# alguoo314/JASPER

Hardware: AMD Instinct MI355X
Metric: assembly Mbp/s polished + Gk-mers/s counted, k=37 (higher is better)
Workload: dtype u64

## Files before the change

jasper_amd/csrc/polish.hip:

```cpp
#include "polish.hpp"
#include <algorithm>

namespace jk {

constexpr int SMAX = 384;

__device__ __forceinline__ void pyslice(int64_t len, int64_t a, int64_t b, int64_t &lo, int64_t &hi) {
    if (a < 0) { a += len; if (a < 0) a = 0; } else if (a > len) a = len;
    if (b < 0) { b += len; if (b < 0) b = 0; } else if (b > len) b = len;
    if (b < a) b = a;
    lo = a; hi = b;
}

__device__ __forceinline__ int64_t pyround(double x) { return (int64_t)rint(x); }

struct FrontEntry {
    uint32_t node;
    uint16_t tlen;
    uint8_t alive;
    uint8_t pad;
    uint8_t tail[72];
};
static_assert(sizeof(FrontEntry) == 80, "FrontEntry layout");

// ... 701 lines not shown
            nlook += 64;
            if (m) {
                const int f = (int)__builtin_ctzll(m);
                if (__shfl((int)oob, f)) spec_fail = 1;
                j = j - (int64_t)f;
                break;
            }
            j -= 64;
        }
        if (j < -1) j = -1;
        int64_t gb = j + k - 1;
        uint32_t prev = cnt_seq(j, k + j);
        if (j == -1) gb = -1;
        for (;;) {
            const int64_t il = i + lane;
            bool cont = false;
            if (il < len - k + 1) cont = cnt_seq(il, il + k) < thre;
            const bool giveup = cont && rolling_thre != 0 && (il - j > k);
            const uint64_t m = __ballot(!cont || giveup);
            nlook += 64;
            if (m) {
                const int f = (int)__builtin_ctzll(m);
                const bool g = __shfl((int)giveup, f) != 0;
                i += f;
                if (!is_last && i >= len - k + 1) spec_fail = 1;
                if (g) return i + 1;
                break;
            }
            i += 64;
        }
        int64_t ga = i;
        nlook += 4;
        if (2ull * cnt_seq(gb - k + 2, gb + 2) < (uint64_t)solid && 2ull * cnt_seq(gb - k + 3, gb + 3) < (uint64_t)solid) {
        } else if (rolling_thre == 0) {
            while (2ull * cnt_seq(gb - k + 2, gb + 2) >= (uint64_t)prev && gb - k + 1 < ga) {
                if (gb == -1) break;
                if (2ull * prev >= (uint64_t)thre && 2ull * cnt_seq(gb - k + 2, gb + 2) < (uint64_t)thre &&
                    2ull * cnt_seq(gb - k + 3, gb + 3) < (uint64_t)thre) break;
                prev = cnt_seq(gb - k + 2, gb + 2);
                gb++;
                nlook += 4;
            }
            if (gb >= len - 1) { if (!is_last) spec_fail = 1; brk = true; return i; }
        }
        int64_t s0 = gb - k + 2; if (s0 < 0) s0 = 0;
        if (s0 + k + k >= len) { if (!is_last) spec_fail = 1; brk = true; return s0 + k + k; }
        {
            uint32_t c = 0;
            if (lane == 0) c = cnt_seq(s0 + 1, s0 + k + 1);
            else if (lane == 1) c = cnt_seq(s0 + k - 2, s0 + k + k - 2);
            else if (lane == 2) c = cnt_seq(s0 + k - 1, s0 + k + k - 1);
            else if (lane == 3) c = cnt_seq(s0 + k, s0 + k + k);
            const uint64_t lowm = __ballot(lane < 4 && c < thre) & 0xFull;
            nlook += 4;
            if (lowm == 0x7ull) ga = s0 + k;
        }
        int64_t tlo, thi;
        pyslice(len, s0, ga + k - 1, tlo, thi);
        int64_t n = ga - s0; if (n < 0) n = 0;
        wrong += n;
        const uint64_t tf0 = phase_clock();
        tk[1] += tf0 - th0;
        struct FixTimer { uint64_t &acc; uint64_t t0; __device__ ~FixTimer() { acc += phase_clock() - t0; } } fix_timer{tk[2], tf0};
        if (fix) {
            if (gb < 0) return i;
            const int64_t L = thi - tlo;
            if (n <= k) {
                if (L > SMAX) { status = PS_STRING_TOO_LONG; return i; }
                cp_seq(s_tbf, tlo, thi);
                sync();
            }
            fixing_sid(L, thre, n, gb, ga);
            sync();
        }
        return i;
    }

    __device__ int64_t skip_good(int64_t i) {
        const int64_t end = len - k + 1;
        for (;;) {
            const int64_t p = i + (int64_t)lane * (k - 1);
            bool ev = true;
            bool known = false;
            if (p < end && cls != nullptr && p >= dirty_end + k) {
                const int64_t o = p - delta + seg_lo;
                if (!is_last && o >= stop_orig) known = true;
                else if (o >= 0 && o < cls_n) { known = true; ev = cls[o] != PC_CLEAN; }
            }
            if (p < end && !known) {
                uint32_t w[16];
                load_window(p, k, w);
                int nv;
                const u128 m = encode_words(w, k, nv);
                const bool valid = nv == k;
                if (valid) {
                    const uint32_t occ = clamp32(table_get(T, mix(canonical(m, k), T.B)));
                    ev = occ < solid;
                    if (!ev && p > 0) {
                        const int64_t a = p - k > 0 ? p - k : 0;
                        const int64_t b = p > k ? p : k;
                        ev = 50ull * occ < (uint64_t)cnt_seq(a, b);
                    }
                }
            }
            const uint64_t mask = __ballot(ev);
            nlook += 128;
            if (mask) return i + (int64_t)__builtin_ctzll(mask) * (k - 1);
            i += 64ll * (k - 1);
        }
    }

    __device__ void walk(bool fix, int64_t start_i, int64_t &wrong_out, long long &arrive_out) {
        int64_t i = start_i, wrong = 0;
        bool handed_over = false;
        arrive_out = ARRIVE_FAIL;
        while (i < len - k + 1 && status == PS_OK) {
            if (__ballot(spec_fail != 0)) { spec_fail = 1; break; }
            const uint64_t ts0 = phase_clock();
            i = skip_good(i);
            tk[0] += phase_clock() - ts0;
            if (i >= len - k + 1) { if (!is_last) spec_fail = 1; break; }
            if (!is_last && (i - delta + seg_lo) >= stop_orig) {
                if (i < dirty_end + k) spec_fail = 1;
                else { handed_over = true; arrive_out = i - delta + seg_lo; }
                break;
            }
            uint8_t ch = 'A';
            if (lane < k) ch = at(i + lane);
            const uint64_t inwin = (k >= 64) ? ~0ull : ((1ull << k) - 1ull);
            const uint64_t mN = __ballot(ch == 'N') & inwin;
            if (mN) {
                const int f = (int)__builtin_ctzll(mN);
                i += f + 1;
                if (f == 0) {
                    for (;;) {
                        const int64_t q = i + lane;
                        const bool stop = !(q < len - k + 1 && at(q) == 'N');
                        const uint64_t m = __ballot(stop);
                        if (m) { i += (int64_t)__builtin_ctzll(m); break; }
                        i += 64;
                    }
                }
                continue;
            }
            const uint64_t mn = __ballot(ch == 'n') & inwin;
            if (mn) { i += (int64_t)__builtin_ctzll(mn) + 1; continue; }
            const uint64_t mo = __ballot(code(ch) < 0) & inwin;
            if (mo) { i += 1; continue; }
            const uint32_t occ = cnt_seq(i, i + k);
            nlook += 1;
            bool brk = false;
            if (occ < solid) {
                i = handle_bad_kmers(i, wrong, fix, 0, brk);
                if (brk) break;
                continue;
            }
            bool cond2 = false;
            if (i > 0) {
                const int64_t a = i - k > 0 ? i - k : 0;
                const int64_t b = i > k ? i : k;
                cond2 = 50ull * occ < (uint64_t)cnt_seq(a, b);
                nlook += 1;
            }
            if (!cond2) { i += k - 1; continue; }
            int64_t ind0 = i - k > 0 ? i - k : 0;
            int64_t num = (i - ind0 + step - 1) / step;
            double sum = 0.0;
            for (int64_t base = 0; base < num; base += 64) {
                const int64_t t = base + lane;
                unsigned long long c = 0;
                if (t < num) { const int64_t ind = ind0 + (t + 1) * step; c = cnt_seq(ind, ind + k); }
                for (int o = 32; o > 0; o >>= 1) c += __shfl_xor(c, o);
                sum += (double)c;
            }
            nlook += (uint64_t)num;
            const int64_t rolling = pyround(sum / (double)num / 50.0);
            if ((int64_t)occ < rolling) {
                i = handle_bad_kmers(i, wrong, fix, pyround(sum / (double)num / 2.0), brk);
                if (brk) break;
            } else {
                i += k - 1;
            }
        }
        if (!is_last && !handed_over && status == PS_OK) spec_fail = 1;
        if (__ballot(spec_fail != 0)) spec_fail = 1;
        if (is_last && status == PS_OK && !spec_fail) arrive_out = ARRIVE_END;
        if (spec_fail || status != PS_OK) arrive_out = ARRIVE_FAIL;
        wrong_out = wrong;
    }
};

__device__ __forceinline__ void publish_arrival(long long *slot, long long v) {
    if (threadIdx.x == 0) __hip_atomic_store(slot, v, __ATOMIC_RELAXED, __HIP_MEMORY_SCOPE_AGENT);
}

__global__ __launch_bounds__(64, 2) void seg_walk_kernel(TableDev T, SegDev *segs, int n_segs, PolishParams P, int pass, ScratchPool pool,
                                                      unsigned int *ticket) {
    __shared__ uint8_t s_tbf[SMAX], s_t1[SMAX], s_t2[SMAX], s_gkb[64], s_gka[64];
    unsigned int tk = 0;
    if (threadIdx.x == 0) tk = atomicAdd(ticket, 1u);
    const int c = (int)__shfl(tk, 0);
    if (c >= n_segs) return;
    SegDev *C = &segs[c];
    if (C->status != PS_OK) { publish_arrival(C->arrive, ARRIVE_FAIL); return; }
    if (!C->chain_in) publish_arrival(C->arrive, ARRIVE_WALKING);
    const int k = P.k;
    const int lane = threadIdx.x;
    const uint64_t t0 = wall_clock64();
    int64_t start_i = C->start_i;
    if (C->chain_in) {
        const int64_t lo = C->seg_lo + 4ll * k;
        int64_t hi = C->last ? C->cls_n : C->stop_orig + k;
        if (hi > C->cls_n) hi = C->cls_n;
        bool dirty = C->cls == nullptr;
        static_assert(PC_CLEAN == 0, "the clean test below ORs class bytes");
        for (int64_t p0 = lo; p0 < hi && !dirty; p0 += 64 * 16) {
            bool nc = false;
            const int64_t p = p0 + (int64_t)lane * 16;
            if (p + 16 <= hi) {
                struct __attribute__((packed, aligned(1))) V16 { uint32_t w[4]; };
                const V16 v = *reinterpret_cast<const V16 *>(C->cls + p);
                nc = (v.w[0] | v.w[1] | v.w[2] | v.w[3]) != 0u;
            } else {
                for (int q = 0; q < 16; ++q) nc = nc || (p + q < hi && C->cls[p + q] != PC_CLEAN);
            }
            dirty = __ballot(nc) != 0ull;
        }
        if (lane == 0) __hip_atomic_store(C->arrive, dirty ? ARRIVE_WALKING : ARRIVE_CLEAN, __ATOMIC_RELAXED, __HIP_MEMORY_SCOPE_AGENT);
        long long a = ARRIVE_FAIL;
        {
            int back = 1;
            for (uint32_t spins = 0;; ++spins) {
                const int idx = c - back - lane;
                long long v = ARRIVE_FAIL;
                if (idx >= 0) v = __hip_atomic_load(C->arrive - (c - idx), __ATOMIC_RELAXED, __HIP_MEMORY_SCOPE_AGENT);
                const bool published = v >= 0 || v == ARRIVE_FAIL || v == ARRIVE_END;
                const bool skip = v == ARRIVE_CLEAN && !dirty;
                const unsigned long long stopper = __ballot(!skip);
                if (stopper) {
                    const int l = (int)__builtin_ctzll(stopper);
                    const bool ok = (__ballot(published) >> l) & 1ull;
                    if (ok) {
                        a = __shfl(v, l);
                        if (back + l > 1 && a >= 0) {
                            const long long stop = segs[c - 1].stop_orig;
                            if (a < stop) a += ((stop - a + (k - 2)) / (k - 1)) * (long long)(k - 1);
                        }
                        break;
                    }
                    if (spins > (1u << 24)) { a = ARRIVE_FAIL; break; }
                    __builtin_amdgcn_s_sleep(4);
                } else {
                    back += 64;
                    if (spins > (1u << 24)) { a = ARRIVE_FAIL; break; }
                }
            }
        }
        if (a < 0 || a < lo || a - C->seg_lo >= C->len0) {
            if (lane == 0) { C->spec_fail = 1; C->ticks = wall_clock64() - t0; }
            publish_arrival(C->arrive, ARRIVE_FAIL);
            return;
        }
        if (!dirty) {
            const int64_t stop = C->last ? C->cls_n : C->stop_orig;
            const int64_t steps = a >= stop ? 0 : (stop - a + (k - 2)) / (k - 1);
            if (lane == 0) {
                C->took_shortcut = 1;
                C->lookups = 2ull * (uint64_t)steps;
                C->ticks = wall_clock64() - t0;
            }
            publish_arrival(C->arrive, C->last ? ARRIVE_END : a + steps * (k - 1));
            return;
        }
        start_i = a - C->seg_lo;
    }
    Walker w;
    w.T = T; w.k = P.k; w.step = P.step; w.lane = threadIdx.x; w.solid = P.solid;
    w.buf = C->buf; w.len = C->len; w.gs = C->gs; w.glen = C->glen; w.cap = C->cap;
    w.C = C; w.chunk_id = C->chunk; w.nrec = 0; w.naux = 0; w.seqno = 0; w.nedit = 0; w.pass = pass;
    w.status = PS_OK; w.nlook = 0; for (int q = 0; q < 12; ++q) w.tk[q] = 0;
    w.s_tbf = s_tbf; w.s_t1 = s_t1; w.s_t2 = s_t2; w.s_gkb = s_gkb; w.s_gka = s_gka;
    w.delta = 0; w.dirty_end = INT64_MIN / 2; w.glo = P.k;
    w.is_first = C->first != 0; w.is_last = C->last != 0; w.spec_fail = 0;
    w.cls = C->cls; w.cls_n = C->cls_n; w.seg_lo = C->seg_lo; w.stop_orig = C->stop_orig;
    w.pool = pool; w.bfs_slot = -1; w.bfs_nodes = nullptr; w.bfs_front = nullptr; w.bfs_patch = nullptr;
    const bool fix = P.fix && pass < P.passes;
    int64_t wrong = 0;
    long long arrive = ARRIVE_FAIL;
    w.walk(fix, start_i, wrong, arrive);
    w.release_scratch();
    if (threadIdx.x == 0) {
        C->ticks = wall_clock64() - t0;
        for (int q = 0; q < 12; ++q) C->tk[q] = w.tk[q];
        C->len = w.len; C->gs = w.gs; C->glen = w.glen;
        C->nrec = w.nrec; C->naux = w.naux; C->nedit = w.nedit; C->status = w.status; C->spec_fail = w.spec_fail;
        C->wrong = wrong;
        C->lookups = w.nlook;
    }
    publish_arrival(C->arrive, arrive);
}

constexpr int SC_THREADS = 256, SC_GROUP = 16, SC_TILE = SC_THREADS * SC_GROUP, SC_HALO = 4;

__global__ __launch_bounds__(256) void seg_init_kernel(SegDev *segs, int n_segs, const uint8_t *const *chunk_text) {
    struct __attribute__((packed, aligned(1))) V16 { uint32_t w[4]; };
    for (int s = blockIdx.y; s < n_segs; s += gridDim.y) {
        const SegDev S = segs[s];
        const uint8_t *src = chunk_text[S.chunk] + S.seg_lo;
        uint8_t *dst = S.buf + S.glen;
        const int64_t nblk = (S.len0 + 15) >> 4;
        for (int64_t blk = blockIdx.x * (int64_t)blockDim.x + threadIdx.x; blk < nblk; blk += (int64_t)gridDim.x * blockDim.x) {
            const int64_t q0 = blk << 4;
            if (q0 + 16 <= S.len0) *reinterpret_cast<V16 *>(dst + q0) = *reinterpret_cast<const V16 *>(src + q0);
            else for (int64_t q = q0; q < S.len0; ++q) dst[q] = src[q];
        }
    }
}

constexpr uint32_t STITCH_MAX_EDITS = 32;
__global__ __launch_bounds__(256) void seg_stitch_kernel(const SegDev *segs, int n_segs, uint8_t *const *chunk_out, uint8_t *const *cls_out,
                                                         uint8_t *const *flags) {
    struct __attribute__((packed, aligned(1))) V16 { uint32_t w[4]; };
    for (int s = blockIdx.y; s < n_segs; s += gridDim.y) {
        const SegDev S = segs[s];
        uint8_t *dst = chunk_out[S.chunk] + S.out_off;
        uint8_t *cdst = cls_out ? cls_out[S.chunk] + S.out_off : nullptr;
        uint8_t *fl = cls_out ? flags[S.chunk] : nullptr;
        const int64_t n = S.own_hi - S.own_lo;
        const bool all_dirty = S.nedit > STITCH_MAX_EDITS;
        const int64_t nblk = (n + 15) >> 4;
        for (int64_t blk = blockIdx.x * (int64_t)blockDim.x + threadIdx.x; blk < nblk; blk += (int64_t)gridDim.x * blockDim.x) {
            const int64_t q0 = blk << 4;
            const int64_t p0 = S.own_lo + q0;
            const bool full = q0 + 16 <= n;
            bool text_done = false, cls_done = !cdst;
            if (full && (p0 + 16 <= S.gs || p0 >= S.gs)) {
                *reinterpret_cast<V16 *>(dst + q0) = *reinterpret_cast<const V16 *>(S.buf + (p0 < S.gs ? p0 : p0 + S.glen));
                text_done = true;
            }
            if (full && cdst && !all_dirty) {
                int64_t lA = p0, lB = p0 + 15;
                bool uniform = true;
                for (int e = (int)S.nedit - 1; e >= 0; --e) {
                    const EditRec E = S.edits[e];
                    if (lA > E.a + E.plen) { const int64_t d = (int64_t)E.plen - E.oldlen; lA -= d; lB -= d; }
                    else if (lB < E.a - 1) { }
                    else { uniform = false; break; }
                }
                if (uniform && S.seg_lo + lB < S.cls_n) {
                    *reinterpret_cast<V16 *>(cdst + q0) = *reinterpret_cast<const V16 *>(S.cls + S.seg_lo + lA);
                    cls_done = true;
                }
            }
            if (text_done && cls_done) continue;
            const int64_t qe = q0 + 16 < n ? q0 + 16 : n;
            for (int64_t q = q0; q < qe; ++q) {
                const int64_t p = S.own_lo + q;
                if (!text_done) dst[q] = S.buf[p < S.gs ? p : p + S.glen];
                if (cls_done) continue;
                int64_t l = p;
                bool dirty = all_dirty;
                if (!dirty)
                    for (int e = (int)S.nedit - 1; e >= 0; --e) {
                        const EditRec E = S.edits[e];
                        if (l > E.a + E.plen) l -= (int64_t)E.plen - E.oldlen;
                        else if (l >= E.a - 1) { dirty = true; break; }
                    }
                if (dirty) {
                    fl[(S.out_off + q) >> 6] = 1;
                    cdst[q] = PC_OTHER;
                } else {
                    const int64_t old = S.seg_lo + l;
                    cdst[q] = old < S.cls_n ? S.cls[old] : (uint8_t)PC_OTHER;
                }
            }
        }
    }
}

__global__ __launch_bounds__(64) void seg_gather_kernel(const SegDev *segs, int n_segs, const int64_t *idx_base, const uint32_t *seq_base,
                                                        const uint32_t *rec_off, const uint32_t *aux_off, FixRec *out_recs, uint8_t *out_aux) {
    const int s = blockIdx.x;
    if (s >= n_segs) return;
    const SegDev S = segs[s];
    for (uint32_t r = threadIdx.x; r < S.nrec; r += blockDim.x) {
        FixRec f = S.recs[r];
        f.index += idx_base[s];
        f.seqno += seq_base[s];
        if (f.kind == 'x') f.aux_off += aux_off[s];
        out_recs[rec_off[s] + r] = f;
    }
    for (uint32_t q = threadIdx.x; q < S.naux; q += blockDim.x) out_aux[aux_off[s] + q] = S.aux[q];
}

__device__ __forceinline__ long long wave_scan_incl64(long long v) {
    const int lane = threadIdx.x & 63;
#pragma unroll
    for (int o = 1; o < 64; o <<= 1) { const long long u = __shfl_up(v, o); if (lane >= o) v += u; }
    return v;
}
__global__ __launch_bounds__(64) void seg_summary_kernel(SegDev *segs, const int32_t *first_seg, int n_chunks, int64_t *idx_base, uint32_t *seq_base,
                                                         uint32_t *rec_off, uint32_t *aux_off, ChunkSummary *out) {
    const int c = blockIdx.x;
    if (c >= n_chunks) return;
    const int lane = threadIdx.x;
    const int s0 = first_seg[c], s1 = first_seg[c + 1];
    long long newlen = 0, shift = 0, seqc = 0, recc = 0, auxc = 0, wrong = 0, lookups = 0;
    int bad = -1, spec = 0;
    for (int base = s0; base < s1; base += 64) {
        const int s = base + lane;
        const bool in = s < s1;
        long long d = 0, own = 0, nrec = 0, naux = 0, seg_lo = 0, own_hi = 0;
        if (in) {
            SegDev &S = segs[s];
            d = S.len - S.len0;
            own_hi = S.last ? S.len : S.own_hi0 + d;
            own = own_hi - S.own_lo;
            nrec = S.nrec; naux = S.naux; seg_lo = S.seg_lo;
            wrong += S.wrong; lookups += (long long)S.lookups;
            if (S.status != PS_OK && (bad < 0 || s < bad)) bad = s;
            if (S.spec_fail && S.status == PS_OK) spec = 1;
        }
        const long long i_own = wave_scan_incl64(own), i_d = wave_scan_incl64(d), i_rec = wave_scan_incl64(nrec), i_aux = wave_scan_incl64(naux);
        if (in) {
            SegDev &S = segs[s];
            S.own_hi = own_hi;
            S.out_off = newlen + i_own - own;
            idx_base[s] = seg_lo + shift + i_d - d;
            seq_base[s] = (uint32_t)(seqc + i_rec - nrec);
            rec_off[s] = (uint32_t)(recc + i_rec - nrec);
            aux_off[s] = (uint32_t)(auxc + i_aux - naux);
        }
        newlen += __shfl(i_own, 63); shift += __shfl(i_d, 63);
        seqc += __shfl(i_rec, 63); recc += __shfl(i_rec, 63); auxc += __shfl(i_aux, 63);
    }
    for (int o = 32; o > 0; o >>= 1) {
        wrong += __shfl_xor(wrong, o); lookups += __shfl_xor(lookups, o);
        const int b2 = __shfl_xor(bad, o);
        bad = bad < 0 ? b2 : (b2 < 0 ? bad : (b2 < bad ? b2 : bad));
        spec |= __shfl_xor(spec, o);
    }
    if (lane == 0) {
        ChunkSummary R;
        R.newlen = newlen; R.wrong = wrong; R.lookups = (uint64_t)lookups; R.nrec = (uint32_t)recc; R.naux = (uint32_t)auxc; R.bad_seg = bad; R.spec_fail = spec;
        out[c] = R;
    }
}
__global__ __launch_bounds__(64) void seg_offsets_kernel(const int32_t *first_seg, int n_chunks, uint32_t *rec_off, uint32_t *aux_off, const ChunkSummary *sum) {
    const int c = blockIdx.x;
    if (c >= n_chunks || c == 0) return;
    const int lane = threadIdx.x;
    unsigned long long rb = 0, ab = 0;
    for (int q = lane; q < c; q += 64) { rb += sum[q].nrec; ab += sum[q].naux; }
    for (int o = 32; o > 0; o >>= 1) { rb += __shfl_xor(rb, o); ab += __shfl_xor(ab, o); }
    for (int s = first_seg[c] + lane; s < first_seg[c + 1]; s += 64) { rec_off[s] += (uint32_t)rb; aux_off[s] += (uint32_t)ab; }
}

constexpr int SC_BACK = 64;
constexpr int SC_STRIDE = SC_TILE - SC_BACK;
__global__ __launch_bounds__(SC_THREADS) void scan_classify_batch_kernel(const ScanChunk *__restrict__ chunks, int n_chunks, TableDev T, uint32_t solid) {
    __shared__ uint32_t s_code[SC_THREADS + SC_HALO];
    __shared__ uint32_t s_inv[SC_THREADS + SC_HALO];
    __shared__ uint32_t s_cnt[SC_TILE];
    __shared__ uint8_t s_ok[SC_TILE];
    const int t = threadIdx.x;
    const int k = T.k;
    const u128 kmask = maskbits(2 * k);
    for (int ci = blockIdx.y; ci < n_chunks; ci += gridDim.y) {
        const ScanChunk C = chunks[ci];
        const uint8_t *__restrict__ text = C.text;
        const int64_t n = C.len;
        const int64_t nwin = n - k + 1;
        if (nwin <= 0) continue;
        const int64_t ntiles = (n + SC_STRIDE - 1) / SC_STRIDE;
        for (int64_t tile = blockIdx.x; tile < ntiles; tile += gridDim.x) {
            const int64_t origin = tile * SC_STRIDE - SC_BACK;
            uint32_t c, iv;
            stage16(text, origin + (int64_t)t * SC_GROUP, n, c, iv);
            s_code[t + SC_HALO] = c;
            s_inv[t + SC_HALO] = iv;
            if (t < SC_HALO) {
                uint32_t hc, hiv;
                stage16(text, origin - (int64_t)(SC_HALO - t) * SC_GROUP, n, hc, hiv);
                s_code[t] = hc;
                s_inv[t] = hiv;
            }
            __syncthreads();
            const uint32_t w4 = s_code[t], w3 = s_code[t + 1], w2 = s_code[t + 2], w1 = s_code[t + 3];
            const uint64_t ivprev = ((uint64_t)s_inv[t] << 48) | ((uint64_t)s_inv[t + 1] << 32) | ((uint64_t)s_inv[t + 2] << 16) |
                                    (uint64_t)s_inv[t + 3];
            u128 fwd = band(mk(((uint64_t)w4 << 32) | w3, ((uint64_t)w2 << 32) | w1), kmask);
            u128 rc = revcomp(fwd, k);
            int run = ivprev ? (int)__builtin_ctzll(ivprev) : 64;
            const int64_t e0 = origin + (int64_t)t * SC_GROUP;
#pragma unroll
            for (int j0 = 0; j0 < SC_GROUP; j0 += 4) {
                u128 hs[4];
                bool ok[4];
                ulonglong2 ent[4];
#pragma unroll
                for (int u = 0; u < 4; ++u) {
                    const int j = j0 + u;
                    const uint32_t cj = (c >> (30 - 2 * j)) & 3u;
                    const bool bad = (iv >> (15 - j)) & 1u;
                    fwd = band(bor(shl(fwd, 2), mk(0, cj)), kmask);
                    rc = bor(shr(rc, 2), shl(mk(0, 3u - cj), 2 * (k - 1)));
                    run = bad ? 0 : run + 1;
                    const int64_t e = e0 + j;
                    ok[u] = run >= k && e - k + 1 >= 0 && e < n;
                    hs[u] = mix(lt(rc, fwd) ? rc : fwd, T.B);
                    ent[u] = make_ulonglong2(0ull, 0ull);
                    if (ok[u]) ent[u] = *reinterpret_cast<const ulonglong2 *>(read_slots(T, hs[u]) + 2 * home_of(hs[u], T.B, T.s));
                }
#pragma unroll
                for (int u = 0; u < 4; ++u) {
                    s_cnt[t * SC_GROUP + j0 + u] = ok[u] ? clamp32(table_get_prefetched(T, hs[u], ent[u])) : 0u;
                    s_ok[t * SC_GROUP + j0 + u] = ok[u] ? 1 : 0;
                }
            }
            __syncthreads();
            if (t >= SC_BACK / SC_GROUP) {
                struct __attribute__((packed, aligned(1))) V16 { uint32_t w[4]; };
                V16 out;
                out.w[0] = out.w[1] = out.w[2] = out.w[3] = 0;
                const int64_t p0 = e0 - k + 1;
#pragma unroll
                for (int j = 0; j < SC_GROUP; ++j) {
                    const int64_t p = p0 + j;
                    const uint32_t me = s_cnt[t * SC_GROUP + j];
                    uint8_t cl;
                    if (!s_ok[t * SC_GROUP + j]) cl = PC_OTHER;
                    else if (me < solid) cl = PC_BAD;
                    else if (p > 0) {
                        const int64_t qe = (p - k > 0 ? p - k : 0) + k - 1;
                        const int qi = (int)(qe - origin);
                        cl = (!s_ok[qi] || 50ull * me < (unsigned long long)s_cnt[qi]) ? PC_OTHER : PC_CLEAN;
                    } else cl = PC_CLEAN;
                    out.w[j >> 2] |= (uint32_t)cl << (8 * (j & 3));
                }
                if (p0 >= 0 && p0 + SC_GROUP <= nwin) *reinterpret_cast<V16 *>(C.cls + p0) = out;
                else {
#pragma unroll
                    for (int j = 0; j < SC_GROUP; ++j) {
                        const int64_t p = p0 + j;
                        if (p >= 0 && p < nwin) C.cls[p] = (uint8_t)((out.w[j >> 2] >> (8 * (j & 3))) & 0xFFu);
                    }
                }
            }
            __syncthreads();
        }
    }
}

__global__ __launch_bounds__(256) void find_sync_batch_kernel(const ScanChunk *__restrict__ chunks, int n_chunks, int k) {
    struct __attribute__((packed, aligned(1))) V16 { uint32_t w[4]; };
    const int64_t W = 4ll * k;
    for (int ci = blockIdx.y; ci < n_chunks; ci += gridDim.y) {
        const ScanChunk C = chunks[ci];
        if (!C.want_sync) continue;
        const int64_t nwin = C.len - k + 1;
        const uint8_t *__restrict__ cls = C.cls;
        static_assert(PC_CLEAN == 0 && PC_BAD == 1 && PC_OTHER == 2, "the block test below looks at bit 0 of the class bytes");
        const int64_t nblk = (nwin + 15) >> 4;
        for (int64_t blk = blockIdx.x * (int64_t)blockDim.x + threadIdx.x; blk < nblk; blk += (int64_t)gridDim.x * blockDim.x) {
            const int64_t p0 = blk << 4;
            uint32_t w[4];
            if (p0 + 16 <= nwin) {
                const V16 v = *reinterpret_cast<const V16 *>(cls + p0);
                w[0] = v.w[0]; w[1] = v.w[1]; w[2] = v.w[2]; w[3] = v.w[3];
                if (!((w[0] | w[1] | w[2] | w[3]) & 0x01010101u)) continue;
            }
            const int64_t pe = p0 + 16 < nwin ? p0 + 16 : nwin;
            for (int64_t p = p0; p < pe; ++p) {
                if (p < W || p + k - 1 > nwin) continue;
                if (cls[p] != PC_BAD || cls[p - 1] != PC_CLEAN) continue;
                uint32_t diff = 0;
                {
                    int64_t q = p + 1;
                    const int64_t qe = p + k - 1;
                    for (; q + 16 <= qe; q += 16) {
                        const V16 v = *reinterpret_cast<const V16 *>(cls + q);
                        diff |= (v.w[0] ^ 0x01010101u) | (v.w[1] ^ 0x01010101u) | (v.w[2] ^ 0x01010101u) | (v.w[3] ^ 0x01010101u);
                    }
                    for (; q < qe; ++q) diff |= (uint32_t)(cls[q] ^ (uint8_t)PC_BAD);
                    q = p - W;
                    const int64_t qf = p - 1;
                    for (; q + 16 <= qf; q += 16) {
                        const V16 v = *reinterpret_cast<const V16 *>(cls + q);
                        diff |= v.w[0] | v.w[1] | v.w[2] | v.w[3];
                    }
                    for (; q < qf; ++q) diff |= (uint32_t)cls[q];
                }
                if (diff) continue;
                const unsigned int idx = atomicAdd(C.cand_count, 1u);
                if (idx < C.cand_cap) C.cand[idx] = ((int64_t)ci << 40) | p;
            }
        }
    }
}

__global__ __launch_bounds__(256) void rescan_batch_kernel(const ScanChunk *__restrict__ chunks, int n_chunks, TableDev T, uint32_t solid) {
    __shared__ uint32_t s_cnt[4][128];
    __shared__ uint8_t s_valid[4][128];
    __shared__ uint8_t s_text[4][256];
    const int wave = threadIdx.x >> 6, lane = threadIdx.x & 63;
    const int k = T.k;
    for (int ci = blockIdx.y; ci < n_chunks; ci += gridDim.y) {
        const ScanChunk C = chunks[ci];
        const int64_t nwin = C.len - k + 1;
        if (nwin <= 0) continue;
        const int64_t ntile = (nwin + 63) >> 6, nflag = (C.len >> 6) + 1;
        const int64_t W = (int64_t)gridDim.x * 4;
        for (int64_t tile0 = (int64_t)blockIdx.x * 4 + wave; tile0 < ntile; tile0 += 64 * W) {
            uint8_t f = 0;
            {
                const int64_t tl = tile0 + (int64_t)lane * W;
                if (tl < ntile) {
                    f = C.flags[tl];
                    if (tl > 0) f |= C.flags[tl - 1];
                    if (tl + 1 < nflag) f |= C.flags[tl + 1];
                }
            }
            unsigned long long todo = __ballot(f != 0);
          while (todo) {
            const int64_t tile = tile0 + (int64_t)__builtin_ctzll(todo) * W;
            todo &= todo - 1ull;
            const int64_t base = tile * 64 - 64;
#pragma unroll
            for (int q = 0; q < 4; ++q) {
                const int64_t pos = base + (int64_t)lane * 4 + q;
                s_text[wave][lane * 4 + q] = (pos >= 0 && pos < C.len) ? C.text[pos] : (uint8_t)'N';
            }
            __builtin_amdgcn_fence(__ATOMIC_SEQ_CST, "workgroup");
            __builtin_amdgcn_wave_barrier();
#pragma unroll
            for (int r = 0; r < 2; ++r) {
                const int64_t p = base + r * 64 + lane;
                uint32_t cnt = 0;
                uint8_t valid = 0;
                if (p >= 0 && p < nwin) {
                    u128 fwd = mk(0, 0);
                    bool ok = true;
                    for (int j = 0; j < k; ++j) {
                        const int c = code(s_text[wave][r * 64 + lane + j]);
                        ok = ok && c >= 0;
                        fwd = bor(shl(fwd, 2), mk(0, (uint64_t)(c & 3)));
                    }
                    if (ok) {
                        cnt = clamp32(table_get(T, mix(canonical(fwd, k), T.B)));
                        valid = 1;
                    }
                }
                s_cnt[wave][r * 64 + lane] = cnt;
                s_valid[wave][r * 64 + lane] = valid;
            }
            __builtin_amdgcn_fence(__ATOMIC_SEQ_CST, "workgroup");
            __builtin_amdgcn_wave_barrier();
            const int64_t p = tile * 64 + lane;
            if (p < nwin) {
                const int me = 64 + lane;
                uint8_t c;
                if (!s_valid[wave][me]) c = PC_OTHER;
                else if (s_cnt[wave][me] < solid) c = PC_BAD;
                else if (p > 0) {
                    const int qi = p - k > 0 ? me - k : 64;
                    c = (!s_valid[wave][qi] || 50ull * s_cnt[wave][me] < (unsigned long long)s_cnt[wave][qi]) ? PC_OTHER : PC_CLEAN;
                } else c = PC_CLEAN;
                C.cls[p] = c;
            }
            __builtin_amdgcn_wave_barrier();
          }
        }
    }
}

__global__ __launch_bounds__(64) void find_clean_batch_kernel(const ScanChunk *__restrict__ chunks, int n_chunks, int k) {
    const int lane = threadIdx.x;
    for (int ci = blockIdx.y; ci < n_chunks; ci += gridDim.y) {
        const ScanChunk C = chunks[ci];
        const int64_t nwin = C.len - k + 1;
        for (uint32_t g = blockIdx.x; g < C.n_cells; g += gridDim.x) {
            int64_t p0 = (int64_t)g * CLEAN_CELL + CLEAN_CELL / 2;
            const int64_t cell_end = (int64_t)(g + 1) * CLEAN_CELL;
            int64_t cand = -1;
            for (int attempt = 0; attempt < 8; ++attempt) {
                if (p0 - 4ll * k < 0 || p0 + k > nwin || p0 + k > cell_end) break;
                int64_t last_bad = -1;
                for (int64_t q0 = p0 - 4ll * k; q0 < p0 + k; q0 += 64) {
                    const int64_t q = q0 + lane;
                    const bool nc = q < p0 + k && C.cls[q] != PC_CLEAN;
                    const uint64_t m = __ballot(nc);
                    if (m) last_bad = q0 + 63 - (int64_t)__builtin_clzll(m);
                }
                if (last_bad < 0) { cand = p0; break; }
                p0 = last_bad + 4ll * k + 1;
            }
            if (lane == 0) C.clean_cand[g] = cand;
        }
    }
}

static void launch_find_clean(const ScanChunk *d_chunks, int n_chunks, int k, hipStream_t stream) {
    const int gy = n_chunks < 1024 ? n_chunks : 1024;
    const int gx = std::max(1, 8192 / gy);
    hipLaunchKernelGGL(find_clean_batch_kernel, dim3(gx, gy), dim3(64), 0, stream, d_chunks, n_chunks, k);
}

void launch_rescan_batch(const TableDev &T, const ScanChunk *d_chunks, int n_chunks, int k, uint32_t solid, hipStream_t stream) {
    if (n_chunks <= 0) return;
    const int gy = n_chunks < 1024 ? n_chunks : 1024;
    const int gx = std::max(1, 4096 / gy);
    hipLaunchKernelGGL(rescan_batch_kernel, dim3(gx, gy), dim3(256), 0, stream, d_chunks, n_chunks, T, solid);
    hipLaunchKernelGGL(find_sync_batch_kernel, dim3(gx, gy), dim3(256), 0, stream, d_chunks, n_chunks, k);
    launch_find_clean(d_chunks, n_chunks, k, stream);
}

void launch_scan_batch(const TableDev &T, const ScanChunk *d_chunks, int n_chunks, int k, uint32_t solid, hipStream_t stream) {
    if (n_chunks <= 0) return;
    const int gy = n_chunks < 1024 ? n_chunks : 1024;
    const int gx = std::max(1, 4096 / gy);
    hipLaunchKernelGGL(scan_classify_batch_kernel, dim3(gx, gy), dim3(SC_THREADS), 0, stream, d_chunks, n_chunks, T, solid);
    hipLaunchKernelGGL(find_sync_batch_kernel, dim3(gx, gy), dim3(256), 0, stream, d_chunks, n_chunks, k);
    launch_find_clean(d_chunks, n_chunks, k, stream);
}

__global__ __launch_bounds__(256) void copy_chunks_kernel(uint8_t *const *__restrict__ chunk_ptr, uint8_t *__restrict__ pack, const int64_t *__restrict__ offs, int n,
                                                          int to_chunks) {
    for (int c = blockIdx.x; c < n; c += gridDim.x) {
        const int64_t len = offs[c + 1] - offs[c];
        uint8_t *a = chunk_ptr[c], *b = pack + offs[c];
        const uint8_t *src = to_chunks ? b : a;
        uint8_t *dst = to_chunks ? a : b;
        for (int64_t i = threadIdx.x; i < len; i += 256) dst[i] = src[i];
    }
}
void launch_copy_chunks(uint8_t *const *d_chunk_ptr, uint8_t *d_pack, const int64_t *d_offs, int n, bool to_chunks, hipStream_t stream) {
    if (n <= 0) return;
    hipLaunchKernelGGL(copy_chunks_kernel, dim3((unsigned)std::min(n, 256 * 16)), dim3(256), 0, stream, d_chunk_ptr, d_pack, d_offs, n, to_chunks ? 1 : 0);
}

void launch_seg_init(SegDev *d_segs, int n_segs, const uint8_t *const *d_chunk_text, hipStream_t stream) {
    if (n_segs <= 0) return;
    dim3 grid(n_segs >= 512 ? 4 : 64, n_segs < 4096 ? n_segs : 4096);
    hipLaunchKernelGGL(seg_init_kernel, grid, dim3(256), 0, stream, d_segs, n_segs, d_chunk_text);
}
void launch_seg_walk(const TableDev &T, SegDev *d_segs, int n_segs, PolishParams pp, int pass, ScratchPool pool, unsigned int *d_ticket,
                     hipStream_t stream) {
    if (n_segs <= 0) return;
    (void)hipMemsetAsync(d_ticket, 0, sizeof(unsigned int), stream);
    hipLaunchKernelGGL(seg_walk_kernel, dim3(n_segs), dim3(64), 0, stream, T, d_segs, n_segs, pp, pass, pool, d_ticket);
}
void launch_seg_summary(SegDev *d_segs, int n_segs, const int32_t *d_first_seg, int n_chunks, int64_t *idx_base, uint32_t *seq_base, uint32_t *rec_off,
                        uint32_t *aux_off, ChunkSummary *d_out, hipStream_t stream) {
    if (n_segs <= 0 || n_chunks <= 0) return;
    hipLaunchKernelGGL(seg_summary_kernel, dim3(n_chunks), dim3(64), 0, stream, d_segs, d_first_seg, n_chunks, idx_base, seq_base, rec_off, aux_off, d_out);
    hipLaunchKernelGGL(seg_offsets_kernel, dim3(n_chunks), dim3(64), 0, stream, d_first_seg, n_chunks, rec_off, aux_off, d_out);
}
void launch_seg_gather(const SegDev *d_segs, int n_segs, const int64_t *idx_base, const uint32_t *seq_base, const uint32_t *rec_off,
                       const uint32_t *aux_off, FixRec *out_recs, uint8_t *out_aux, hipStream_t stream) {
    if (n_segs <= 0) return;
    hipLaunchKernelGGL(seg_gather_kernel, dim3(n_segs), dim3(64), 0, stream, d_segs, n_segs, idx_base, seq_base, rec_off, aux_off, out_recs, out_aux);
}
void launch_seg_stitch(const SegDev *d_segs, int n_segs, uint8_t *const *d_chunk_out, uint8_t *const *d_cls_out, uint8_t *const *d_flags,
                       hipStream_t stream) {
    if (n_segs <= 0) return;
    dim3 grid(n_segs >= 2048 ? 2 : n_segs >= 512 ? 4 : 64, n_segs < 4096 ? n_segs : 4096);
    hipLaunchKernelGGL(seg_stitch_kernel, grid, dim3(256), 0, stream, d_segs, n_segs, d_chunk_out, d_cls_out, d_flags);
}

}
```

jasper_amd/csrc/polish.hpp:

```cpp
#pragma once
#include "table.hpp"

namespace jk {

struct FixRec {
    int64_t index;
    uint32_t chunk;
    uint32_t seqno;
    uint8_t pass;
    uint8_t kind;
    uint8_t newc;
    uint8_t oldc;
    uint32_t rep;
    uint32_t aux_off;
    uint32_t aux_len;
};
static_assert(sizeof(FixRec) == 32, "FixRec layout");

enum PolishStatus {
    PS_OK = 0,
    PS_GAP_EXHAUSTED = 1,
    PS_REC_OVERFLOW = 2,
    PS_AUX_OVERFLOW = 3,
    PS_BFS_ARENA = 4,
    PS_REF_INDEXERROR = 5,
    PS_STRING_TOO_LONG = 6
};

enum PosClass : uint8_t {
    PC_CLEAN = 0,
    PC_BAD = 1,
    PC_OTHER = 2
};

struct ScratchPool {
    unsigned int *locks;
    uint8_t *base;
    size_t stride;
    uint32_t nslots;
    uint32_t node_cap;
    uint32_t front_cap;
    uint32_t patch_cap;
    size_t off_front, off_patch;
};

struct EditRec {
    int64_t a;
    int32_t plen, oldlen;
};

struct SegDev {
    uint8_t *buf;
    int64_t cap;
    int64_t len;
    int64_t gs, glen;
    int64_t len0;
    int64_t seg_lo;
    int64_t start_i;
    int64_t stop_orig;
    int32_t first, last;
    int32_t chain_in;
    int32_t took_shortcut;
    long long *arrive;
    const uint8_t *cls;
    int64_t cls_n;
    FixRec *recs;
    uint32_t rec_cap, nrec;
    uint8_t *aux;
    uint32_t aux_cap, naux;
    EditRec *edits;
    uint32_t edit_cap, nedit;
    uint32_t chunk;
    int32_t status;
    int32_t spec_fail;
    int64_t wrong;
    uint64_t lookups;
    uint64_t ticks;
    uint64_t tk[12];
    int64_t own_lo, own_hi;
    int64_t own_hi0;
    int64_t out_off;
};

struct ChunkSummary {
    int64_t newlen;
    int64_t wrong;
    uint64_t lookups;
    uint32_t nrec, naux;
    int32_t bad_seg;
    int32_t spec_fail;
};

constexpr long long ARRIVE_PENDING = (long long)0x8080808080808080ull;
constexpr long long ARRIVE_FAIL = -2, ARRIVE_END = -1;
constexpr long long ARRIVE_CLEAN = -3, ARRIVE_WALKING = -4;

struct PolishParams {
    int k;
    int step;
    uint32_t solid;
    int passes;
    int fix;
};

struct ScanChunk {
    const uint8_t *text;
    int64_t len;
    uint8_t *cls;
    int64_t *cand;
    unsigned int *cand_count;
    unsigned int cand_cap;
    int32_t want_sync;
    const uint8_t *flags;
    int64_t *clean_cand;
    uint32_t n_cells;
};
constexpr int64_t CLEAN_CELL = 65536;
void launch_scan_batch(const TableDev &T, const ScanChunk *d_chunks, int n_chunks, int k, uint32_t solid, hipStream_t stream);
void launch_rescan_batch(const TableDev &T, const ScanChunk *d_chunks, int n_chunks, int k, uint32_t solid, hipStream_t stream);

void launch_copy_chunks(uint8_t *const *d_chunk_ptr, uint8_t *d_pack, const int64_t *d_offs, int n, bool to_chunks, hipStream_t stream);
void launch_seg_init(SegDev *d_segs, int n_segs, const uint8_t *const *d_chunk_text, hipStream_t stream);
void launch_seg_walk(const TableDev &T, SegDev *d_segs, int n_segs, PolishParams pp, int pass, ScratchPool pool, unsigned int *d_ticket,
                     hipStream_t stream);
void launch_seg_stitch(const SegDev *d_segs, int n_segs, uint8_t *const *d_chunk_out, uint8_t *const *d_cls_out, uint8_t *const *d_flags,
                       hipStream_t stream);
void launch_seg_summary(SegDev *d_segs, int n_segs, const int32_t *d_first_seg, int n_chunks, int64_t *idx_base, uint32_t *seq_base, uint32_t *rec_off,
                        uint32_t *aux_off, ChunkSummary *d_out, hipStream_t stream);
void launch_seg_gather(const SegDev *d_segs, int n_segs, const int64_t *idx_base, const uint32_t *seq_base, const uint32_t *rec_off,
                       const uint32_t *aux_off, FixRec *out_recs, uint8_t *out_aux, hipStream_t stream);

}
```

jasper_amd/csrc/polish_host.hip:

```cpp
#include "polish_host.hpp"
#include <algorithm>
#include <chrono>
#include <cstdio>
#include <cstdlib>
#include <cstring>
#include <thread>

namespace jk {

#define HIPCHK(x)                                                                     \
    do {                                                                              \
        hipError_t e_ = (x);                                                          \
        if (e_ != hipSuccess) {                                                       \
            err = std::string(#x) + ": " + hipGetErrorString(e_);                     \
            return -1;                                                                \
        }                                                                             \
    } while (0)

static inline size_t al256(size_t x) { return (x + 255) & ~(size_t)255; }

namespace {
struct DevBuf {
    void *p = nullptr;
    bool owned = false;
    ~DevBuf() { if (p && owned) (void)hipFree(p); }
    template <typename T> T *as() { return reinterpret_cast<T *>(p); }
};
}

static int run_polish_lane(Table &T, const int lane, hipStream_t st, int n_chunks, const char *const *seqs, const int64_t *lens, int solid_thre, int passes, int fix,
                           PolishOut &R, std::string &err, bool device_in, bool keep_on_device, int roomy) {
    const int64_t RM = roomy ? 8 : 1;
    const bool tight = !roomy && getenv("JASPER_POLISH_TIGHT") != nullptr;
    const int k = T.k;
    const int64_t W = 4ll * k;
    const int64_t M = 3ll * k;
    const int64_t TMIN = 1024;
    const int64_t CMIN = 32768;
    HIPCHK(hipSetDevice(T.device));
    const int ws_base = lane ? Table::WS_LANE0 + (lane - 1) * Table::WS_POLISH_MAX : 0, pin_base = lane * Table::PIN_PER_LANE;
    R.seqs.assign(n_chunks, std::string());
    R.d_seqs.clear();
    R.d_lens.clear();
    R.aux.assign(n_chunks, std::string());
    R.recs.clear();
    R.qv[0] = R.qv[1] = R.qv[2] = R.qv[3] = 0;
    R.qv_chunk.assign((size_t)4 * n_chunks, 0);
    R.lookups = 0;
    R.seconds = 0;
    R.n_segments = 0;
    R.n_respeculated = 0;
    if (n_chunks == 0) return 0;

    const bool dbg = getenv("JASPER_POLISH_DEBUG") != nullptr;
    auto now = []() { return std::chrono::duration<double, std::milli>(std::chrono::steady_clock::now().time_since_epoch()).count(); };
    const double t_begin = now();
    std::vector<int64_t> len(lens, lens + n_chunks), cap(n_chunks);
    std::vector<size_t> off_text(n_chunks), off_pos(n_chunks), off_cand(n_chunks), off_flag(n_chunks), off_cell(n_chunks);
    std::vector<uint32_t> n_cells(n_chunks);
    size_t cell_items = 0;
    std::vector<uint32_t> cand_cap(n_chunks);
    size_t text_bytes = 0, pos_items = 0, cand_items = 0, flag_items = 0, seg_text_bound = 0, seg_rec_bound = 0, seg_aux_bound = 0;
    int64_t max_segs = 0;
    for (int c = 0; c < n_chunks; ++c) {
        cap[c] = len[c] + RM * std::max<int64_t>(4096, len[c] / 8) + 64;
        off_text[c] = text_bytes;  text_bytes += al256((size_t)cap[c]);
        off_pos[c] = pos_items;    pos_items += al256((size_t)cap[c]);
        cand_cap[c] = (uint32_t)std::min<int64_t>(1 << 28, cap[c] / (4 * k) + 16);
        off_cand[c] = cand_items;  cand_items += cand_cap[c];
        off_flag[c] = flag_items;  flag_items += al256((size_t)(cap[c] >> 6) + 2);
        n_cells[c] = (uint32_t)(cap[c] / CLEAN_CELL + 1);
        off_cell[c] = cell_items;  cell_items += n_cells[c];
        const int64_t ms = cap[c] / TMIN + 2;
        max_segs += ms;
        const int64_t tb = cap[c] + ms * (W + M + 64);
        seg_text_bound += (size_t)(tb + RM * (tb / 8 + ms * 1280));
        seg_rec_bound += (size_t)(RM * (2 * tb / k + 16 * ms));
        seg_aux_bound += (size_t)(RM * (2 * tb + 1024 * ms));
    }
    DevBuf b_textA, b_textB, b_pack, b_cls, b_clsB, b_flags, b_segedit, b_cells, b_arrive, b_ptrA, b_segs, b_segtext, b_segrec, b_segaux, b_pool, b_locks, b_scan, b_ticket;
    int ws_next = 0;
    auto dmalloc = [&](DevBuf &b, size_t bytes) -> bool {
        if (ws_next >= Table::WS_POLISH_MAX) { err = "polish: workspace slots exhausted"; return false; }
        b.p = T.workspace(ws_base + ws_next++, bytes, err);
        b.owned = false;
        return b.p != nullptr;
    };
    if (!dmalloc(b_textA, text_bytes) || !dmalloc(b_textB, text_bytes) || 
        !dmalloc(b_cls, pos_items) || !dmalloc(b_clsB, pos_items) || !dmalloc(b_flags, flag_items) ||
        !dmalloc(b_segedit, seg_rec_bound * sizeof(EditRec)) || !dmalloc(b_cells, (2 + cell_items + cand_items) * 8) ||
        !dmalloc(b_arrive, ((size_t)max_segs + 4) * 8) ||
        !dmalloc(b_ptrA, (size_t)6 * n_chunks * sizeof(void *)) ||
        !dmalloc(b_segs, (size_t)max_segs * sizeof(SegDev)) || !dmalloc(b_segtext, seg_text_bound) ||
        !dmalloc(b_segrec, seg_rec_bound * sizeof(FixRec)) || !dmalloc(b_segaux, seg_aux_bound))
        return -2;
    ScratchPool pool;
    pool.nslots = 256;
    pool.node_cap = (uint32_t)(RM << 18);
    pool.front_cap = 20480;
    pool.patch_cap = (uint32_t)(RM << 16);
    if (roomy) pool.nslots = 64;
    if (const char *e = getenv("JASPER_POLISH_TEST_NSLOTS")) pool.nslots = (uint32_t)std::max(1, std::min(atoi(e), 256));
    pool.off_front = al256((size_t)pool.node_cap * 4);
    pool.off_patch = pool.off_front + al256((size_t)pool.front_cap * 80);
    pool.stride = pool.off_patch + al256(pool.patch_cap);
    if (!dmalloc(b_pool, pool.stride * pool.nslots) || !dmalloc(b_locks, pool.nslots * 4) || !dmalloc(b_scan, sizeof(ScanChunk) * n_chunks) ||
        !dmalloc(b_ticket, 256)) return -2;
    DevBuf b_first, b_sum, b_idx, b_seq, b_ro, b_ao;
    if (!dmalloc(b_first, ((size_t)n_chunks + 1) * 4) || !dmalloc(b_sum, (size_t)n_chunks * sizeof(ChunkSummary)) || !dmalloc(b_idx, (size_t)max_segs * 8) ||
        !dmalloc(b_seq, (size_t)max_segs * 4) || !dmalloc(b_ro, (size_t)max_segs * 4) || !dmalloc(b_ao, (size_t)max_segs * 4)) return -2;
    const size_t PIN_RECS = 1u << 18, PIN_AUX = 8u << 20;
    SegDev *segs_p = reinterpret_cast<SegDev *>(T.pinned(pin_base + 0, (size_t)max_segs * sizeof(SegDev), err));
    int32_t *first_p = reinterpret_cast<int32_t *>(T.pinned(pin_base + 1, ((size_t)n_chunks + 1) * 4, err));
    ChunkSummary *sum_p = reinterpret_cast<ChunkSummary *>(T.pinned(pin_base + 2, (size_t)n_chunks * sizeof(ChunkSummary), err));
    int64_t *cand_p = reinterpret_cast<int64_t *>(T.pinned(pin_base + 3, (std::min<size_t>(cand_items, 32768) + cell_items + 8) * 8, err));
    FixRec *recs_p = reinterpret_cast<FixRec *>(T.pinned(pin_base + 4, PIN_RECS * sizeof(FixRec), err));
    uint8_t *aux_p = reinterpret_cast<uint8_t *>(T.pinned(pin_base + 5, PIN_AUX, err));
    ScanChunk *sc_p = reinterpret_cast<ScanChunk *>(T.pinned(pin_base + 6, sizeof(ScanChunk) * (size_t)n_chunks, err));
    if (!segs_p || !first_p || !sum_p || !cand_p || !recs_p || !aux_p || !sc_p) return -2;
    int64_t total_len = 0;
    for (int c = 0; c < n_chunks; ++c) total_len += len[c];
    const bool packed_io = !device_in && n_chunks > 256 && total_len / n_chunks < 65536 && !getenv("JASPER_POLISH_NO_PACKED_IO");
    DevBuf b_iooffs;
    std::vector<int64_t> io_offs;
    uint8_t *io_stage = nullptr;
    if (!packed_io) ws_next += 2;
    if (packed_io) {
        if (!dmalloc(b_iooffs, ((size_t)n_chunks + 1) * 8) || !dmalloc(b_pack, text_bytes)) return -2;
        io_offs.resize((size_t)n_chunks + 1);
        io_stage = reinterpret_cast<uint8_t *>(T.pinned(pin_base + 7, std::max<size_t>((size_t)total_len, 1) + (size_t)(RM * std::max<int64_t>(4096, total_len / 8)) + 64, err));
        if (!io_stage) return -2;
    }
    size_t pin_recs_used = 0, pin_aux_used = 0;
    struct PinnedPass { size_t rec_at, nrec, aux_at, naux, r0, pass_i; };
    std::vector<PinnedPass> pinned_passes;
    pool.base = b_pool.as<uint8_t>();
    pool.locks = b_locks.as<unsigned int>();
    HIPCHK(hipMemsetAsync(pool.locks, 0, pool.nslots * 4, st));

    uint8_t *clsIn = b_cls.as<uint8_t>(), *clsOut = b_clsB.as<uint8_t>();
    std::vector<uint8_t *> tables((size_t)6 * n_chunks);
    uint8_t **hIn = tables.data(), **hOut = hIn + n_chunks, **hSpare = hOut + n_chunks, **hCA = hSpare + n_chunks, **hCB = hCA + n_chunks,
            **hF = hCB + n_chunks;
    for (int c = 0; c < n_chunks; ++c) {
        uint8_t *a = b_textA.as<uint8_t>() + off_text[c];
        hIn[c] = device_in ? reinterpret_cast<uint8_t *>(const_cast<char *>(seqs[c])) : a;
        hOut[c] = b_textB.as<uint8_t>() + off_text[c];
        hSpare[c] = a;
        hCA[c] = b_cls.as<uint8_t>() + off_pos[c];
        hCB[c] = b_clsB.as<uint8_t>() + off_pos[c];
        hF[c] = b_flags.as<uint8_t>() + off_flag[c];
        if (len[c] && !device_in && !packed_io) HIPCHK(hipMemcpyAsync(a, seqs[c], (size_t)len[c], hipMemcpyHostToDevice, st));
    }
    HIPCHK(hipMemcpyAsync(b_ptrA.p, tables.data(), tables.size() * sizeof(void *), hipMemcpyHostToDevice, st));
    uint8_t **dIn = b_ptrA.as<uint8_t *>(), **dOut = dIn + n_chunks, **dSpare = dOut + n_chunks;
    uint8_t **ptrClsIn = dSpare + n_chunks, **ptrClsOut = ptrClsIn + n_chunks, **ptrFlags = ptrClsOut + n_chunks;
    if (packed_io) {
        int64_t at = 0;
        for (int c = 0; c < n_chunks; ++c) { io_offs[c] = at; if (len[c]) memcpy(io_stage + at, seqs[c], (size_t)len[c]); at += len[c]; }
        io_offs[n_chunks] = at;
        HIPCHK(hipMemcpyAsync(b_iooffs.p, io_offs.data(), io_offs.size() * 8, hipMemcpyHostToDevice, st));
        if (at) HIPCHK(hipMemcpyAsync(b_pack.p, io_stage, (size_t)at, hipMemcpyHostToDevice, st));
        launch_copy_chunks(dIn, b_pack.as<uint8_t>(), b_iooffs.as<int64_t>(), n_chunks, true, st);
        HIPCHK(hipGetLastError());
        HIPCHK(jk_stream_wait(st));
    }

    if (dbg) { (void)jk_stream_wait(st); fprintf(stderr, "[polish] setup + H2D: %.2f ms\n", now() - t_begin); }
    const double t_loop = now();
    PolishParams pp;
    pp.k = k;
    pp.step = std::max(2, (int)std::nearbyint((double)k / 8.0));
    pp.solid = (uint32_t)solid_thre;
    pp.passes = passes;
    pp.fix = fix ? 1 : 0;

    hipEvent_t ev0, ev1;
    HIPCHK(hipEventCreate(&ev0));
    HIPCHK(hipEventCreate(&ev1));
    HIPCHK(hipEventRecord(ev0, st));

    std::vector<SegDev> segs;
    std::vector<ScanChunk> sc(n_chunks);
    int64_t *const d_count = b_cells.as<int64_t>(), *const d_cells = d_count + 2, *const d_cands = d_cells + cell_items;
    std::vector<int64_t> all_cands(cand_items);
    std::vector<int64_t> all_cells(cell_items);
    std::vector<std::vector<int64_t>> chunk_cands(n_chunks);
    std::vector<int64_t> cands;
    std::vector<uint32_t> aux_total(n_chunks, 0);
    std::vector<std::vector<uint8_t>> aux_pass;
    std::vector<size_t> rec_pass_begin;
    int rc = 0;

    for (int pass = 0; pass <= passes && rc == 0; ++pass) {
        HIPCHK(hipMemsetAsync(d_count, 0, 4, st));
        {
            for (int c = 0; c < n_chunks; ++c) {
                ScanChunk &S = sc[c];
                S.text = hIn[c];
                S.len = len[c];
                S.cls = clsIn + off_pos[c];
                S.flags = b_flags.as<uint8_t>() + off_flag[c];
                S.cand = d_cands;
                S.cand_count = reinterpret_cast<unsigned int *>(d_count);
                S.cand_cap = (unsigned int)std::min<size_t>(cand_items, 0x7fffffffu);
                S.want_sync = (len[c] - k + 1) > 2 * TMIN;
                S.clean_cand = d_cells + off_cell[c];
                S.n_cells = (uint32_t)std::min<int64_t>(n_cells[c], std::max<int64_t>(0, len[c] - k + 1) / CLEAN_CELL + 1);
            }
            memcpy(sc_p, sc.data(), sizeof(ScanChunk) * n_chunks);
            HIPCHK(hipMemcpyAsync(b_scan.p, sc_p, sizeof(ScanChunk) * n_chunks, hipMemcpyHostToDevice, st));
            if (pass == 0) launch_scan_batch(T.d, b_scan.as<ScanChunk>(), n_chunks, k, pp.solid, st);
            else launch_rescan_batch(T.d, b_scan.as<ScanChunk>(), n_chunks, k, pp.solid, st);
        }
        HIPCHK(hipGetLastError());
        const size_t CAND_PRE = std::min<size_t>(cand_items, 32768);
        unsigned int n_cand = 0;
        {
            HIPCHK(hipMemcpyAsync(cand_p, d_count, (2 + cell_items + CAND_PRE) * 8, hipMemcpyDeviceToHost, st));
            HIPCHK(jk_stream_wait(st));
            n_cand = *reinterpret_cast<const unsigned int *>(cand_p);
            if (cell_items) memcpy(all_cells.data(), cand_p + 2, cell_items * 8);
            if (CAND_PRE) memcpy(all_cands.data(), cand_p + 2 + cell_items, std::min<size_t>(n_cand, CAND_PRE) * 8);
        }
        n_cand = (unsigned int)std::min<size_t>(n_cand, cand_items);
        if (n_cand > CAND_PRE) {
            HIPCHK(hipMemcpyAsync(all_cands.data() + CAND_PRE, d_cands + CAND_PRE, (n_cand - CAND_PRE) * 8, hipMemcpyDeviceToHost, st));
            HIPCHK(jk_stream_wait(st));
        }
        for (int c = 0; c < n_chunks; ++c) chunk_cands[c].clear();
        for (unsigned int i = 0; i < n_cand; ++i) {
            const int64_t v = all_cands[i];
            const int64_t c = v >> 40;
            if (c >= 0 && c < n_chunks) chunk_cands[c].push_back(v & ((1ll << 40) - 1));
        }

        auto build_segments = [&](const std::vector<int> &chunks, bool speculate, SegDev *out, size_t &n_out, int32_t *first_of, std::string &e2) -> int {
            n_out = 0;
            size_t tpos = 0, rpos = 0, apos = 0, ci = 0;
            for (int c : chunks) {
                if (first_of) first_of[ci++] = (int32_t)n_out;
                std::vector<int64_t> sync;
                if (speculate && !chunk_cands[c].empty()) {
                    cands = chunk_cands[c];
                    std::sort(cands.begin(), cands.end());
                    int64_t last = 0;
                    for (int64_t p : cands)
                        if (p - last >= TMIN && len[c] - p >= TMIN) { sync.push_back(p); last = p; }
                }
                std::vector<char> chained(sync.size(), 0);
                if (speculate && len[c] - k + 1 > 2 * CMIN) {
                    const uint32_t nc = sc[c].n_cells;
                    std::vector<int64_t> merged;
                    std::vector<char> mtype;
                    size_t si = 0;
                    int64_t last = 0;
                    for (uint32_t g = 0; g <= nc; ++g) {
                        const int64_t p = g < nc ? all_cells[off_cell[c] + g] : INT64_MAX;
                        while (si < sync.size() && sync[si] <= p) { merged.push_back(sync[si]); mtype.push_back(0); last = sync[si]; ++si; }
                        if (g == nc || p < 0) continue;
                        const int64_t next = si < sync.size() ? sync[si] : len[c];
                        if (p - last >= CMIN && next - p >= CMIN) { merged.push_back(p); mtype.push_back(1); last = p; }
                    }
                    sync.swap(merged);
                    chained.swap(mtype);
                }
                const int m = (int)sync.size();
                if ((int64_t)n_out + m + 1 > max_segs) { e2 = "polish: internal segment arena bound exceeded"; return -2; }
                for (int j = 0; j <= m; ++j) {
                    SegDev &S = out[n_out++];
                    memset(&S, 0, sizeof S);
                    S.chunk = (uint32_t)c;
                    S.first = (j == 0);
                    S.last = (j == m);
                    S.seg_lo = j == 0 ? 0 : sync[j - 1] - W;
                    S.start_i = j == 0 ? 0 : W;
                    S.chain_in = j > 0 && chained[j - 1];
                    S.arrive = b_arrive.as<long long>() + n_out;
                    S.stop_orig = j == m ? INT64_MAX : sync[j];
                    const int64_t seg_hi = j == m ? len[c] : std::min<int64_t>(len[c], sync[j] + M);
                    S.len0 = seg_hi - S.seg_lo;
                    S.len = S.len0;
                    S.cap = S.len0 + (tight ? 2 : RM * std::max<int64_t>(1024, S.len0 / 8));
                    S.gs = 0;
                    S.glen = S.cap - S.len0;
                    S.cls = (len[c] - k + 1 > 0) ? clsIn + off_pos[c] : nullptr;
                    S.cls_n = std::max<int64_t>(0, len[c] - k + 1);
                    S.rec_cap = (uint32_t)std::min<int64_t>(0x7fffffff, RM * (2 * S.len0 / k + 16));
                    S.aux_cap = (uint32_t)std::min<int64_t>(0x7fffffff, RM * (2 * S.len0 + 1024));
                    S.buf = b_segtext.as<uint8_t>() + tpos;            tpos += al256((size_t)S.cap);
                    S.recs = b_segrec.as<FixRec>() + rpos;
                    S.edits = b_segedit.as<EditRec>() + rpos;
                    S.edit_cap = S.rec_cap;                            rpos += S.rec_cap;
                    S.aux = b_segaux.as<uint8_t>() + apos;             apos += al256(S.aux_cap);
                    S.own_lo = j == 0 ? 0 : 2ll * k;
                    S.own_hi = j == m ? -1 : (sync[j] - 2ll * k) - S.seg_lo;
                    S.own_hi0 = S.own_hi;
                }
            }
            if (first_of) first_of[ci] = (int32_t)n_out;
            if (tpos > seg_text_bound || rpos > seg_rec_bound || apos > seg_aux_bound || (int64_t)n_out > max_segs) {
                e2 = "polish: internal segment arena bound exceeded"; return -2;
            }
            return 0;
        };
        auto run_segments = [&](SegDev *sv, size_t nsv, bool summary, std::string &e2) -> int {
            if (!nsv) return 0;
            const bool fine = dbg && getenv("JASPER_POLISH_DEBUG") && atoi(getenv("JASPER_POLISH_DEBUG")) >= 2;
            double tf[5] = {fine ? now() : 0, 0, 0, 0, 0};
            if (hipMemcpyAsync(b_segs.p, sv, nsv * sizeof(SegDev), hipMemcpyHostToDevice, st) != hipSuccess) { e2 = "polish: H2D segs"; return -1; }
            if (summary && hipMemcpyAsync(b_first.p, first_p, ((size_t)n_chunks + 1) * 4, hipMemcpyHostToDevice, st) != hipSuccess) { e2 = "polish: H2D first"; return -1; }
            if (fine) { (void)jk_stream_wait(st); tf[1] = now(); }
            launch_seg_init(b_segs.as<SegDev>(), (int)nsv, (const uint8_t *const *)dIn, st);
            if (hipMemsetAsync(b_arrive.p, 0x80, (nsv + 2) * 8, st) != hipSuccess) { e2 = "polish: memset"; return -1; }
            if (fine) { (void)jk_stream_wait(st); tf[2] = now(); }
            launch_seg_walk(T.d, b_segs.as<SegDev>(), (int)nsv, pp, pass, pool, b_ticket.as<unsigned int>(), st);
            if (hipGetLastError() != hipSuccess) { e2 = "polish: kernel launch failed"; return -1; }
            if (fine) { (void)jk_stream_wait(st); tf[3] = now(); }
            if (summary) {
                launch_seg_summary(b_segs.as<SegDev>(), (int)nsv, b_first.as<int32_t>(), n_chunks, b_idx.as<int64_t>(), b_seq.as<uint32_t>(), b_ro.as<uint32_t>(),
                                   b_ao.as<uint32_t>(), b_sum.as<ChunkSummary>(), st);
                if (hipMemcpyAsync(sum_p, b_sum.p, (size_t)n_chunks * sizeof(ChunkSummary), hipMemcpyDeviceToHost, st) != hipSuccess) { e2 = "polish: D2H summary"; return -1; }
            } else if (hipMemcpyAsync(sv, b_segs.p, nsv * sizeof(SegDev), hipMemcpyDeviceToHost, st) != hipSuccess) { e2 = "polish: D2H segs"; return -1; }
            if (jk_stream_wait(st) != hipSuccess) { e2 = "polish: kernel execution failed"; return -1; }
            if (fine) {
                tf[4] = now();
                fprintf(stderr, "[polish]     %zu segments x %zu B: H2D %.3f ms, init + memset %.3f ms, walk %.3f ms, %s %.3f ms\n", nsv, sizeof(SegDev), tf[1] - tf[0], tf[2] - tf[1],
                        tf[3] - tf[2], summary ? "summary + D2H" : "D2H", tf[4] - tf[3]);
            }
            return 0;
        };
        std::vector<int> all(n_chunks);
        for (int c = 0; c < n_chunks; ++c) all[c] = c;
        const double tb0 = dbg ? now() : 0;
        size_t ns = 0;
        if ((rc = build_segments(all, true, segs_p, ns, first_p, err))) break;
        const double tb1 = dbg ? now() : 0;
        if ((rc = run_segments(segs_p, ns, true, err))) break;
        if (dbg) fprintf(stderr, "[polish]   host: build %zu segments %.3f ms, upload + walk + summary %.3f ms\n", ns, tb1 - tb0, now() - tb1);

        bool ordinary = !getenv("JASPER_POLISH_DEBUG") && !getenv("JASPER_POLISH_HOST_BOOKKEEPING");
        for (int c = 0; c < n_chunks && ordinary; ++c) ordinary = sum_p[c].bad_seg < 0 && !sum_p[c].spec_fail;
        std::vector<int64_t> idx_base;
        std::vector<uint32_t> seq_base, rec_off, aux_off;
        std::vector<int64_t> newlen(n_chunks, 0), shift(n_chunks, 0);
        std::vector<uint32_t> seqc(n_chunks, 0);
        size_t nrec_pass = 0, naux_pass = 0;
        if (ordinary) {
            R.n_segments += ns;
            for (int c = 0; c < n_chunks; ++c) {
                const ChunkSummary &S = sum_p[c];
                newlen[c] = S.newlen;
                nrec_pass += S.nrec;
                naux_pass += S.naux;
                R.lookups += S.lookups;
                if (pass == 0) { R.qv[0] += S.wrong; R.qv_chunk[4 * (size_t)c + 0] += S.wrong; }
                if (pass == passes) { R.qv[2] += S.wrong; R.qv_chunk[4 * (size_t)c + 2] += S.wrong; }
            }
        } else {
        segs.resize(ns);
        HIPCHK(hipMemcpyAsync(segs.data(), b_segs.p, ns * sizeof(SegDev), hipMemcpyDeviceToHost, st));
        HIPCHK(jk_stream_wait(st));
        R.n_segments += segs.size();

        std::vector<char> failed(n_chunks, 0);
        bool any_failed = false;
        for (const SegDev &S : segs)
            if (S.spec_fail && S.status == PS_OK) { failed[S.chunk] = 1; any_failed = true; }
        if (any_failed) {
            std::vector<int> redo;
            for (int c = 0; c < n_chunks; ++c) if (failed[c]) redo.push_back(c);
            R.n_respeculated += redo.size();
            std::vector<SegDev> good, bad;
            for (const SegDev &S : segs) if (!failed[S.chunk]) good.push_back(S);
            size_t tpos = 0, rpos = 0, apos = 0;
            for (const SegDev &S : segs) { tpos += al256((size_t)S.cap); rpos += S.rec_cap; apos += al256(S.aux_cap); }
            std::vector<SegDev> redo_segs((size_t)max_segs);
            size_t nredo = 0;
            if ((rc = build_segments(redo, false, redo_segs.data(), nredo, nullptr, err))) break;
            redo_segs.resize(nredo);
            size_t t2 = tpos, r2 = rpos, a2 = apos;
            for (SegDev &S : redo_segs) {
                S.buf = b_segtext.as<uint8_t>() + t2;  t2 += al256((size_t)S.cap);
                S.recs = b_segrec.as<FixRec>() + r2;
                S.edits = b_segedit.as<EditRec>() + r2; r2 += S.rec_cap;
                S.aux = b_segaux.as<uint8_t>() + a2;   a2 += al256(S.aux_cap);
            }
            if (t2 > seg_text_bound || r2 > seg_rec_bound || a2 > seg_aux_bound) {
                segs.assign((size_t)max_segs, SegDev{});
                size_t nall = 0;
                if ((rc = build_segments(all, false, segs.data(), nall, nullptr, err))) break;
                segs.resize(nall);
                if ((rc = run_segments(segs.data(), segs.size(), false, err))) break;
            } else {
                if ((rc = run_segments(redo_segs.data(), redo_segs.size(), false, err))) break;
                segs = good;
                segs.insert(segs.end(), redo_segs.begin(), redo_segs.end());
                std::stable_sort(segs.begin(), segs.end(), [](const SegDev &a, const SegDev &b) {
                    return a.chunk != b.chunk ? a.chunk < b.chunk : a.seg_lo < b.seg_lo;
                });
            }
        }
        if (getenv("JASPER_POLISH_DEBUG")) {
            uint64_t mx = 0, sum = 0, mxl = 0; int64_t mxlen = 0; size_t nrecs = 0, mxrec = 0;
            uint64_t tks[12] = {0, 0, 0, 0, 0, 0, 0, 0, 0, 0, 0, 0}, mxtk[12] = {0, 0, 0, 0, 0, 0, 0, 0, 0, 0, 0, 0};
            for (const SegDev &S : segs) {
                sum += S.ticks; nrecs += S.nrec;
                for (int q = 0; q < 12; ++q) tks[q] += S.tk[q];
                if (S.ticks > mx) { mx = S.ticks; mxl = S.lookups; mxlen = S.len0; mxrec = S.nrec; for (int q = 0; q < 12; ++q) mxtk[q] = S.tk[q]; }
            }
            fprintf(stderr, "[polish] pass %d: %zu segments, %zu records, walk ticks(10ns): mean %.0f max %llu (that segment: len %lld, %llu lookups, %zu records)\n",
                    pass, segs.size(), nrecs, segs.empty() ? 0.0 : (double)sum / segs.size(), (unsigned long long)mx, (long long)mxlen,
                    (unsigned long long)mxl, mxrec);
            fprintf(stderr, "[polish]   of all walk ticks: skip_good %.1f%%, find run %.1f%%, choose fix %.1f%% (of which splice %.1f%%)\n",
                    100.0 * tks[0] / (sum + 1), 100.0 * tks[1] / (sum + 1), 100.0 * tks[2] / (sum + 1), 100.0 * tks[3] / (sum + 1));
            fprintf(stderr, "[polish]   inside choose fix: k_case_sub %.1f%%, insert %.1f%%, del %.1f%%, diploid %.1f%%, same_base_del %.1f%%, same_base_ins %.1f%%, path search %.1f%%\n",
                    100.0 * tks[4] / (sum + 1), 100.0 * tks[5] / (sum + 1), 100.0 * tks[6] / (sum + 1), 100.0 * tks[7] / (sum + 1),
                    100.0 * tks[8] / (sum + 1), 100.0 * tks[9] / (sum + 1), 100.0 * tks[10] / (sum + 1));
            fprintf(stderr, "[polish]   slowest segment (10ns ticks): skip %llu, find run %llu, choose fix %llu [sub %llu ins %llu del %llu diploid %llu sb_del %llu sb_ins %llu path %llu], splice %llu\n",
                    (unsigned long long)mxtk[0], (unsigned long long)mxtk[1], (unsigned long long)mxtk[2], (unsigned long long)mxtk[4], (unsigned long long)mxtk[5],
                    (unsigned long long)mxtk[6], (unsigned long long)mxtk[7], (unsigned long long)mxtk[8], (unsigned long long)mxtk[9], (unsigned long long)mxtk[10],
                    (unsigned long long)mxtk[3]);
            int hb[8] = {0, 0, 0, 0, 0, 0, 0, 0};
            for (const SegDev &S : segs) { double ms = S.ticks * 1e-5; int b = ms < 0.1 ? 0 : ms < 0.3 ? 1 : ms < 1 ? 2 : ms < 2 ? 3 : ms < 4 ? 4 : ms < 8 ? 5 : ms < 16 ? 6 : 7; hb[b]++; }
            fprintf(stderr, "[polish]   segments by walk time: <0.1ms %d, <0.3 %d, <1 %d, <2 %d, <4 %d, <8 %d, <16 %d, more %d\n", hb[0], hb[1], hb[2], hb[3], hb[4], hb[5], hb[6], hb[7]);
        }

        ns = segs.size();
        idx_base.assign(ns, 0);
        seq_base.assign(ns, 0); rec_off.assign(ns, 0); aux_off.assign(ns, 0);
        for (size_t s = 0; s < ns && rc == 0; ++s) {
            SegDev &S = segs[s];
            const int c = (int)S.chunk;
            if (S.status != PS_OK) {
                static const char *names[] = {"ok", "text grew beyond its slack", "fix-record buffer overflow", "aux buffer overflow",
                                              "path-extension scratch exhausted", "reference IndexError (src/jasper.py:221)",
                                              "trial string too long"};
                err = std::string("polish: chunk ") + std::to_string(c) + ": " + names[S.status];
                rc = S.status == PS_REF_INDEXERROR ? -4 : -2;
                break;
            }
            const int64_t d = S.len - S.len0;
            S.own_hi = S.last ? S.len : S.own_hi0 + d;
            S.out_off = newlen[c];
            newlen[c] += S.own_hi - S.own_lo;
            idx_base[s] = S.seg_lo + shift[c];
            shift[c] += d;
            seq_base[s] = seqc[c];
            seqc[c] += S.nrec;
            rec_off[s] = (uint32_t)nrec_pass;
            aux_off[s] = (uint32_t)naux_pass;
            nrec_pass += S.nrec;
            naux_pass += S.naux;
            R.lookups += S.lookups;
            if (pass == 0) { R.qv[0] += S.wrong; R.qv_chunk[4 * (size_t)c + 0] += S.wrong; }
            if (pass == passes) { R.qv[2] += S.wrong; R.qv_chunk[4 * (size_t)c + 2] += S.wrong; }
        }
        if (rc) break;
        }
        if (rc) break;
        for (int c = 0; c < n_chunks; ++c) {
            if (pass == 0) { R.qv[1] += len[c] - k + 1; R.qv_chunk[4 * (size_t)c + 1] += len[c] - k + 1; }
            if (pass == passes) { R.qv[3] += len[c] - k + 1; R.qv_chunk[4 * (size_t)c + 3] += len[c] - k + 1; }
            if (newlen[c] > cap[c]) { err = "polish: chunk grew beyond its slack"; rc = -2; }
        }
        if (rc) break;

        rec_pass_begin.push_back(R.recs.size());
        aux_pass.emplace_back();
        const int64_t *g_idx = b_idx.as<int64_t>();
        const uint32_t *g_seq = b_seq.as<uint32_t>(), *g_ro = b_ro.as<uint32_t>(), *g_ao = b_ao.as<uint32_t>();
        if (!ordinary) {
            HIPCHK(hipMemcpyAsync(b_segs.p, segs.data(), ns * sizeof(SegDev), hipMemcpyHostToDevice, st));
            HIPCHK(hipMemcpyAsync(b_idx.p, idx_base.data(), ns * 8, hipMemcpyHostToDevice, st));
            HIPCHK(hipMemcpyAsync(b_seq.p, seq_base.data(), ns * 4, hipMemcpyHostToDevice, st));
            HIPCHK(hipMemcpyAsync(b_ro.p, rec_off.data(), ns * 4, hipMemcpyHostToDevice, st));
            HIPCHK(hipMemcpyAsync(b_ao.p, aux_off.data(), ns * 4, hipMemcpyHostToDevice, st));
        }
        if (nrec_pass) {
            DevBuf d_recs, d_aux;
            int ws_save = ws_next;
            if (!dmalloc(d_recs, nrec_pass * sizeof(FixRec)) || !dmalloc(d_aux, naux_pass)) { rc = -2; break; }
            ws_next = ws_save;
            launch_seg_gather(b_segs.as<SegDev>(), (int)ns, g_idx, g_seq, g_ro, g_ao, d_recs.as<FixRec>(), d_aux.as<uint8_t>(), st);
            HIPCHK(hipGetLastError());
            const size_t r0 = R.recs.size();
            R.recs.resize(r0 + nrec_pass);
            aux_pass.back().resize(naux_pass);
            if (pin_recs_used + nrec_pass <= PIN_RECS && pin_aux_used + naux_pass <= PIN_AUX) {
                HIPCHK(hipMemcpyAsync(recs_p + pin_recs_used, d_recs.p, nrec_pass * sizeof(FixRec), hipMemcpyDeviceToHost, st));
                if (naux_pass) HIPCHK(hipMemcpyAsync(aux_p + pin_aux_used, d_aux.p, naux_pass, hipMemcpyDeviceToHost, st));
                pinned_passes.push_back(PinnedPass{pin_recs_used, nrec_pass, pin_aux_used, naux_pass, r0, aux_pass.size() - 1});
                pin_recs_used += nrec_pass;
                pin_aux_used += naux_pass;
            } else {
                HIPCHK(hipMemcpyAsync(&R.recs[r0], d_recs.p, nrec_pass * sizeof(FixRec), hipMemcpyDeviceToHost, st));
                if (naux_pass) HIPCHK(hipMemcpyAsync(aux_pass.back().data(), d_aux.p, naux_pass, hipMemcpyDeviceToHost, st));
                HIPCHK(jk_stream_wait(st));
            }
        }
        const bool carry = pass < passes;
        if (carry) HIPCHK(hipMemsetAsync(b_flags.p, 0, flag_items, st));
        launch_seg_stitch(b_segs.as<SegDev>(), (int)ns, (uint8_t *const *)dOut, carry ? (uint8_t *const *)ptrClsOut : nullptr,
                          carry ? (uint8_t *const *)ptrFlags : nullptr, st);
        HIPCHK(hipGetLastError());
        for (int c = 0; c < n_chunks; ++c) len[c] = newlen[c];
        if (!ordinary) HIPCHK(jk_stream_wait(st));
        std::swap(hIn, hOut);
        std::swap(dIn, dOut);
        if (pass == 0) { hOut = hSpare; dOut = dSpare; }
        std::swap(clsIn, clsOut);
        std::swap(ptrClsIn, ptrClsOut);
    }
    if (dbg) { (void)jk_stream_wait(st); fprintf(stderr, "[polish] passes: %.2f ms\n", now() - t_loop); }
    const double t_out = now();
    if (rc == 0) {
        HIPCHK(hipEventRecord(ev1, st));
        if (keep_on_device) {
            R.d_seqs.resize(n_chunks);
            R.d_lens.assign(len.begin(), len.end());
            for (int c = 0; c < n_chunks; ++c) R.d_seqs[c] = hIn[c];
        }
        bool packed_back = false;
        if (packed_io && !keep_on_device) {
            int64_t at = 0;
            for (int c = 0; c < n_chunks; ++c) { io_offs[c] = at; at += len[c]; }
            io_offs[n_chunks] = at;
            if ((size_t)at <= text_bytes && (size_t)at <= (size_t)total_len + (size_t)(RM * std::max<int64_t>(4096, total_len / 8)) + 64) {
                packed_back = true;
                HIPCHK(hipMemcpyAsync(b_iooffs.p, io_offs.data(), io_offs.size() * 8, hipMemcpyHostToDevice, st));
                launch_copy_chunks(dIn, b_pack.as<uint8_t>(), b_iooffs.as<int64_t>(), n_chunks, false, st);
                HIPCHK(hipGetLastError());
                if (at) HIPCHK(hipMemcpyAsync(io_stage, b_pack.p, (size_t)at, hipMemcpyDeviceToHost, st));
            }
        }
        for (int c = 0; c < n_chunks && !keep_on_device && !packed_back; ++c) {
            R.seqs[c].resize((size_t)len[c]);
            if (len[c]) HIPCHK(hipMemcpyAsync(&R.seqs[c][0], hIn[c], (size_t)len[c], hipMemcpyDeviceToHost, st));
        }
        HIPCHK(jk_stream_wait(st));
        if (packed_back)
            for (int c = 0; c < n_chunks; ++c) R.seqs[c].assign(reinterpret_cast<const char *>(io_stage) + io_offs[c], (size_t)len[c]);
        float ms = 0;
        HIPCHK(hipEventElapsedTime(&ms, ev0, ev1));
        R.seconds = ms * 1e-3;
        for (const PinnedPass &P : pinned_passes) {
            memcpy(&R.recs[P.r0], recs_p + P.rec_at, P.nrec * sizeof(FixRec));
            if (P.naux) memcpy(aux_pass[P.pass_i].data(), aux_p + P.aux_at, P.naux);
        }
        for (size_t p = 0; p < rec_pass_begin.size(); ++p) {
            const size_t b = rec_pass_begin[p], e = p + 1 < rec_pass_begin.size() ? rec_pass_begin[p + 1] : R.recs.size();
            for (size_t i = b; i < e; ++i) {
                FixRec &f = R.recs[i];
                if (f.kind == 'x') {
                    std::string &a = R.aux[f.chunk];
                    const size_t n = (size_t)f.aux_len + f.rep;
                    const uint32_t no = (uint32_t)a.size();
                    a.append(reinterpret_cast<const char *>(aux_pass[p].data()) + f.aux_off, n);
                    f.aux_off = no;
                }
            }
        }
        std::stable_sort(R.recs.begin(), R.recs.end(), [](const FixRec &a, const FixRec &b) {
            if (a.chunk != b.chunk) return a.chunk < b.chunk;
            if (a.pass != b.pass) return a.pass < b.pass;
            return a.seqno < b.seqno;
        });
    }
    (void)jk_stream_wait(st);
    if (dbg) fprintf(stderr, "[polish] D2H + record sort: %.2f ms; total %.2f ms\n", now() - t_out, now() - t_begin);
    (void)hipEventDestroy(ev0);
    (void)hipEventDestroy(ev1);
    return rc;
}

int run_polish(Table &T, int n_chunks, const char *const *seqs, const int64_t *lens, int solid_thre, int passes, int fix,
               PolishOut &R, std::string &err, bool device_in, bool keep_on_device, int roomy) {
    HIPCHK(hipSetDevice(T.device));
    if (T.materialize(err)) return -1;
    int lanes = T.polish_calls++ >= 1 && n_chunks >= 12 ? 3 : 1;
    if (const char *e = getenv("JASPER_POLISH_LANES")) lanes = atoi(e);
    if (getenv("JASPER_POLISH_DEBUG")) lanes = 1;
    lanes = std::max(1, std::min(std::min(lanes, (int)Table::POLISH_LANES_MAX), n_chunks / 2));
    if (lanes == 1) return run_polish_lane(T, 0, T.stream, n_chunks, seqs, lens, solid_thre, passes, fix, R, err, device_in, keep_on_device, roomy);

    std::vector<int> order(n_chunks);
    for (int c = 0; c < n_chunks; ++c) order[c] = c;
    std::stable_sort(order.begin(), order.end(), [&](int a, int b) { return lens[a] > lens[b]; });
    std::vector<std::vector<int>> mine(lanes);
    std::vector<int64_t> load(lanes, 0);
    for (int c : order) {
        int l = 0;
        for (int j = 1; j < lanes; ++j) if (load[j] < load[l]) l = j;
        mine[l].push_back(c);
        load[l] += lens[c];
    }
    for (auto &m : mine) std::sort(m.begin(), m.end());
    if (!T.polish_ev) HIPCHK(hipEventCreateWithFlags(&T.polish_ev, hipEventDisableTiming));
    HIPCHK(hipEventRecord(T.polish_ev, T.stream));
    for (int l = 1; l < lanes; ++l) {
        if (!T.polish_stream[l]) HIPCHK(hipStreamCreateWithFlags(&T.polish_stream[l], hipStreamNonBlocking));
        HIPCHK(hipStreamWaitEvent(T.polish_stream[l], T.polish_ev, 0));
    }
    std::vector<PolishOut> out(lanes);
    std::vector<std::string> errs(lanes);
    std::vector<int> rcs(lanes, 0);
    std::vector<std::vector<const char *>> lseqs(lanes);
    std::vector<std::vector<int64_t>> llens(lanes);
    for (int l = 0; l < lanes; ++l)
        for (int c : mine[l]) { lseqs[l].push_back(seqs[c]); llens[l].push_back(lens[c]); }
    auto run = [&](int l) {
        rcs[l] = run_polish_lane(T, l, l ? T.polish_stream[l] : T.stream, (int)mine[l].size(), lseqs[l].data(), llens[l].data(), solid_thre, passes, fix, out[l],
                                 errs[l], device_in, keep_on_device, roomy);
    };
    {
        std::vector<std::thread> th;
        for (int l = 1; l < lanes; ++l) th.emplace_back(run, l);
        run(0);
        for (auto &t : th) t.join();
    }
    for (int want : {-1, -4, -2})
        for (int l = 0; l < lanes; ++l)
            if (rcs[l] == want) { err = errs[l]; return want; }
    for (int l = 0; l < lanes; ++l)
        if (rcs[l]) { err = errs[l]; return rcs[l]; }
    R.seqs.assign(n_chunks, std::string());
    R.aux.assign(n_chunks, std::string());
    R.d_seqs.clear();
    R.d_lens.clear();
    if (keep_on_device) { R.d_seqs.assign(n_chunks, nullptr); R.d_lens.assign(n_chunks, 0); }
    R.recs.clear();
    R.qv[0] = R.qv[1] = R.qv[2] = R.qv[3] = 0;
    R.qv_chunk.assign((size_t)4 * n_chunks, 0);
    R.lookups = 0; R.seconds = 0; R.n_segments = 0; R.n_respeculated = 0;
    for (int l = 0; l < lanes; ++l) {
        PolishOut &O = out[l];
        for (size_t j = 0; j < mine[l].size(); ++j) {
            const int c = mine[l][j];
            R.seqs[c].swap(O.seqs[j]);
            R.aux[c].swap(O.aux[j]);
            if (keep_on_device) { R.d_seqs[c] = O.d_seqs[j]; R.d_lens[c] = O.d_lens[j]; }
            for (int q = 0; q < 4; ++q) R.qv_chunk[4 * (size_t)c + q] = O.qv_chunk[4 * j + q];
        }
        for (FixRec f : O.recs) { f.chunk = (uint32_t)mine[l][f.chunk]; R.recs.push_back(f); }
        for (int q = 0; q < 4; ++q) R.qv[q] += O.qv[q];
        R.lookups += O.lookups;
        R.n_segments += O.n_segments;
        R.n_respeculated += O.n_respeculated;
        R.seconds = std::max(R.seconds, O.seconds);
    }
    std::stable_sort(R.recs.begin(), R.recs.end(), [](const FixRec &a, const FixRec &b) {
        if (a.chunk != b.chunk) return a.chunk < b.chunk;
        if (a.pass != b.pass) return a.pass < b.pass;
        return a.seqno < b.seqno;
    });
    return 0;
}

}
```

jasper_amd/csrc/table.hip:

```cpp
#include "table.hpp"
#include <algorithm>
#include <cmath>
#include <cstdio>
#include <cstdlib>
#include <cstring>
#include <ctime>
#include <thread>
#include <chrono>
#include <vector>

namespace jk {

#define HIPCHK(x)                                                                     \
    do {                                                                              \
        hipError_t e_ = (x);                                                          \
        if (e_ != hipSuccess) {                                                       \
            err = std::string(#x) + ": " + hipGetErrorString(e_);                     \
            return -1;                                                                \
        }                                                                             \
    } while (0)

constexpr int CT_THREADS = 256;
constexpr int CT_GROUP = 16;
constexpr int CT_TILE = CT_THREADS * CT_GROUP;
// ... 311 lines not shown
        if (have && idx < cap) out[(size_t)owner * cap + idx] = o;
        __syncthreads();
    }
}

__device__ __forceinline__ int table_set(const TableDev &T, u128 h, unsigned long long val) {
    if (T.ext) return table_put_wide(T, h, val, true);
    const uint64_t home = home_of(h, T.B, T.s);
    const uint64_t rem = rem_of(h, T.B, T.s);
    for (uint32_t off = 0; off < MAXPROBE; ++off) {
        const uint64_t slot = (home + off) & T.mask;
        const unsigned long long want = tag_of(rem, off);
        unsigned long long *p = T.slots + 2 * slot;
        unsigned long long cur = __hip_atomic_load(p, __ATOMIC_RELAXED, __HIP_MEMORY_SCOPE_AGENT);
        int fresh = 1;
        if (cur == 0ull) {
            cur = atomicCAS(p, 0ull, want);
            if (cur == 0ull) { fresh = 2; cur = want; }
        }
        if (cur == want) {
            __hip_atomic_store(p + 1, val, __ATOMIC_RELAXED, __HIP_MEMORY_SCOPE_AGENT);
            return fresh;
        }
    }
    return 0;
}

__global__ __launch_bounds__(256) void import_packed_kernel(const ulonglong2 *__restrict__ in, uint64_t n, TableDev T, int mode) {
    unsigned long long fresh = 0;
    const int sh = packed_count_shift(T.B);
    const unsigned long long himask = sh ? ((1ull << sh) - 1ull) : 0ull;
    for (uint64_t i = blockIdx.x * (uint64_t)blockDim.x + threadIdx.x; i < n; i += (uint64_t)gridDim.x * blockDim.x) {
        const ulonglong2 e = in[i];
        const u128 h = mk(e.y & himask, e.x);
        const unsigned long long c = sh ? (e.y >> sh) : e.y;
        if (!c) continue;
        if (mode == 0) fresh += table_add_or_spill(T, h, c);
        else {
            const int r = table_set(T, h, c);
            if (r == 2) ++fresh;
            else if (r == 0) table_spill(T, h, c);
        }
    }
    for (int o = 32; o > 0; o >>= 1) fresh += __shfl_xor(fresh, o);
    if ((threadIdx.x & 63) == 0 && fresh) atomicAdd(&T.stats[ST_DISTINCT], fresh);
}

struct MultiSrc { const ulonglong2 *p[MAX_SHARDS]; unsigned long long n[MAX_SHARDS]; uint32_t n_src; };
constexpr uint32_t IMP_BPC = 64;
__global__ __launch_bounds__(256) void import_packed_multi_kernel(MultiSrc S, uint32_t nchunks, TableDev T) {
    unsigned long long fresh = 0;
    const int sh = packed_count_shift(T.B);
    const unsigned long long himask = sh ? ((1ull << sh) - 1ull) : 0ull;
    const uint32_t c = blockIdx.x / IMP_BPC, j = blockIdx.x % IMP_BPC;
#pragma unroll 1
    for (uint32_t s = 0; s < S.n_src; ++s) {
        const ulonglong2 *__restrict__ in = S.p[s];
        const unsigned long long lo = S.n[s] / nchunks * c + (S.n[s] % nchunks) * c / nchunks;
        const unsigned long long hi = c + 1 == nchunks ? S.n[s] : S.n[s] / nchunks * (c + 1) + (S.n[s] % nchunks) * (c + 1) / nchunks;
        for (unsigned long long i = lo + (unsigned long long)j * 256 + threadIdx.x; i < hi; i += (unsigned long long)IMP_BPC * 256) {
            const ulonglong2 e = in[i];
            const u128 h = mk(e.y & himask, e.x);
            const unsigned long long cnt = sh ? (e.y >> sh) : e.y;
            if (cnt) fresh += table_add_or_spill(T, h, cnt);
        }
    }
    for (int o = 32; o > 0; o >>= 1) fresh += __shfl_xor(fresh, o);
    if ((threadIdx.x & 63) == 0 && fresh) atomicAdd(&T.stats[ST_DISTINCT], fresh);
}

constexpr uint32_t IMPR_LOG = 12, IMPR = 1u << IMPR_LOG;
__global__ __launch_bounds__(256) void imp_region_hist_kernel(MultiSrc S, TableDev T, uint32_t nreg, unsigned int *__restrict__ hist) {
    const int sh = packed_count_shift(T.B);
    const unsigned long long himask = sh ? ((1ull << sh) - 1ull) : 0ull;
    for (uint32_t s = 0; s < S.n_src; ++s) {
        const ulonglong2 *__restrict__ in = S.p[s];
        unsigned int *__restrict__ hs = hist + (size_t)s * (nreg + 1);
        const unsigned long long n = S.n[s], step = (unsigned long long)gridDim.x * blockDim.x;
        for (unsigned long long i0 = (unsigned long long)blockIdx.x * blockDim.x; i0 < n; i0 += step) {
            const unsigned long long i = i0 + threadIdx.x;
            uint32_t reg = 0xFFFFFFFFu;
            if (i < n) {
                const ulonglong2 e = in[i];
                reg = (uint32_t)(home_of(mk(e.y & himask, e.x), T.B, T.s) >> IMPR_LOG);
            }
            uint64_t todo = __ballot(reg != 0xFFFFFFFFu);
            while (todo) {
                const int leader = (int)__builtin_ctzll(todo);
                const uint32_t r = __shfl(reg, leader);
                const uint64_t same = __ballot(reg == r);
                if ((threadIdx.x & 63) == leader) atomicAdd(&hs[r], (unsigned int)__popcll(same));
                todo &= ~same;
            }
        }
    }
}
__global__ __launch_bounds__(1024) void imp_region_scan_kernel(unsigned int *__restrict__ hist, uint32_t nreg) {
    __shared__ unsigned int s_w[16];
    __shared__ unsigned int s_carry;
    unsigned int *h = hist + (size_t)blockIdx.x * (nreg + 1);
    const int t = threadIdx.x;
    if (t == 0) s_carry = 0;
    __syncthreads();
    for (uint32_t base = 0; base < nreg; base += 1024) {
        const unsigned int v = base + t < nreg ? h[base + t] : 0u;
        unsigned int inc = v;
        for (int o = 1; o < 64; o <<= 1) { const unsigned int u = __shfl_up(inc, o); if ((t & 63) >= o) inc += u; }
        if ((t & 63) == 63) s_w[t >> 6] = inc;
        __syncthreads();
        unsigned int wbase = s_carry;
        for (int w = 0; w < (t >> 6); ++w) wbase += s_w[w];
        if (base + t < nreg) h[base + t] = wbase + inc - v;
        __syncthreads();
        if (t == 1023) s_carry = wbase + inc;
        __syncthreads();
    }
    if (t == 0) h[nreg] = s_carry;
}
__global__ __launch_bounds__(256) void lds_import_kernel(MultiSrc S, TableDev T, uint32_t nreg, const unsigned int *__restrict__ bounds,
                                                         ulonglong2 *__restrict__ deferred, unsigned long long *__restrict__ deferred_n, unsigned long long deferred_cap) {
    __shared__ unsigned long long s_tag[IMPR];
    __shared__ unsigned long long s_cnt[IMPR];
    __shared__ unsigned int s_fresh[4];
    const uint32_t r = blockIdx.x;
    const int sh = packed_count_shift(T.B);
    const unsigned long long himask = sh ? ((1ull << sh) - 1ull) : 0ull;
    for (uint32_t j = threadIdx.x; j < IMPR; j += 256) { s_tag[j] = 0ull; s_cnt[j] = 0ull; }
    __syncthreads();
    unsigned int fresh = 0;
    for (uint32_t s = 0; s < S.n_src; ++s) {
        const ulonglong2 *__restrict__ in = S.p[s];
        const unsigned int *__restrict__ b = bounds + (size_t)s * (nreg + 1);
        const unsigned int lo = b[r], hi = b[r + 1];
        for (unsigned int i = lo + threadIdx.x; i < hi; i += 256) {
            const ulonglong2 e = in[i];
            const u128 h = mk(e.y & himask, e.x);
            const unsigned long long c = sh ? (e.y >> sh) : e.y;
            if (!c) continue;
            const uint64_t home = home_of(h, T.B, T.s);
            bool placed = false;
            if ((uint32_t)(home >> IMPR_LOG) == r) {
                const uint64_t rem = rem_of(h, T.B, T.s);
                const uint32_t local = (uint32_t)(home & (IMPR - 1));
                for (uint32_t off = 0; off < MAXPROBE && local + off < IMPR; ++off) {
                    const unsigned long long want = tag_of(rem, off);
                    unsigned long long cur = s_tag[local + off];
                    if (cur == 0ull) {
                        cur = atomicCAS(&s_tag[local + off], 0ull, want);
                        if (cur == 0ull) { ++fresh; cur = want; }
                    }
                    if (cur == want) { atomicAdd(&s_cnt[local + off], c); placed = true; break; }
                }
            }
            if (!placed) {
                const unsigned long long di = atomicAdd(deferred_n, 1ull);
                if (di < deferred_cap) deferred[di] = e;
            }
        }
    }
    __syncthreads();
    ulonglong2 *out = reinterpret_cast<ulonglong2 *>(T.slots) + (size_t)r * IMPR;
    for (uint32_t j = threadIdx.x; j < IMPR; j += 256) out[j] = make_ulonglong2(s_tag[j], s_cnt[j]);
    for (int o = 32; o > 0; o >>= 1) fresh += __shfl_xor(fresh, o);
    if ((threadIdx.x & 63) == 0) s_fresh[threadIdx.x >> 6] = fresh;
    __syncthreads();
    if (threadIdx.x == 0) {
        const unsigned int f = s_fresh[0] + s_fresh[1] + s_fresh[2] + s_fresh[3];
        if (f) atomicAdd(&T.stats[ST_DISTINCT], (unsigned long long)f);
    }
}

__global__ __launch_bounds__(256) void zero_kernel(ulonglong2 *__restrict__ p, uint64_t n16) {
    for (uint64_t i = blockIdx.x * (uint64_t)blockDim.x + threadIdx.x; i < n16; i += (uint64_t)gridDim.x * blockDim.x)
        p[i] = make_ulonglong2(0ull, 0ull);
}

__global__ __launch_bounds__(256) void rehash_kernel(TableDev oldT, TableDev newT) {
    unsigned long long fresh = 0;
    const uint64_t nslots = oldT.mask + 1;
    for (uint64_t i = blockIdx.x * (uint64_t)blockDim.x + threadIdx.x; i < nslots; i += (uint64_t)gridDim.x * blockDim.x) {
        const ulonglong2 e = *reinterpret_cast<const ulonglong2 *>(oldT.slots + 2 * i);
        if (e.x == 0ull) continue;
        fresh += table_add_or_spill(newT, slot_hash(oldT, i, e.x), e.y);
    }
    for (int o = 32; o > 0; o >>= 1) fresh += __shfl_xor(fresh, o);
    if ((threadIdx.x & 63) == 0 && fresh) atomicAdd(&newT.stats[ST_DISTINCT], fresh);
}

static size_t slot_alloc_bytes(uint64_t nslots) {
    size_t b = (size_t)nslots * 16;
    if ((b & (1ull << 31)) && !getenv("JASPER_NO_IPC_PAD")) b += 1ull << 31;
    return b;
}

static int grid_for(uint64_t work_items, int per_block) {
    uint64_t b = (work_items + per_block - 1) / per_block;
    const uint64_t cap = 256ull * 8;
    if (b > cap) b = cap;
    if (b < 1) b = 1;
    return (int)b;
}

int Table::min_log2_slots(int k) {
    int need = 2 * k - (63 - OFFBITS) - 64;
    return std::max(need, 10);
}

int Table::init(int k_, uint64_t min_slots, int device_, std::string &err) {
    if (k_ < 1 || k_ > 64) { err = "k must be in [1,64]"; return -1; }
    k = k_;
    device = device_;
    HIPCHK(hipSetDevice(device));
    if (const char *e = getenv("JASPER_EXPERIMENT_CU_MASK")) {
        uint32_t m[8];
        for (int w = 0; w < 8; ++w)
            m[w] = !strcmp(e, "alt2") ? 0x55555555u : !strcmp(e, "alt4x3") ? 0x77777777u : !strcmp(e, "lo128") ? (w < 4 ? ~0u : 0u) : !strcmp(e, "lo192") ? (w < 6 ? ~0u : 0u) : ~0u;
        HIPCHK(hipExtStreamCreateWithCUMask(&stream, 8, m));
    } else
    HIPCHK(hipStreamCreateWithFlags(&stream, hipStreamNonBlocking));
    int s = min_log2_slots(k);
    size_hint = min_slots;
    while ((1ull << s) < min_slots) ++s;
    if (s > 2 * k) s = 2 * k;
    if (s < min_log2_slots(k)) {
        err = "internal: slot count below tag-format minimum"; return -1;
    }
    nslots = 1ull << s;
    d = TableDev{};
    d.s = s; d.B = 2 * k; d.k = k; d.mask = nslots - 1;
    d.spill_cap = 1u << 16;
    HIPCHK(hipMalloc((void **)&d.slots, slot_alloc_bytes(nslots)));
    if (wide_rem(d.B, d.s)) HIPCHK(hipMalloc((void **)&d.ext, (size_t)nslots * 8));
    HIPCHK(hipMalloc((void **)&d.stats, ST_WORDS * sizeof(unsigned long long)));
    HIPCHK(hipMalloc((void **)&d.spill, d.spill_cap * 3 * sizeof(unsigned long long)));
    HIPCHK(hipMalloc((void **)&d_histo, 2 * HISTO_WORDS * sizeof(unsigned long long)));
    histo_cached = histo_request = false;
    slots_dirty = true;
    HIPCHK(hipMemsetAsync(d.stats, 0, ST_WORDS * sizeof(unsigned long long), stream));
    HIPCHK(hipHostMalloc((void **)&h_stats, ST_WORDS * sizeof(unsigned long long), hipHostMallocDefault));
    HIPCHK(hipEventCreate(&ev_k0));
    HIPCHK(hipEventCreate(&ev_k1));
    memset(h_stats, 0, ST_WORDS * sizeof(unsigned long long));
    HIPCHK(jk_stream_wait(stream));
    return 0;
}

std::atomic<int> g_cancel{0};

void Table::wait_streams() {
    if (stream) (void)jk_stream_wait(stream);
    for (hipStream_t ps : polish_stream) if (ps) (void)jk_stream_wait(ps);
    if (jf_stream) (void)jk_stream_wait(jf_stream);
    if (ingest_stream) (void)jk_stream_wait(ingest_stream);
    if (ingest_copy_stream) (void)jk_stream_wait(ingest_copy_stream);
    if (gz_stream) (void)jk_stream_wait(gz_stream);
}

void *Table::workspace(int id, size_t bytes, std::string &err) {
    if (bytes == 0) bytes = 256;
    WsBuf &b = ws[id];
    if (b.bytes >= bytes) return b.p;
    if (b.p) { wait_streams(); (void)hipFree(b.p); b.p = nullptr; b.bytes = 0; }
    const size_t want = bytes + std::min<size_t>(bytes / 8, (size_t)256 << 20);
    const char *dbg_e = getenv("JASPER_COUNT_DEBUG");
    const bool dbg = dbg_e != nullptr && (want >= (256u << 20) || atoi(dbg_e) >= 2);
    const auto t0 = std::chrono::steady_clock::now();
    hipError_t e = hipMalloc(&b.p, want);
    if (dbg) fprintf(stderr, "[workspace] slot %d: hipMalloc of %.3f GB took %.1f ms\n", id, (double)want / 1e9,
                     std::chrono::duration<double, std::milli>(std::chrono::steady_clock::now() - t0).count());
    if (e != hipSuccess) {
        e = hipMalloc(&b.p, bytes);
        if (e != hipSuccess) { err = std::string("device workspace allocation failed: ") + hipGetErrorString(e); b.p = nullptr; return nullptr; }
        b.bytes = bytes;
        return b.p;
    }
    b.bytes = want;
    if (const char *pz = getenv("JASPER_DEBUG_POISON")) {
        const char *only = getenv("JASPER_DEBUG_POISON_SLOT");
        if (!only || atoi(only) == id) { (void)hipMemset(b.p, atoi(pz) & 0xFF, want); (void)hipDeviceSynchronize(); }
    }
    return b.p;
}

void *Table::pinned(int id, size_t bytes, std::string &err) {
    if (bytes == 0) bytes = 256;
    WsBuf &b = pin[id];
    if (b.bytes >= bytes) return b.p;
    if (b.p) { wait_streams(); (void)hipHostFree(b.p); b.p = nullptr; b.bytes = 0; }
    const size_t want = bytes + bytes / 4;
    const char *dbg_e = getenv("JASPER_COUNT_DEBUG");
    const auto t0 = std::chrono::steady_clock::now();
    if (hipHostMalloc(&b.p, want, hipHostMallocDefault) != hipSuccess) { err = "pinned host buffer allocation failed"; b.p = nullptr; return nullptr; }
    if (dbg_e && atoi(dbg_e) >= 2) fprintf(stderr, "[pinned] slot %d: hipHostMalloc of %.1f MB took %.1f ms\n", id, (double)want / 1e6,
                                           std::chrono::duration<double, std::milli>(std::chrono::steady_clock::now() - t0).count());
    b.bytes = want;
    return b.p;
}

void Table::destroy() {
    feed_stop();
    (void)hipSetDevice(device);
    if (stream) (void)jk_stream_wait(stream);
    detach_shards();
    for (hipStream_t &ps : polish_stream) { if (ps) { (void)jk_stream_wait(ps); (void)hipStreamDestroy(ps); ps = nullptr; } }
    if (polish_ev) { (void)hipEventDestroy(polish_ev); polish_ev = nullptr; }
    if (jf_stream) { (void)jk_stream_wait(jf_stream); (void)hipStreamDestroy(jf_stream); jf_stream = nullptr; }
    if (ingest_stream) { (void)jk_stream_wait(ingest_stream); (void)hipStreamDestroy(ingest_stream); ingest_stream = nullptr; }
    if (ingest_copy_stream) { (void)jk_stream_wait(ingest_copy_stream); (void)hipStreamDestroy(ingest_copy_stream); ingest_copy_stream = nullptr; }
    for (hipEvent_t &e : ingest_copy_ev) { if (e) (void)hipEventDestroy(e); e = nullptr; }
    if (gz_stream) { (void)jk_stream_wait(gz_stream); (void)hipStreamDestroy(gz_stream); gz_stream = nullptr; }
    for (WsBuf &b : ws) { if (b.p) (void)hipFree(b.p); b.p = nullptr; b.bytes = 0; }
    for (WsBuf &b : pin) { if (b.p) (void)hipHostFree(b.p); b.p = nullptr; b.bytes = 0; }
    for (int i = 0; i < 2; ++i) {
        if (d_stage[i]) (void)hipFree(d_stage[i]);
        if (h_stage[i]) (void)hipHostFree(h_stage[i]);
        if (ev_stage[i]) (void)hipEventDestroy(ev_stage[i]);
    }
    release_retired();
    if (d.slots) (void)hipFree(d.slots);
    if (d.ext) (void)hipFree(d.ext);
    if (d.stats) (void)hipFree(d.stats);
    if (d.spill) (void)hipFree(d.spill);
    if (d_histo) (void)hipFree(d_histo);
    d_histo = nullptr;
    if (h_ingest) (void)hipHostFree(h_ingest);
    h_ingest = nullptr;
    if (h_stats) (void)hipHostFree(h_stats);
    if (ev_k0) (void)hipEventDestroy(ev_k0);
    if (ev_k1) (void)hipEventDestroy(ev_k1);
    if (stream) (void)hipStreamDestroy(stream);
    d = TableDev{};
    stream = nullptr;
}

int Table::zero_slots(unsigned long long *slots, uint64_t n, std::string &err) {
    hipLaunchKernelGGL(zero_kernel, dim3(256 * 16), dim3(256), 0, stream, reinterpret_cast<ulonglong2 *>(slots), n);
    HIPCHK(hipGetLastError());
    return 0;
}

__global__ void zero_stats_kernel(unsigned long long *stats) { if (threadIdx.x < ST_WORDS) stats[threadIdx.x] = 0ull; }

int Table::clear(std::string &err) {
    HIPCHK(hipSetDevice(device));
    slots_dirty = true;
    histo_cached = false;
    timespec a, b, c;
    const bool dbg = getenv("JASPER_COUNT_DEBUG") != nullptr;
    if (dbg) clock_gettime(CLOCK_MONOTONIC, &a);
    hipLaunchKernelGGL(zero_stats_kernel, dim3(1), dim3(64), 0, stream, d.stats);
    HIPCHK(hipGetLastError());
    if (dbg) {
        clock_gettime(CLOCK_MONOTONIC, &b);
        (void)jk_stream_wait(stream);
        clock_gettime(CLOCK_MONOTONIC, &c);
        fprintf(stderr, "[count] clear: launch %.3f ms, wait %.3f ms\n", (b.tv_sec - a.tv_sec) * 1e3 + (b.tv_nsec - a.tv_nsec) * 1e-6,
                (c.tv_sec - b.tv_sec) * 1e3 + (c.tv_nsec - b.tv_nsec) * 1e-6);
    }
    return 0;
}

int Table::read_stats(std::string &err) {
    HIPCHK(hipSetDevice(device));
    HIPCHK(hipMemcpyAsync(h_stats, d.stats, ST_WORDS * sizeof(unsigned long long), hipMemcpyDeviceToHost, stream));
    HIPCHK(jk_stream_wait(stream));
    return 0;
}

int Table::grow(int new_s, std::string &err) {
    if (new_s > d.B) new_s = d.B;
    if (new_s <= d.s) return 0;
    return resize(new_s, err);
}

int Table::fit(double max_load, std::string &err) {
    HIPCHK(hipSetDevice(device));
    if (materialize(err)) return -1;
    if (read_stats(err)) return -1;
    if (!(max_load > 0.05 && max_load <= 0.9)) { err = "fit: load must be in (0.05, 0.9]"; return -1; }
    int ns = min_log2_slots(k);
    if (!d.ext) ns = std::max(ns, std::min(d.s, d.B - (63 - OFFBITS)));
    while ((double)h_stats[ST_DISTINCT] > max_load * (double)(1ull << ns) && ns < d.B) ++ns;
    if (ns == d.s) return 0;
    histo_cached = false;
    if (resize(ns, err)) return -1;
    return after_batch(err);
}

int Table::resize(int new_s, std::string &err) {
    if (new_s == d.s) return 0;
    detach_shards();
    unsigned long long *new_ext = nullptr, *ns = nullptr;
    auto fail = [&](hipError_t e, const char *what) {
        err = std::string(what) + ": " + hipGetErrorString(e);
        if (new_ext) (void)hipFree(new_ext);
        if (ns) (void)hipFree(ns);
        return -1;
    };
    hipError_t e;
    if (wide_rem(d.B, new_s) && (e = hipMalloc((void **)&new_ext, (size_t)(1ull << new_s) * 8)) != hipSuccess) return fail(e, "resize: hipMalloc(ext)");
    if ((e = hipMalloc((void **)&ns, slot_alloc_bytes(1ull << new_s))) != hipSuccess) return fail(e, "resize: hipMalloc(slots)");
    auto drop_old = [&]() {
        if (exported) { retired.push_back(d.slots); exported = false; }
        else (void)hipFree(d.slots);
        if (d.ext) (void)hipFree(d.ext);
    };
    if (slots_dirty) {
        if ((e = jk_stream_wait(stream)) != hipSuccess) return fail(e, "resize: stream");
        drop_old();
        d.slots = ns; d.ext = new_ext; d.s = new_s; d.mask = (1ull << new_s) - 1; nslots = 1ull << new_s;
        return 0;
    }
    TableDev nt = d;
    nt.s = new_s;
    nt.mask = (1ull << new_s) - 1;
    nt.ext = new_ext;
    nt.slots = ns;
    if (zero_slots(nt.slots, 1ull << new_s, err)) { (void)fail(hipSuccess, "resize"); return -1; }
    if ((e = hipMemsetAsync(d.stats + ST_DISTINCT, 0, sizeof(unsigned long long), stream)) != hipSuccess) return fail(e, "resize: memset");
    hipLaunchKernelGGL(rehash_kernel, dim3(grid_for(nslots, 256)), dim3(256), 0, stream, d, nt);
    if ((e = hipGetLastError()) != hipSuccess) return fail(e, "resize: rehash launch");
    if ((e = jk_stream_wait(stream)) != hipSuccess) return fail(e, "resize: rehash");
    drop_old();
    d = nt;
    nslots = 1ull << new_s;
    return 0;
}

int Table::after_batch(std::string &err) {
    for (int round = 0; round < 8; ++round) {
        if (read_stats(err)) return -1;
        if (h_stats[ST_FATAL]) { err = "k-mer table overflow (spill buffer exhausted): pass a larger size hint"; return -2; }
        const uint64_t spilled = h_stats[ST_SPILL];
        if (getenv("JASPER_COUNT_DEBUG") && spilled) fprintf(stderr, "[count] after_batch: %llu spilled insertions\n", (unsigned long long)spilled);
        const bool too_full = (double)h_stats[ST_DISTINCT] > grow_at * (double)nslots && d.s < d.B;
        if (!spilled && !too_full) return 0;
        std::vector<unsigned long long> sp;
        if (spilled) {
            sp.resize(3 * spilled);
            HIPCHK(hipMemcpy(sp.data(), d.spill, sp.size() * sizeof(unsigned long long), hipMemcpyDeviceToHost));
            HIPCHK(hipMemsetAsync(d.stats + ST_SPILL, 0, sizeof(unsigned long long), stream));
        }
        int ns = d.s + 1;
        while ((double)h_stats[ST_DISTINCT] > 0.5 * grow_at * (double)(1ull << ns) && ns < d.B) ++ns;
        if (d.s >= d.B && spilled) { err = "k-mer table cannot grow further"; return -2; }
        if (grow(ns, err)) return -1;
        if (spilled) {
            unsigned long long *tmp = nullptr;
            HIPCHK(hipMalloc((void **)&tmp, sp.size() * sizeof(unsigned long long)));
            HIPCHK(hipMemcpy(tmp, sp.data(), sp.size() * sizeof(unsigned long long), hipMemcpyHostToDevice));
            hipLaunchKernelGGL(import_kernel, dim3(grid_for(spilled, 256)), dim3(256), 0, stream, tmp, spilled, d);
            HIPCHK(hipGetLastError());
            HIPCHK(jk_stream_wait(stream));
            HIPCHK(hipFree(tmp));
        }
    }
    err = "k-mer table did not settle after growth";
    return -2;
}

int Table::ensure_capacity(uint64_t upcoming_kmers, std::string &err) {
    if (read_stats(err)) return -1;
    int ns = d.s;
    while ((double)(h_stats[ST_DISTINCT] + upcoming_kmers) > 0.75 * (double)(1ull << ns) && ns < d.B) ++ns;
    if (ns != d.s) return grow(ns, err);
    return 0;
}

int Table::launch_count(const uint8_t *d_piece, uint64_t len, uint64_t emit_from, std::string &err) {
    alignas(16) char geom[64];
    if (!part_off && len >= (slots_dirty ? nslots / 6 : nslots / 4)) {
        if (partition_geometry(len, geom)) {
            ++count_partitioned_launches;
            return launch_count_partitioned(d_piece, len, emit_from, geom, err);
        }
    }
    histo_request = false;
    count_path = 0;
    if (materialize(err)) return -1;
    const uint64_t ntiles = (len + CT_TILE - 1) / CT_TILE;
    HIPCHK(hipEventRecord(ev_k0, stream));
    static const int mode = getenv("JASPER_EXPERIMENT_MODE") ? atoi(getenv("JASPER_EXPERIMENT_MODE")) : 0;
    if (mode == 1) hipLaunchKernelGGL(count_kernel<1>, dim3(grid_for(ntiles, 1)), dim3(CT_THREADS), 0, stream, d_piece, len, ntiles, emit_from, d);
    else if (mode == 2) hipLaunchKernelGGL(count_kernel<2>, dim3(grid_for(ntiles, 1)), dim3(CT_THREADS), 0, stream, d_piece, len, ntiles, emit_from, d);
    else hipLaunchKernelGGL(count_kernel<0>, dim3(grid_for(ntiles, 1)), dim3(CT_THREADS), 0, stream, d_piece, len, ntiles, emit_from, d);
    HIPCHK(hipGetLastError());
    HIPCHK(hipEventRecord(ev_k1, stream));
    return 0;
}

int Table::count_device(const uint8_t *d_bases, uint64_t n, std::string &err, uint64_t first_new) {
    HIPCHK(hipSetDevice(device));
    if (read_stats(err)) return -1;
    histo_cached = false;
    const uint64_t halo = (uint64_t)(k - 1);
    const uint64_t misalign = reinterpret_cast<uintptr_t>(d_bases) & 15;
    uint64_t pos = std::min(first_new, n);
    bool have_ratio = false;
    if (size_hint > 0 && n > (1u << 24) && h_stats[ST_DISTINCT] == 0 && h_stats[ST_OCCURRENCES] == 0) {
        dup_ratio = std::min(1.0, (double)size_hint / (double)n);
        have_ratio = dup_ratio < 0.6;
    }
    const bool started_empty = h_stats[ST_DISTINCT] == 0 && h_stats[ST_OCCURRENCES] == 0;
    size_t mem_have = 0;
    {
        size_t free_b = 0, total_b = 0;
        if (hipMemGetInfo(&free_b, &total_b) == hipSuccess) {
            mem_have = free_b;
            for (int w = WS_COUNT; w < WS_COUNT + 4; ++w) mem_have += ws[w].bytes;
        }
    }
    const bool dbg = getenv("JASPER_COUNT_DEBUG") != nullptr;
    auto now_ms = []() { timespec ts; clock_gettime(CLOCK_MONOTONIC, &ts); return ts.tv_sec * 1e3 + ts.tv_nsec * 1e-6; };
    const double t_call = now_ms();
    if (dbg) fprintf(stderr, "[count] call start: %llu bases\n", (unsigned long long)n);
    while (pos < n) {
        const uint64_t room = (uint64_t)(0.75 * (double)nslots) > h_stats[ST_DISTINCT] ? (uint64_t)(0.75 * (double)nslots) - h_stats[ST_DISTINCT] : 0;
        uint64_t piece = std::max<uint64_t>(room, 1u << 20);
        if ((pos > 0 || have_ratio) && dup_ratio < 0.6) piece = std::max<uint64_t>(piece, (uint64_t)((double)room / std::max(0.05, 1.5 * dup_ratio)));
        if (mem_have) piece = std::min<uint64_t>(piece, std::max<uint64_t>(mem_have / 28, 1u << 20));
        piece = std::min<uint64_t>(piece, 1ull << 33);
        if ((pos > 0 || have_ratio) && dup_ratio < 0.6 && n - pos <= piece + piece / 4 && n - pos <= (1ull << 33)) piece = n - pos;
        if (have_ratio && pos == 0 && (double)n * dup_ratio <= (double)room && n <= (1ull << 33) && (!mem_have || n <= mem_have / 28)) piece = n;
        if (const char *e = getenv("JASPER_EXPERIMENT_PIECE")) piece = strtoull(e, nullptr, 10);
        {
            const uint64_t todo = std::min<uint64_t>(piece, n - pos);
            const uint64_t expect = (pos > 0 || have_ratio) && dup_ratio < 0.6 ? (uint64_t)((double)todo * std::min(1.0, dup_ratio)) : todo;
            if (expect > room && !getenv("JASPER_EXPERIMENT_PIECE")) {
                if (ensure_capacity(expect, err)) return -1;
            }
        }
        uint64_t start = pos >= halo ? pos - halo : 0;
        const uint64_t a = (start + misalign) & 15;
        start = start >= a ? start - a : 0;
        const uint64_t end = std::min<uint64_t>(n, pos + piece);
        const uint64_t distinct_before = h_stats[ST_DISTINCT], occ_before = h_stats[ST_OCCURRENCES];
        const double t_l0 = dbg ? now_ms() : 0;
        if (dbg) fprintf(stderr, "[count] host: %.2f ms since call start (sizing, capacity)\n", t_l0 - t_call);
        histo_request = started_empty && pos == 0 && first_new == 0 && end == n && h_stats[ST_DISTINCT] == 0;
        histo_cached = false;
        const int lrc = launch_count(d_bases + start, end - start, pos - start, err);
        const bool fused_histo = histo_request;
        histo_request = false;
        if (lrc) return -1;
        const double t_l1 = dbg ? now_ms() : 0;
        const uint64_t pos_piece = pos;
        pos = end;
        int rc = after_batch(err);
        histo_cached = rc == 0 && fused_histo;
        if (rc == -2 && count_path == 1 && part_defer_header) {
            unsigned long long abandoned = 0;
            HIPCHK(hipMemcpy(&abandoned, part_defer_header + 1, 8, hipMemcpyDeviceToHost));
            if (abandoned) {
                if (dbg) {
                    float m1 = 0, m2 = 0;
                    (void)hipEventElapsedTime(&m1, ev_stage_t[0], ev_stage_t[1]);
                    (void)hipEventElapsedTime(&m2, ev_stage_t[1], ev_stage_t[2]);
                    fprintf(stderr, "[count] partitioned piece abandoned (lists overflowed the deferred list; its partition passes took %.2f + %.2f ms): direct kernel from here on\n", m1, m2);
                }
                err.clear();
                part_off = true;
                part_stage_pending = false;
                slots_dirty = part_slots_dirty_before;
                const unsigned long long zero = 0, occ = occ_before;
                HIPCHK(hipMemcpy(d.stats + ST_FATAL, &zero, 8, hipMemcpyHostToDevice));
                HIPCHK(hipMemcpy(d.stats + ST_OCCURRENCES, &occ, 8, hipMemcpyHostToDevice));
                if (read_stats(err)) return -1;
                pos = pos_piece;
                continue;
            }
        }
        if (dbg) fprintf(stderr, "[count] host: launch calls %.2f ms, wait + after_batch %.2f ms\n", t_l1 - t_l0, now_ms() - t_l1);
        if (rc == -2 && have_ratio && started_empty) {
            if (dbg) fprintf(stderr, "[count] size hint too small for this input: restarting with worst-case sizing\n");
            err.clear();
            if (clear(err)) return -1;
            if (read_stats(err)) return -1;
            if (grow(std::min(d.B, d.s + 2), err)) return -1;
            have_ratio = false;
            dup_ratio = 1.0;
            pos = std::min(first_new, n);
            continue;
        }
        if (rc) return rc;
        if (h_stats[ST_OCCURRENCES] > occ_before)
            dup_ratio = (double)(h_stats[ST_DISTINCT] - distinct_before) / (double)(h_stats[ST_OCCURRENCES] - occ_before);
        if (part_stage_pending) {
            for (int i = 0; i < part_stage_n; ++i) { float m = 0; if (hipEventElapsedTime(&m, ev_stage_t[i], ev_stage_t[i + 1]) == hipSuccess) part_stage_ms[i] += m; }
            part_stage_pending = false;
        }
        if (getenv("JASPER_COUNT_DEBUG"))
            fprintf(stderr, "[count] piece done: pos %llu / %llu, distinct %llu, slots 2^%d, dup_ratio %.3f, stage ms so far %.2f %.2f %.2f %.2f %.2f\n",
                    (unsigned long long)pos, (unsigned long long)n, (unsigned long long)h_stats[ST_DISTINCT], d.s, dup_ratio,
                    part_stage_ms[0], part_stage_ms[1], part_stage_ms[2], part_stage_ms[3], part_stage_ms[4]);
        float ms = 0;
        HIPCHK(hipEventElapsedTime(&ms, ev_k0, ev_k1));
        count_kernel_ms += ms;
        count_launches += 1;
    }
    return 0;
}

int Table::count_host(const char *bases, uint64_t n, std::string &err) {
    HIPCHK(hipSetDevice(device));
    if (read_stats(err)) return -1;
    histo_cached = histo_request = false;
// ... 427 lines not shown
```

jasper_amd/csrc/table.hpp:

```cpp
#pragma once
#include "kmer.hpp"
#include <atomic>
#include <functional>
#include <string>
#include <vector>

namespace jk {

extern std::atomic<int> g_cancel;


constexpr uint32_t MAX_SHARDS = 8;
struct TableDev {
    unsigned long long *slots;
    uint64_t mask;
    int s;
    int B;
    int k;
    unsigned long long *stats;
    unsigned long long *spill;
    uint64_t spill_cap;
    const unsigned long long *shard[MAX_SHARDS];
    uint32_t nshard;
    unsigned long long *ext;
};

__device__ __forceinline__ u128 slot_hash(const TableDev &T, uint64_t i, unsigned long long tag) {
    const uint32_t off = (uint32_t)(tag & (MAXPROBE - 1));
    const uint64_t rem = (tag & ~OCC) >> OFFBITS;
    const uint64_t home = (i - off) & T.mask;
    if (T.ext) return hash_from_wide(home, rem, T.ext[i], T.B, T.s);
    return hash_from(home, rem, T.B, T.s);
}
__device__ __forceinline__ int table_put_wide(const TableDev &T, u128 h, unsigned long long val, bool assign) {
    const uint64_t home = home_of(h, T.B, T.s);
    const uint64_t rem = tag_rem_of(h, T.B, T.s);
    const unsigned long long ext = ext_of(h, T.B, T.s);
    int result = -1;
    uint32_t off = 0, waited = 0;
    for (;;) {
        if (result < 0) {
            const uint64_t slot = (home + off) & T.mask;
            const unsigned long long want = tag_of(rem, off);
            unsigned long long *p = T.slots + 2 * slot;
            unsigned long long cur = __hip_atomic_load(p, __ATOMIC_RELAXED, __HIP_MEMORY_SCOPE_AGENT);
            if (cur == 0ull) {
                cur = atomicCAS(p, 0ull, want);
                if (cur == 0ull) {
                    __hip_atomic_store(T.ext + slot, ext, __ATOMIC_RELAXED, __HIP_MEMORY_SCOPE_AGENT);
                    __hip_atomic_store(p + 1, val, __ATOMIC_RELEASE, __HIP_MEMORY_SCOPE_AGENT);
                    result = 2;
                }
            }
            if (result < 0) {
                bool next = true;
                if (cur == want) {
                    const unsigned long long c = __hip_atomic_load(p + 1, __ATOMIC_ACQUIRE, __HIP_MEMORY_SCOPE_AGENT);
                    if (c == 0ull) {
                        next = false;
                        if (++waited > (1u << 16)) result = 0;
                    } else if (__hip_atomic_load(T.ext + slot, __ATOMIC_RELAXED, __HIP_MEMORY_SCOPE_AGENT) == ext) {
                        if (assign) __hip_atomic_store(p + 1, val, __ATOMIC_RELAXED, __HIP_MEMORY_SCOPE_AGENT);
                        else __hip_atomic_fetch_add(p + 1, val, __ATOMIC_RELAXED, __HIP_MEMORY_SCOPE_AGENT);
                        result = 1;
                    }
                }
                if (result < 0 && next && ++off >= MAXPROBE) result = 0;
            }
        }
        if (__ballot(result < 0) == 0ull) break;
    }
    return result;
}

JK_HD uint32_t owner_of(u128 h, uint32_t n) {
    uint32_t x = (uint32_t)h.lo ^ (uint32_t)(h.lo >> 32) ^ (uint32_t)h.hi;
    x *= 0x9E3779B1u; x ^= x >> 15; x *= 0x85EBCA77u; x ^= x >> 13;
    return (uint32_t)(((uint64_t)x * n) >> 32);
}
__device__ __forceinline__ const unsigned long long *read_slots(const TableDev &T, u128 h) {
    if (T.nshard <= 1) return T.slots;
    const uint32_t o = owner_of(h, T.nshard);
    const unsigned long long *b = T.shard[0];
#pragma unroll
    for (uint32_t i = 1; i < MAX_SHARDS; ++i) b = (o == i) ? T.shard[i] : b;
    return b;
}

enum { ST_DISTINCT = 0, ST_SPILL = 1, ST_OCCURRENCES = 2, ST_FATAL = 3, ST_WORDS = 8 };

__device__ __forceinline__ int table_add(const TableDev &T, u128 h, unsigned long long inc) {
    if (T.ext) return table_put_wide(T, h, inc, false);
    const uint64_t home = home_of(h, T.B, T.s);
    const uint64_t rem = rem_of(h, T.B, T.s);
    for (uint32_t off = 0; off < MAXPROBE; ++off) {
        const uint64_t slot = (home + off) & T.mask;
        const unsigned long long want = tag_of(rem, off);
        unsigned long long *p = T.slots + 2 * slot;
        unsigned long long cur = __hip_atomic_load(p, __ATOMIC_RELAXED, __HIP_MEMORY_SCOPE_AGENT);
        int fresh = 1;
        if (cur == 0ull) {
            cur = atomicCAS(p, 0ull, want);
            if (cur == 0ull) {
                fresh = 2;
                cur = want;
            }
        }
        if (cur == want) {
            __hip_atomic_fetch_add(p + 1, inc, __ATOMIC_RELAXED, __HIP_MEMORY_SCOPE_AGENT);
            return fresh;
        }
    }
    return 0;
}

__device__ __forceinline__ int table_add_prefetched(const TableDev &T, u128 h, unsigned long long inc, unsigned long long cur0) {
    if (T.ext) return table_add(T, h, inc);
    const uint64_t home = home_of(h, T.B, T.s);
    const uint64_t rem = rem_of(h, T.B, T.s);
    for (uint32_t off = 0; off < MAXPROBE; ++off) {
        const uint64_t slot = (home + off) & T.mask;
        const unsigned long long want = tag_of(rem, off);
        unsigned long long *p = T.slots + 2 * slot;
        unsigned long long cur = off == 0 ? cur0 : __hip_atomic_load(p, __ATOMIC_RELAXED, __HIP_MEMORY_SCOPE_AGENT);
        int fresh = 1;
        if (cur == 0ull) {
            cur = atomicCAS(p, 0ull, want);
            if (cur == 0ull) { fresh = 2; cur = want; }
        }
        if (cur == want) {
            __hip_atomic_fetch_add(p + 1, inc, __ATOMIC_RELAXED, __HIP_MEMORY_SCOPE_AGENT);
            return fresh;
        }
    }
    return 0;
}
__device__ __forceinline__ void table_spill(const TableDev &T, u128 h, unsigned long long inc) {
    unsigned long long idx = atomicAdd(&T.stats[ST_SPILL], 1ull);
    if (idx < T.spill_cap) {
        T.spill[3 * idx + 0] = h.hi;
        T.spill[3 * idx + 1] = h.lo;
        T.spill[3 * idx + 2] = inc;
    } else {
        atomicExch(&T.stats[ST_FATAL], 1ull);
    }
}

__device__ __forceinline__ unsigned table_add_or_spill(const TableDev &T, u128 h, unsigned long long inc) {
    const int r = table_add(T, h, inc);
    if (r == 2) return 1u;
    if (r == 0) {
        unsigned long long idx = atomicAdd(&T.stats[ST_SPILL], 1ull);
        if (idx < T.spill_cap) {
            T.spill[3 * idx + 0] = h.hi;
            T.spill[3 * idx + 1] = h.lo;
            T.spill[3 * idx + 2] = inc;
        } else {
            atomicExch(&T.stats[ST_FATAL], 1ull);
        }
    }
    return 0u;
}

__device__ __forceinline__ unsigned long long table_get(const TableDev &T, u128 h) {
    const uint64_t home = home_of(h, T.B, T.s);
    const uint64_t rem = tag_rem_of(h, T.B, T.s);
    const unsigned long long *S = read_slots(T, h);
    const bool wide = T.ext != nullptr;
    const unsigned long long ext = wide ? ext_of(h, T.B, T.s) : 0ull;
    for (uint32_t off = 0; off < MAXPROBE; ++off) {
        const uint64_t slot = (home + off) & T.mask;
        const ulonglong2 e = *reinterpret_cast<const ulonglong2 *>(S + 2 * slot);
        if (e.x == tag_of(rem, off) && (!wide || T.ext[slot] == ext)) return e.y;
        if (e.x == 0ull) return 0ull;
    }
    return 0ull;
}

__device__ __forceinline__ unsigned long long table_get_prefetched(const TableDev &T, u128 h, ulonglong2 e0) {
    if (T.ext) return table_get(T, h);
    const uint64_t home = home_of(h, T.B, T.s);
    const uint64_t rem = rem_of(h, T.B, T.s);
    if (e0.x == tag_of(rem, 0)) return e0.y;
    if (e0.x == 0ull) return 0ull;
    const unsigned long long *S = read_slots(T, h);
    for (uint32_t off = 1; off < MAXPROBE; ++off) {
        const uint64_t slot = (home + off) & T.mask;
        const ulonglong2 e = *reinterpret_cast<const ulonglong2 *>(S + 2 * slot);
        if (e.x == tag_of(rem, off)) return e.y;
        if (e.x == 0ull) return 0ull;
    }
    return 0ull;
}

__device__ __forceinline__ uint32_t clamp32(unsigned long long c) { return c > 0xFFFFFFFFull ? 0xFFFFFFFFu : (uint32_t)c; }

__device__ __forceinline__ void encode16(const uint32_t w[4], uint32_t &codes, uint32_t &inv) {
    codes = 0;
    inv = 0;
#pragma unroll
    for (int i = 0; i < 4; ++i) {
        const uint32_t x0 = (w[i] >> 1) & 0x03030303u;
        const uint32_t x = x0 ^ ((x0 >> 1) & 0x01010101u);
        const uint32_t expect = __builtin_amdgcn_perm(0u, 0x54474341u, x);
        const uint32_t d = expect ^ (w[i] & 0xDFDFDFDFu);
        const uint32_t nz = (((d & 0x7F7F7F7Fu) + 0x7F7F7F7Fu) | d) & 0x80808080u;
        codes = (codes << 8) | ((x * 0x40100401u) >> 24);
        inv = (inv << 4) | ((((nz >> 7) * 0x08040201u) >> 24) & 0xFu);
    }
}
struct Raw16 { uint32_t w[4]; };
__device__ __forceinline__ Raw16 load16(const uint8_t *__restrict__ text, int64_t pos, int64_t n) {
    struct __attribute__((packed, aligned(1))) V16 { uint32_t w[4]; };
    Raw16 r;
    if (pos >= 0 && pos + 16 <= n) {
        const V16 v = *reinterpret_cast<const V16 *>(text + pos);
        r.w[0] = v.w[0]; r.w[1] = v.w[1]; r.w[2] = v.w[2]; r.w[3] = v.w[3];
    } else {
        r.w[0] = r.w[1] = r.w[2] = r.w[3] = 0x4E4E4E4Eu;
#pragma unroll
        for (int j = 0; j < 16; ++j) {
            const int64_t p = pos + j;
            if (p >= 0 && p < n) r.w[j >> 2] = (r.w[j >> 2] & ~(0xFFu << (8 * (j & 3)))) | ((uint32_t)text[p] << (8 * (j & 3)));
        }
    }
    return r;
}
__device__ __forceinline__ void stage16(const uint8_t *__restrict__ text, int64_t pos, int64_t n, uint32_t &codes, uint32_t &inv) {
    const Raw16 r = load16(text, pos, n);
    encode16(r.w, codes, inv);
}

template <typename Get>
__device__ __forceinline__ u128 encode_padded(int k, long n, Get get) {
    u128 m = mk(0, 0);
    int t = 0;
    const int lim = n < k ? (int)n : k;
    for (; t < lim; ++t) {
        int c = code(get(t));
        if (c < 0) break;
        m = bor(shl(m, 2), mk(0, (uint64_t)c));
    }
    if (t < k) m = shl(m, 2 * (k - t));
    return m;
}

struct Table {
    int device = 0;
    int k = 0;
    hipStream_t stream = nullptr;
    TableDev d{};
    uint64_t nslots = 0;
    uint8_t *d_stage[2] = {nullptr, nullptr};
    uint8_t *h_stage[2] = {nullptr, nullptr};
    hipEvent_t ev_stage[2] = {nullptr, nullptr};
    size_t stage_bytes = 0;
    unsigned long long *h_stats = nullptr;
    double grow_at = 0.5;
    hipEvent_t ev_k0 = nullptr, ev_k1 = nullptr;
    double count_kernel_ms = 0;
    uint64_t count_launches = 0;
    void reset_timing() { count_kernel_ms = 0; count_launches = 0; count_partitioned_launches = 0; for (double &m : part_stage_ms) m = 0; }
    int launch_count(const uint8_t *d_piece, uint64_t len, uint64_t emit_from, std::string &err);
    bool partition_geometry(uint64_t piece_bases, void *geom_out) const;
    int launch_count_partitioned(const uint8_t *d_piece, uint64_t len, uint64_t emit_from, const void *geom, std::string &err);
    uint64_t count_partitioned_launches = 0;
    static constexpr int N_STAGES = 8;
    hipEvent_t ev_stage_t[N_STAGES + 1] = {};
    double part_stage_ms[N_STAGES] = {};
    int part_stage_n = 5;
    int count_path = 0;
    bool part_stage_pending = false;
    unsigned long long *part_defer_header = nullptr;
    bool part_slots_dirty_before = false, part_off = false;
    bool xchg_partitioned = false;
    bool xchg_deduped = false;
    static constexpr int HISTO_WORDS = 10002 + 6;
    unsigned long long *d_histo = nullptr;
    bool histo_cached = false, histo_request = false;
    double dup_ratio = 1.0;
    uint64_t size_hint = 0;
    struct WsBuf { void *p = nullptr; size_t bytes = 0; };
    static constexpr int POLISH_LANES_MAX = 4;
    static constexpr int WS_POLISH_MAX = 40, WS_COUNT = 40, WS_INGEST = 44, WS_XCHG = 51, WS_HOSTBASES = 55, WS_LANE0 = 56,
                         WS_GZ = WS_LANE0 + (POLISH_LANES_MAX - 1) * WS_POLISH_MAX,
                         WS_SLOTS = WS_GZ + 5;
    WsBuf ws[WS_SLOTS];
    hipStream_t polish_stream[POLISH_LANES_MAX] = {nullptr, nullptr, nullptr, nullptr};
    hipEvent_t polish_ev = nullptr;
    uint64_t polish_calls = 0;
    hipStream_t jf_stream = nullptr;
    hipStream_t ingest_stream = nullptr;
    hipStream_t ingest_copy_stream = nullptr;
    hipEvent_t ingest_copy_ev[2] = {nullptr, nullptr};
    void *workspace(int id, size_t bytes, std::string &err);
    void wait_streams();
    static constexpr int PIN_PER_LANE = 8, PIN_SLOTS = PIN_PER_LANE * POLISH_LANES_MAX;
    WsBuf pin[PIN_SLOTS];
    void *pinned(int id, size_t bytes, std::string &err);

    static int min_log2_slots(int k);
    int init(int k, uint64_t min_slots, int device, std::string &err);
    void destroy();
    int read_stats(std::string &err);
    int zero_slots(unsigned long long *slots, uint64_t n, std::string &err);
    bool slots_dirty = false;
    int materialize(std::string &err) { if (!slots_dirty) return 0; slots_dirty = false; return zero_slots(d.slots, nslots, err); }
    int clear(std::string &err);
    int ensure_capacity(uint64_t upcoming_kmers, std::string &err);
    int grow(int new_s, std::string &err);
    int resize(int new_s, std::string &err);
    int ensure_narrow(std::string &err);
    int fit(double max_load, std::string &err);
    int after_batch(std::string &err);
    int count_device(const uint8_t *d_bases, uint64_t n, std::string &err, uint64_t first_new = 0);
    int count_host(const char *bases, uint64_t n, std::string &err);
    int count_files_gpu(const char *const *paths, int n_paths, uint64_t *gpu_bytes, uint64_t *host_bytes, std::string &err);
    uint64_t ingest_gpu_bytes = 0, ingest_host_bytes = 0;
    uint64_t inflate_stats[6] = {};
    hipStream_t gz_stream = nullptr;
    const int64_t *ingest_begin = nullptr, *ingest_end = nullptr;
    std::function<int(const uint8_t *d_bases, uint64_t n)> bases_sink;
    struct Feed;
    Feed *feed = nullptr;
    int feed_start(const char *const *paths, const int64_t *begins, const int64_t *ends, int n_paths, std::string &err);
    int feed_next(const void **d_bases, uint64_t *n, std::string &err);
    int feed_release(std::string &err);
    void feed_stop();
    char *h_ingest = nullptr;
    size_t ingest_chunk = 0;
    int histogram(uint64_t *out10002, std::string &err);
    int histogram_part(uint32_t part, uint32_t nparts, uint64_t *out10002, std::string &err);
    void part_span(uint32_t part, uint32_t nparts, uint64_t &first, uint64_t &span) const;
    int lookup_strings(const char *chars, const int64_t *offsets, uint64_t n, uint32_t *out, std::string &err);
    int export_entries(uint64_t *n_out, unsigned long long **d_entries_out, std::string &err);
    int import_entries(const unsigned long long *d_entries, uint64_t n, std::string &err);
    int export_packed(void *d_dst, uint64_t cap, uint64_t *n_out, uint32_t part, uint32_t nparts, std::string &err);
    int import_packed(const void *d_src, uint64_t n, int mode, std::string &err);
    int import_packed_multi(const void *const *d_srcs, const uint64_t *counts, uint32_t n_src, std::string &err);
    int reserve(uint64_t min_slots, std::string &err);
    int export_owner(void *d_dst, uint64_t cap, uint32_t nown, int sort_r, uint64_t *counts_out, std::string &err);
    int xchg_plan(uint64_t piece_max, uint64_t records_max, uint32_t nown, uint64_t out[8], std::string &err);
    int xchg_scan(const uint8_t *d_bases, uint64_t n, uint64_t pos, uint64_t end, uint64_t piece_max, uint32_t nown, void *d_defer, uint64_t defer_cap, uint64_t *records,
                  std::string &err);
    int xchg_partition(uint64_t piece_max, uint64_t records_max, uint32_t nown, void *d_send, void *d_send_cnt, void *d_defer, uint64_t defer_cap, std::string &err);
    int xchg_dedupe(uint64_t piece_max, uint64_t records_max, uint32_t nown, void *d_send, void *d_send_cnt, uint32_t *max_fill, int *cbits_out, std::string &err);
    int xchg_insert(const void *d_recv, const void *d_recv_cnt, uint64_t piece_max, uint64_t records_max, uint32_t nown, uint32_t self, const void *d_defer_all,
                    uint64_t n_defer_all, int whole_input, uint32_t slice_cap, int cbits, std::string &err);
    int ipc_handle(void *out64, std::string &err);
    int attach_ipc(const void *handles64, uint32_t n, uint32_t self, std::string &err);
    int attach_tables(Table *const *peers, uint32_t n, uint32_t self, std::string &err);
    void detach_shards();
    bool exported = false;
    std::vector<void *> retired;
    void release_retired();
    void *ipc_mapped[MAX_SHARDS] = {};
    int write_jf(const char *path, const char *const *cmdline, int n_cmd, std::string &err, int r_bits = -1, int what = 0);
    int load_jf_records(const char *path, uint64_t data_offset, uint64_t n_records, int key_len_bits, int counter_len, std::string &err);
};

}
```

Before: 3056.

## Cut polish launch and host overhead with fused kernels, device seg expansion, and a worker pool

Several changes aim to reduce per-call overhead in the polish pipeline. Segment descriptors are now expanded into SegDev on device inside seg_init, which also resets arrival flags and the ticket, removing a memset and host-side setup. An in-place mode skips the text copy. find_sync and find_clean are fused into one launch, and summary plus offsets become a single-block kernel when there are few chunks. On the host, lane threads are reused through a persistent worker pool, and a k-way merge of per-lane record runs replaces the full stable sort. The cost is more complex code, and correctness of ordering now depends on the ticket reset moving into earlier kernels.

```diff
diff --git a/jasper_amd/csrc/polish.hip b/jasper_amd/csrc/polish.hip
--- a/jasper_amd/csrc/polish.hip
+++ b/jasper_amd/csrc/polish.hip
@@ -1027,11 +1027,31 @@
 
 constexpr int SC_THREADS = 256, SC_GROUP = 16, SC_TILE = SC_THREADS * SC_GROUP, SC_HALO = 4;
 
-__global__ __launch_bounds__(256) void seg_init_kernel(SegDev *segs, int n_segs, const uint8_t *const *chunk_text) {
+__global__ __launch_bounds__(256) void seg_init_kernel(SegDev *segs, const SegDesc *descs, int n_segs, const ScanChunk *__restrict__ chunks, SegArena A,
+                                                       unsigned int *ticket) {
     struct __attribute__((packed, aligned(1))) V16 { uint32_t w[4]; };
+    const bool writer = blockIdx.x == 0 && threadIdx.x == 0;
+    if (writer && blockIdx.y == 0) *ticket = 0u;
     for (int s = blockIdx.y; s < n_segs; s += gridDim.y) {
-        const SegDev S = segs[s];
-        const uint8_t *src = chunk_text[S.chunk] + S.seg_lo;
+        SegDev S;
+        const uint8_t *text;
+        if (descs) {
+            const SegDesc D = descs[s];
+            const ScanChunk C = chunks[D.chunk];
+            seg_expand(S, D, (size_t)s, C.len, C.cls, C.text, A);
+            text = C.text;
+            if (writer) segs[s] = S;
+        } else {
+            S = segs[s];
+            text = chunks[S.chunk].text;
+        }
+        if (writer) {
+            A.arrive[s + 1] = ARRIVE_PENDING;
+            if (s == 0) A.arrive[0] = ARRIVE_PENDING;
+            if (s == n_segs - 1) A.arrive[n_segs + 1] = ARRIVE_PENDING;
+        }
+        if (A.in_place) continue;
+        const uint8_t *src = text + S.seg_lo;
         uint8_t *dst = S.buf + S.glen;
         const int64_t nblk = (S.len0 + 15) >> 4;
         for (int64_t blk = blockIdx.x * (int64_t)blockDim.x + threadIdx.x; blk < nblk; blk += (int64_t)gridDim.x * blockDim.x) {
@@ -1124,11 +1144,9 @@
     for (int o = 1; o < 64; o <<= 1) { const long long u = __shfl_up(v, o); if (lane >= o) v += u; }
     return v;
 }
-__global__ __launch_bounds__(64) void seg_summary_kernel(SegDev *segs, const int32_t *first_seg, int n_chunks, int64_t *idx_base, uint32_t *seq_base,
-                                                         uint32_t *rec_off, uint32_t *aux_off, ChunkSummary *out) {
-    const int c = blockIdx.x;
-    if (c >= n_chunks) return;
-    const int lane = threadIdx.x;
+__device__ __forceinline__ ChunkSummary summarize_chunk(SegDev *segs, const int32_t *first_seg, int c, int64_t *idx_base, uint32_t *seq_base,
+                                                        uint32_t *rec_off, uint32_t *aux_off) {
+    const int lane = threadIdx.x & 63;
     const int s0 = first_seg[c], s1 = first_seg[c + 1];
     long long newlen = 0, shift = 0, seqc = 0, recc = 0, auxc = 0, wrong = 0, lookups = 0;
     int bad = -1, spec = 0;
@@ -1165,11 +1183,17 @@
         bad = bad < 0 ? b2 : (b2 < 0 ? bad : (b2 < bad ? b2 : bad));
         spec |= __shfl_xor(spec, o);
     }
-    if (lane == 0) {
-        ChunkSummary R;
-        R.newlen = newlen; R.wrong = wrong; R.lookups = (uint64_t)lookups; R.nrec = (uint32_t)recc; R.naux = (uint32_t)auxc; R.bad_seg = bad; R.spec_fail = spec;
-        out[c] = R;
-    }
+    ChunkSummary R;
+    R.newlen = newlen; R.wrong = wrong; R.lookups = (uint64_t)lookups; R.nrec = (uint32_t)recc; R.naux = (uint32_t)auxc; R.bad_seg = bad; R.spec_fail = spec;
+    return R;
+}
+__global__ __launch_bounds__(64) void seg_summary_kernel(SegDev *segs, const int32_t *first_seg, int n_chunks, int64_t *idx_base, uint32_t *seq_base,
+                                                         uint32_t *rec_off, uint32_t *aux_off, ChunkSummary *out, unsigned int *zero_word) {
+    const int c = blockIdx.x;
+    if (c >= n_chunks) return;
+    if (zero_word && c == 0 && threadIdx.x == 0) *zero_word = 0u;
+    const ChunkSummary R = summarize_chunk(segs, first_seg, c, idx_base, seq_base, rec_off, aux_off);
+    if (threadIdx.x == 0) out[c] = R;
 }
 __global__ __launch_bounds__(64) void seg_offsets_kernel(const int32_t *first_seg, int n_chunks, uint32_t *rec_off, uint32_t *aux_off, const ChunkSummary *sum) {
     const int c = blockIdx.x;
@@ -1179,6 +1203,26 @@
     for (int q = lane; q < c; q += 64) { rb += sum[q].nrec; ab += sum[q].naux; }
     for (int o = 32; o > 0; o >>= 1) { rb += __shfl_xor(rb, o); ab += __shfl_xor(ab, o); }
     for (int s = first_seg[c] + lane; s < first_seg[c + 1]; s += 64) { rec_off[s] += (uint32_t)rb; aux_off[s] += (uint32_t)ab; }
+}
+
+constexpr int SUMMARY_FUSED_MAX = 64, SUMMARY_FUSED_WAVES = 16;
+__global__ __launch_bounds__(64 * SUMMARY_FUSED_WAVES) void seg_summary_offsets_kernel(SegDev *segs, const int32_t *first_seg, int n_chunks, int64_t *idx_base,
+                                                                                       uint32_t *seq_base, uint32_t *rec_off, uint32_t *aux_off,
+                                                                                       ChunkSummary *out, unsigned int *zero_word) {
+    __shared__ uint32_t s_nrec[SUMMARY_FUSED_MAX], s_naux[SUMMARY_FUSED_MAX];
+    const int wave = threadIdx.x >> 6, lane = threadIdx.x & 63;
+    if (zero_word && threadIdx.x == 0) *zero_word = 0u;
+    for (int c = wave; c < n_chunks; c += SUMMARY_FUSED_WAVES) {
+        const ChunkSummary R = summarize_chunk(segs, first_seg, c, idx_base, seq_base, rec_off, aux_off);
+        if (lane == 0) { out[c] = R; s_nrec[c] = R.nrec; s_naux[c] = R.naux; }
+    }
+    __syncthreads();
+    for (int c = wave; c < n_chunks; c += SUMMARY_FUSED_WAVES) {
+        if (c == 0) continue;
+        uint32_t rb = 0, ab = 0;
+        for (int q = 0; q < c; ++q) { rb += s_nrec[q]; ab += s_naux[q]; }
+        for (int s = first_seg[c] + lane; s < first_seg[c + 1]; s += 64) { rec_off[s] += rb; aux_off[s] += ab; }
+    }
 }
 
 constexpr int SC_BACK = 64;
@@ -1277,7 +1321,7 @@
     }
 }
 
-__global__ __launch_bounds__(256) void find_sync_batch_kernel(const ScanChunk *__restrict__ chunks, int n_chunks, int k) {
+__device__ __forceinline__ void find_sync_blocks(const ScanChunk *__restrict__ chunks, int n_chunks, int k, int bx, int nbx) {
     struct __attribute__((packed, aligned(1))) V16 { uint32_t w[4]; };
     const int64_t W = 4ll * k;
     for (int ci = blockIdx.y; ci < n_chunks; ci += gridDim.y) {
@@ -1287,7 +1331,7 @@
         const uint8_t *__restrict__ cls = C.cls;
         static_assert(PC_CLEAN == 0 && PC_BAD == 1 && PC_OTHER == 2, "the block test below looks at bit 0 of the class bytes");
         const int64_t nblk = (nwin + 15) >> 4;
-        for (int64_t blk = blockIdx.x * (int64_t)blockDim.x + threadIdx.x; blk < nblk; blk += (int64_t)gridDim.x * blockDim.x) {
+        for (int64_t blk = bx * (int64_t)blockDim.x + threadIdx.x; blk < nblk; blk += (int64_t)nbx * blockDim.x) {
             const int64_t p0 = blk << 4;
             uint32_t w[4];
             if (p0 + 16 <= nwin) {
@@ -1399,12 +1443,12 @@
     }
 }
 
-__global__ __launch_bounds__(64) void find_clean_batch_kernel(const ScanChunk *__restrict__ chunks, int n_chunks, int k) {
-    const int lane = threadIdx.x;
+__device__ __forceinline__ void find_clean_waves(const ScanChunk *__restrict__ chunks, int n_chunks, int k, uint32_t wx, uint32_t nwx) {
+    const int lane = threadIdx.x & 63;
     for (int ci = blockIdx.y; ci < n_chunks; ci += gridDim.y) {
         const ScanChunk C = chunks[ci];
         const int64_t nwin = C.len - k + 1;
-        for (uint32_t g = blockIdx.x; g < C.n_cells; g += gridDim.x) {
+        for (uint32_t g = wx; g < C.n_cells; g += nwx) {
             int64_t p0 = (int64_t)g * CLEAN_CELL + CLEAN_CELL / 2;
             const int64_t cell_end = (int64_t)(g + 1) * CLEAN_CELL;
             int64_t cand = -1;
@@ -1425,10 +1469,13 @@
     }
 }
 
-static void launch_find_clean(const ScanChunk *d_chunks, int n_chunks, int k, hipStream_t stream) {
-    const int gy = n_chunks < 1024 ? n_chunks : 1024;
-    const int gx = std::max(1, 8192 / gy);
-    hipLaunchKernelGGL(find_clean_batch_kernel, dim3(gx, gy), dim3(64), 0, stream, d_chunks, n_chunks, k);
+__global__ __launch_bounds__(256) void find_sync_clean_batch_kernel(const ScanChunk *__restrict__ chunks, int n_chunks, int k, int sync_bx) {
+    if ((int)blockIdx.x < sync_bx) find_sync_blocks(chunks, n_chunks, k, (int)blockIdx.x, sync_bx);
+    else find_clean_waves(chunks, n_chunks, k, (blockIdx.x - sync_bx) * 4u + (threadIdx.x >> 6), (gridDim.x - sync_bx) * 4u);
+}
+static void launch_find_sync_clean(const ScanChunk *d_chunks, int n_chunks, int k, int sync_bx, int gy, hipStream_t stream) {
+    const int clean_bx = std::max(1, 2048 / gy);
+    hipLaunchKernelGGL(find_sync_clean_batch_kernel, dim3(sync_bx + clean_bx, gy), dim3(256), 0, stream, d_chunks, n_chunks, k, sync_bx);
 }
 
 void launch_rescan_batch(const TableDev &T, const ScanChunk *d_chunks, int n_chunks, int k, uint32_t solid, hipStream_t stream) {
@@ -1436,8 +1483,7 @@
     const int gy = n_chunks < 1024 ? n_chunks : 1024;
     const int gx = std::max(1, 4096 / gy);
     hipLaunchKernelGGL(rescan_batch_kernel, dim3(gx, gy), dim3(256), 0, stream, d_chunks, n_chunks, T, solid);
-    hipLaunchKernelGGL(find_sync_batch_kernel, dim3(gx, gy), dim3(256), 0, stream, d_chunks, n_chunks, k);
-    launch_find_clean(d_chunks, n_chunks, k, stream);
+    launch_find_sync_clean(d_chunks, n_chunks, k, gx, gy, stream);
 }
 
 void launch_scan_batch(const TableDev &T, const ScanChunk *d_chunks, int n_chunks, int k, uint32_t solid, hipStream_t stream) {
@@ -1445,8 +1491,7 @@
     const int gy = n_chunks < 1024 ? n_chunks : 1024;
     const int gx = std::max(1, 4096 / gy);
     hipLaunchKernelGGL(scan_classify_batch_kernel, dim3(gx, gy), dim3(SC_THREADS), 0, stream, d_chunks, n_chunks, T, solid);
-    hipLaunchKernelGGL(find_sync_batch_kernel, dim3(gx, gy), dim3(256), 0, stream, d_chunks, n_chunks, k);
-    launch_find_clean(d_chunks, n_chunks, k, stream);
+    launch_find_sync_clean(d_chunks, n_chunks, k, gx, gy, stream);
 }
 
 __global__ __launch_bounds__(256) void copy_chunks_kernel(uint8_t *const *__restrict__ chunk_ptr, uint8_t *__restrict__ pack, const int64_t *__restrict__ offs, int n,
@@ -1464,21 +1509,26 @@
     hipLaunchKernelGGL(copy_chunks_kernel, dim3((unsigned)std::min(n, 256 * 16)), dim3(256), 0, stream, d_chunk_ptr, d_pack, d_offs, n, to_chunks ? 1 : 0);
 }
 
-void launch_seg_init(SegDev *d_segs, int n_segs, const uint8_t *const *d_chunk_text, hipStream_t stream) {
+void launch_seg_init(SegDev *d_segs, const SegDesc *d_descs, int n_segs, const ScanChunk *d_chunks, const SegArena &arena, unsigned int *d_ticket,
+                     hipStream_t stream) {
     if (n_segs <= 0) return;
-    dim3 grid(n_segs >= 512 ? 4 : 64, n_segs < 4096 ? n_segs : 4096);
-    hipLaunchKernelGGL(seg_init_kernel, grid, dim3(256), 0, stream, d_segs, n_segs, d_chunk_text);
+    dim3 grid(arena.in_place ? 1 : n_segs >= 512 ? 4 : 64, n_segs < 4096 ? n_segs : 4096);
+    hipLaunchKernelGGL(seg_init_kernel, grid, dim3(256), 0, stream, d_segs, d_descs, n_segs, d_chunks, arena, d_ticket);
 }
 void launch_seg_walk(const TableDev &T, SegDev *d_segs, int n_segs, PolishParams pp, int pass, ScratchPool pool, unsigned int *d_ticket,
                      hipStream_t stream) {
     if (n_segs <= 0) return;
-    (void)hipMemsetAsync(d_ticket, 0, sizeof(unsigned int), stream);
     hipLaunchKernelGGL(seg_walk_kernel, dim3(n_segs), dim3(64), 0, stream, T, d_segs, n_segs, pp, pass, pool, d_ticket);
 }
 void launch_seg_summary(SegDev *d_segs, int n_segs, const int32_t *d_first_seg, int n_chunks, int64_t *idx_base, uint32_t *seq_base, uint32_t *rec_off,
-                        uint32_t *aux_off, ChunkSummary *d_out, hipStream_t stream) {
+                        uint32_t *aux_off, ChunkSummary *d_out, unsigned int *d_zero_word, hipStream_t stream) {
     if (n_segs <= 0 || n_chunks <= 0) return;
-    hipLaunchKernelGGL(seg_summary_kernel, dim3(n_chunks), dim3(64), 0, stream, d_segs, d_first_seg, n_chunks, idx_base, seq_base, rec_off, aux_off, d_out);
+    if (n_chunks <= SUMMARY_FUSED_MAX) {
+        hipLaunchKernelGGL(seg_summary_offsets_kernel, dim3(1), dim3(64 * SUMMARY_FUSED_WAVES), 0, stream, d_segs, d_first_seg, n_chunks, idx_base, seq_base, rec_off,
+                           aux_off, d_out, d_zero_word);
+        return;
+    }
+    hipLaunchKernelGGL(seg_summary_kernel, dim3(n_chunks), dim3(64), 0, stream, d_segs, d_first_seg, n_chunks, idx_base, seq_base, rec_off, aux_off, d_out, d_zero_word);
     hipLaunchKernelGGL(seg_offsets_kernel, dim3(n_chunks), dim3(64), 0, stream, d_first_seg, n_chunks, rec_off, aux_off, d_out);
 }
 void launch_seg_gather(const SegDev *d_segs, int n_segs, const int64_t *idx_base, const uint32_t *seq_base, const uint32_t *rec_off,
diff --git a/jasper_amd/csrc/polish.hpp b/jasper_amd/csrc/polish.hpp
--- a/jasper_amd/csrc/polish.hpp
+++ b/jasper_amd/csrc/polish.hpp
@@ -1,21 +1,8 @@
 #pragma once
 #include "table.hpp"
+#include "polish_seg.hpp"
 
 namespace jk {
-
-struct FixRec {
-    int64_t index;
-    uint32_t chunk;
-    uint32_t seqno;
-    uint8_t pass;
-    uint8_t kind;
-    uint8_t newc;
-    uint8_t oldc;
-    uint32_t rep;
-    uint32_t aux_off;
-    uint32_t aux_len;
-};
-static_assert(sizeof(FixRec) == 32, "FixRec layout");
 
 enum PolishStatus {
     PS_OK = 0,
@@ -42,44 +29,6 @@
     uint32_t front_cap;
     uint32_t patch_cap;
     size_t off_front, off_patch;
-};
-
-struct EditRec {
-    int64_t a;
-    int32_t plen, oldlen;
-};
-
-struct SegDev {
-    uint8_t *buf;
-    int64_t cap;
-    int64_t len;
-    int64_t gs, glen;
-    int64_t len0;
-    int64_t seg_lo;
-    int64_t start_i;
-    int64_t stop_orig;
-    int32_t first, last;
-    int32_t chain_in;
-    int32_t took_shortcut;
-    long long *arrive;
-    const uint8_t *cls;
-    int64_t cls_n;
-    FixRec *recs;
-    uint32_t rec_cap, nrec;
-    uint8_t *aux;
-    uint32_t aux_cap, naux;
-    EditRec *edits;
-    uint32_t edit_cap, nedit;
-    uint32_t chunk;
-    int32_t status;
-    int32_t spec_fail;
-    int64_t wrong;
-    uint64_t lookups;
-    uint64_t ticks;
-    uint64_t tk[12];
-    int64_t own_lo, own_hi;
-    int64_t own_hi0;
-    int64_t out_off;
 };
 
 struct ChunkSummary {
@@ -120,13 +69,14 @@
 void launch_rescan_batch(const TableDev &T, const ScanChunk *d_chunks, int n_chunks, int k, uint32_t solid, hipStream_t stream);
 
 void launch_copy_chunks(uint8_t *const *d_chunk_ptr, uint8_t *d_pack, const int64_t *d_offs, int n, bool to_chunks, hipStream_t stream);
-void launch_seg_init(SegDev *d_segs, int n_segs, const uint8_t *const *d_chunk_text, hipStream_t stream);
+void launch_seg_init(SegDev *d_segs, const SegDesc *d_descs, int n_segs, const ScanChunk *d_chunks, const SegArena &arena, unsigned int *d_ticket,
+                     hipStream_t stream);
 void launch_seg_walk(const TableDev &T, SegDev *d_segs, int n_segs, PolishParams pp, int pass, ScratchPool pool, unsigned int *d_ticket,
                      hipStream_t stream);
 void launch_seg_stitch(const SegDev *d_segs, int n_segs, uint8_t *const *d_chunk_out, uint8_t *const *d_cls_out, uint8_t *const *d_flags,
                        hipStream_t stream);
 void launch_seg_summary(SegDev *d_segs, int n_segs, const int32_t *d_first_seg, int n_chunks, int64_t *idx_base, uint32_t *seq_base, uint32_t *rec_off,
-                        uint32_t *aux_off, ChunkSummary *d_out, hipStream_t stream);
+                        uint32_t *aux_off, ChunkSummary *d_out, unsigned int *d_zero_word, hipStream_t stream);
 void launch_seg_gather(const SegDev *d_segs, int n_segs, const int64_t *idx_base, const uint32_t *seq_base, const uint32_t *rec_off,
                        const uint32_t *aux_off, FixRec *out_recs, uint8_t *out_aux, hipStream_t stream);
 
diff --git a/jasper_amd/csrc/polish_host.hip b/jasper_amd/csrc/polish_host.hip
--- a/jasper_amd/csrc/polish_host.hip
+++ b/jasper_amd/csrc/polish_host.hip
@@ -4,6 +4,9 @@
 #include <cstdio>
 #include <cstdlib>
 #include <cstring>
+#include <condition_variable>
+#include <functional>
+#include <mutex>
 #include <thread>
 
 namespace jk {
@@ -26,6 +29,25 @@
     ~DevBuf() { if (p && owned) (void)hipFree(p); }
     template <typename T> T *as() { return reinterpret_cast<T *>(p); }
 };
+}
+
+static inline bool rec_before(const FixRec &a, const FixRec &b) {
+    if (a.chunk != b.chunk) return a.chunk < b.chunk;
+    if (a.pass != b.pass) return a.pass < b.pass;
+    return a.seqno < b.seqno;
+}
+static void merge_record_runs(std::vector<FixRec> &recs, const std::vector<size_t> &run_begin, int n_chunks) {
+    const size_t nr = run_begin.size();
+    if (nr <= 1 || recs.empty()) { if (!std::is_sorted(recs.begin(), recs.end(), rec_before)) std::stable_sort(recs.begin(), recs.end(), rec_before); return; }
+    std::vector<size_t> cur(run_begin), end(nr);
+    for (size_t r = 0; r < nr; ++r) end[r] = r + 1 < nr ? run_begin[r + 1] : recs.size();
+    std::vector<FixRec> out;
+    out.reserve(recs.size());
+    for (int c = 0; c < n_chunks && out.size() < recs.size(); ++c)
+        for (size_t r = 0; r < nr; ++r)
+            while (cur[r] < end[r] && recs[cur[r]].chunk == (uint32_t)c) out.push_back(recs[cur[r]++]);
+    if (out.size() == recs.size() && std::is_sorted(out.begin(), out.end(), rec_before)) recs.swap(out);
+    else std::stable_sort(recs.begin(), recs.end(), rec_before);
 }
 
 static int run_polish_lane(Table &T, const int lane, hipStream_t st, int n_chunks, const char *const *seqs, const int64_t *lens, int solid_thre, int passes, int fix,
@@ -78,7 +100,7 @@
         seg_rec_bound += (size_t)(RM * (2 * tb / k + 16 * ms));
         seg_aux_bound += (size_t)(RM * (2 * tb + 1024 * ms));
     }
-    DevBuf b_textA, b_textB, b_pack, b_cls, b_clsB, b_flags, b_segedit, b_cells, b_arrive, b_ptrA, b_segs, b_segtext, b_segrec, b_segaux, b_pool, b_locks, b_scan, b_ticket;
+    DevBuf b_textA, b_textB, b_pack, b_cls, b_clsB, b_flags, b_segedit, b_cells, b_arrive, b_ptrA, b_segs, b_desc, b_segtext, b_segrec, b_segaux, b_pool, b_locks, b_scan, b_ticket;
     int ws_next = 0;
     auto dmalloc = [&](DevBuf &b, size_t bytes) -> bool {
         if (ws_next >= Table::WS_POLISH_MAX) { err = "polish: workspace slots exhausted"; return false; }
@@ -91,7 +113,7 @@
         !dmalloc(b_segedit, seg_rec_bound * sizeof(EditRec)) || !dmalloc(b_cells, (2 + cell_items + cand_items) * 8) ||
         !dmalloc(b_arrive, ((size_t)max_segs + 4) * 8) ||
         !dmalloc(b_ptrA, (size_t)6 * n_chunks * sizeof(void *)) ||
-        !dmalloc(b_segs, (size_t)max_segs * sizeof(SegDev)) || !dmalloc(b_segtext, seg_text_bound) ||
+        !dmalloc(b_segs, (size_t)max_segs * sizeof(SegDev)) || !dmalloc(b_desc, (size_t)max_segs * sizeof(SegDesc)) || !dmalloc(b_segtext, seg_text_bound) ||
         !dmalloc(b_segrec, seg_rec_bound * sizeof(FixRec)) || !dmalloc(b_segaux, seg_aux_bound))
         return -2;
     ScratchPool pool;
@@ -110,14 +132,18 @@
     if (!dmalloc(b_first, ((size_t)n_chunks + 1) * 4) || !dmalloc(b_sum, (size_t)n_chunks * sizeof(ChunkSummary)) || !dmalloc(b_idx, (size_t)max_segs * 8) ||
         !dmalloc(b_seq, (size_t)max_segs * 4) || !dmalloc(b_ro, (size_t)max_segs * 4) || !dmalloc(b_ao, (size_t)max_segs * 4)) return -2;
     const size_t PIN_RECS = 1u << 18, PIN_AUX = 8u << 20;
-    SegDev *segs_p = reinterpret_cast<SegDev *>(T.pinned(pin_base + 0, (size_t)max_segs * sizeof(SegDev), err));
+    const char *su = getenv("JASPER_POLISH_SEG_UPLOAD");
+    const bool full_upload = su && !strcmp(su, "full");
+    SegDev *segs_p = full_upload ? reinterpret_cast<SegDev *>(T.pinned(pin_base + 0, (size_t)max_segs * sizeof(SegDev), err)) : nullptr;
+    SegDesc *desc_p = full_upload ? nullptr : reinterpret_cast<SegDesc *>(T.pinned(pin_base + 0, (size_t)max_segs * sizeof(SegDesc), err));
+    std::vector<SegDesc> descs_h;
     int32_t *first_p = reinterpret_cast<int32_t *>(T.pinned(pin_base + 1, ((size_t)n_chunks + 1) * 4, err));
     ChunkSummary *sum_p = reinterpret_cast<ChunkSummary *>(T.pinned(pin_base + 2, (size_t)n_chunks * sizeof(ChunkSummary), err));
     int64_t *cand_p = reinterpret_cast<int64_t *>(T.pinned(pin_base + 3, (std::min<size_t>(cand_items, 32768) + cell_items + 8) * 8, err));
     FixRec *recs_p = reinterpret_cast<FixRec *>(T.pinned(pin_base + 4, PIN_RECS * sizeof(FixRec), err));
     uint8_t *aux_p = reinterpret_cast<uint8_t *>(T.pinned(pin_base + 5, PIN_AUX, err));
     ScanChunk *sc_p = reinterpret_cast<ScanChunk *>(T.pinned(pin_base + 6, sizeof(ScanChunk) * (size_t)n_chunks, err));
-    if (!segs_p || !first_p || !sum_p || !cand_p || !recs_p || !aux_p || !sc_p) return -2;
+    if ((!segs_p && !desc_p) || !first_p || !sum_p || !cand_p || !recs_p || !aux_p || !sc_p) return -2;
     int64_t total_len = 0;
     for (int c = 0; c < n_chunks; ++c) total_len += len[c];
     const bool packed_io = !device_in && n_chunks > 256 && total_len / n_chunks < 65536 && !getenv("JASPER_POLISH_NO_PACKED_IO");
@@ -183,7 +209,7 @@
     std::vector<SegDev> segs;
     std::vector<ScanChunk> sc(n_chunks);
     int64_t *const d_count = b_cells.as<int64_t>(), *const d_cells = d_count + 2, *const d_cands = d_cells + cell_items;
-    std::vector<int64_t> all_cands(cand_items);
+    std::vector<int64_t> all_cands;
     std::vector<int64_t> all_cells(cell_items);
     std::vector<std::vector<int64_t>> chunk_cands(n_chunks);
     std::vector<int64_t> cands;
@@ -191,9 +217,25 @@
     std::vector<std::vector<uint8_t>> aux_pass;
     std::vector<size_t> rec_pass_begin;
     int rc = 0;
+    bool count_cleared = false;
+    SegArena arena;
+    arena.k = k;
+    arena.tight = tight ? 1 : 0;
+    arena.RM = RM;
+    arena.in_place = 0;
+    arena.text = b_segtext.as<uint8_t>();
+    arena.recs = b_segrec.as<FixRec>();
+    arena.edits = b_segedit.as<EditRec>();
+    arena.aux = b_segaux.as<uint8_t>();
+    arena.arrive = b_arrive.as<long long>();
 
     for (int pass = 0; pass <= passes && rc == 0; ++pass) {
-        HIPCHK(hipMemsetAsync(d_count, 0, 4, st));
+        const bool qv_in_place = pass == passes && !getenv("JASPER_POLISH_QV_COPY");
+        const bool reads_caller_text = device_in && pass == 0;
+        const bool carry = pass < passes;
+
+        if (!count_cleared) HIPCHK(hipMemsetAsync(d_count, 0, 4, st));
+        count_cleared = false;
         {
             for (int c = 0; c < n_chunks; ++c) {
                 ScanChunk &S = sc[c];
@@ -220,8 +262,9 @@
             HIPCHK(hipMemcpyAsync(cand_p, d_count, (2 + cell_items + CAND_PRE) * 8, hipMemcpyDeviceToHost, st));
             HIPCHK(jk_stream_wait(st));
             n_cand = *reinterpret_cast<const unsigned int *>(cand_p);
+            if (all_cands.size() < std::min<size_t>(n_cand, cand_items)) all_cands.resize(std::min<size_t>(n_cand, cand_items));
             if (cell_items) memcpy(all_cells.data(), cand_p + 2, cell_items * 8);
-            if (CAND_PRE) memcpy(all_cands.data(), cand_p + 2 + cell_items, std::min<size_t>(n_cand, CAND_PRE) * 8);
+            if (CAND_PRE && n_cand) memcpy(all_cands.data(), cand_p + 2 + cell_items, std::min<size_t>(n_cand, CAND_PRE) * 8);
         }
         n_cand = (unsigned int)std::min<size_t>(n_cand, cand_items);
         if (n_cand > CAND_PRE) {
@@ -235,7 +278,8 @@
             if (c >= 0 && c < n_chunks) chunk_cands[c].push_back(v & ((1ll << 40) - 1));
         }
 
-        auto build_segments = [&](const std::vector<int> &chunks, bool speculate, SegDev *out, size_t &n_out, int32_t *first_of, std::string &e2) -> int {
+        auto build_segments = [&](const std::vector<int> &chunks, bool speculate, const SegArena &A, SegDesc *out, size_t &n_out, int32_t *first_of,
+                                  std::string &e2) -> int {
             n_out = 0;
             size_t tpos = 0, rpos = 0, apos = 0, ci = 0;
             for (int c : chunks) {
@@ -268,34 +312,18 @@
                 const int m = (int)sync.size();
                 if ((int64_t)n_out + m + 1 > max_segs) { e2 = "polish: internal segment arena bound exceeded"; return -2; }
                 for (int j = 0; j <= m; ++j) {
-                    SegDev &S = out[n_out++];
-                    memset(&S, 0, sizeof S);
-                    S.chunk = (uint32_t)c;
-                    S.first = (j == 0);
-                    S.last = (j == m);
-                    S.seg_lo = j == 0 ? 0 : sync[j - 1] - W;
-                    S.start_i = j == 0 ? 0 : W;
-                    S.chain_in = j > 0 && chained[j - 1];
-                    S.arrive = b_arrive.as<long long>() + n_out;
-                    S.stop_orig = j == m ? INT64_MAX : sync[j];
-                    const int64_t seg_hi = j == m ? len[c] : std::min<int64_t>(len[c], sync[j] + M);
-                    S.len0 = seg_hi - S.seg_lo;
-                    S.len = S.len0;
-                    S.cap = S.len0 + (tight ? 2 : RM * std::max<int64_t>(1024, S.len0 / 8));
-                    S.gs = 0;
-                    S.glen = S.cap - S.len0;
-                    S.cls = (len[c] - k + 1 > 0) ? clsIn + off_pos[c] : nullptr;
-                    S.cls_n = std::max<int64_t>(0, len[c] - k + 1);
-                    S.rec_cap = (uint32_t)std::min<int64_t>(0x7fffffff, RM * (2 * S.len0 / k + 16));
-                    S.aux_cap = (uint32_t)std::min<int64_t>(0x7fffffff, RM * (2 * S.len0 + 1024));
-                    S.buf = b_segtext.as<uint8_t>() + tpos;            tpos += al256((size_t)S.cap);
-                    S.recs = b_segrec.as<FixRec>() + rpos;
-                    S.edits = b_segedit.as<EditRec>() + rpos;
-                    S.edit_cap = S.rec_cap;                            rpos += S.rec_cap;
-                    S.aux = b_segaux.as<uint8_t>() + apos;             apos += al256(S.aux_cap);
-                    S.own_lo = j == 0 ? 0 : 2ll * k;
-                    S.own_hi = j == m ? -1 : (sync[j] - 2ll * k) - S.seg_lo;
-                    S.own_hi0 = S.own_hi;
+                    SegDesc &D = out[n_out++];
+                    D.chunk = (uint32_t)c;
+                    D.flags = (j == 0 ? SD_FIRST : 0u) | (j == m ? SD_LAST : 0u) | (j > 0 && chained[j - 1] ? SD_CHAIN : 0u);
+                    D.cut_lo = j == 0 ? 0 : sync[j - 1];
+                    D.cut_hi = j == m ? 0 : sync[j];
+                    D.tpos = tpos;
+                    D.rpos = rpos;
+                    D.apos = apos;
+                    const SegGeom G = seg_geometry(D, len[c], A);
+                    if (!A.in_place) tpos += al256((size_t)G.cap);
+                    rpos += G.rec_cap;
+                    apos += al256(G.aux_cap);
                 }
             }
             if (first_of) first_of[ci] = (int32_t)n_out;
@@ -304,28 +332,36 @@
             }
             return 0;
         };
-        auto run_segments = [&](SegDev *sv, size_t nsv, bool summary, std::string &e2) -> int {
+        auto expand_segments = [&](const SegDesc *dv, size_t n, const SegArena &A, SegDev *out) {
+            for (size_t i = 0; i < n; ++i) {
+                memset(&out[i], 0, sizeof(SegDev));
+                seg_expand(out[i], dv[i], i, sc[dv[i].chunk].len, sc[dv[i].chunk].cls, sc[dv[i].chunk].text, A);
+            }
+        };
+        auto run_segments = [&](const SegDesc *dv, SegDev *sv, size_t nsv, const SegArena &A, bool summary, std::string &e2) -> int {
             if (!nsv) return 0;
             const bool fine = dbg && getenv("JASPER_POLISH_DEBUG") && atoi(getenv("JASPER_POLISH_DEBUG")) >= 2;
             double tf[5] = {fine ? now() : 0, 0, 0, 0, 0};
-            if (hipMemcpyAsync(b_segs.p, sv, nsv * sizeof(SegDev), hipMemcpyHostToDevice, st) != hipSuccess) { e2 = "polish: H2D segs"; return -1; }
+            if (dv) {
+                if (hipMemcpyAsync(b_desc.p, dv, nsv * sizeof(SegDesc), hipMemcpyHostToDevice, st) != hipSuccess) { e2 = "polish: H2D segment descriptors"; return -1; }
+            } else if (hipMemcpyAsync(b_segs.p, sv, nsv * sizeof(SegDev), hipMemcpyHostToDevice, st) != hipSuccess) { e2 = "polish: H2D segs"; return -1; }
             if (summary && hipMemcpyAsync(b_first.p, first_p, ((size_t)n_chunks + 1) * 4, hipMemcpyHostToDevice, st) != hipSuccess) { e2 = "polish: H2D first"; return -1; }
             if (fine) { (void)jk_stream_wait(st); tf[1] = now(); }
-            launch_seg_init(b_segs.as<SegDev>(), (int)nsv, (const uint8_t *const *)dIn, st);
-            if (hipMemsetAsync(b_arrive.p, 0x80, (nsv + 2) * 8, st) != hipSuccess) { e2 = "polish: memset"; return -1; }
+            launch_seg_init(b_segs.as<SegDev>(), dv ? b_desc.as<SegDesc>() : nullptr, (int)nsv, b_scan.as<ScanChunk>(), A, b_ticket.as<unsigned int>(), st);
             if (fine) { (void)jk_stream_wait(st); tf[2] = now(); }
             launch_seg_walk(T.d, b_segs.as<SegDev>(), (int)nsv, pp, pass, pool, b_ticket.as<unsigned int>(), st);
             if (hipGetLastError() != hipSuccess) { e2 = "polish: kernel launch failed"; return -1; }
             if (fine) { (void)jk_stream_wait(st); tf[3] = now(); }
             if (summary) {
                 launch_seg_summary(b_segs.as<SegDev>(), (int)nsv, b_first.as<int32_t>(), n_chunks, b_idx.as<int64_t>(), b_seq.as<uint32_t>(), b_ro.as<uint32_t>(),
-                                   b_ao.as<uint32_t>(), b_sum.as<ChunkSummary>(), st);
+                                   b_ao.as<uint32_t>(), b_sum.as<ChunkSummary>(), reinterpret_cast<unsigned int *>(d_count), st);
+                count_cleared = true;
                 if (hipMemcpyAsync(sum_p, b_sum.p, (size_t)n_chunks * sizeof(ChunkSummary), hipMemcpyDeviceToHost, st) != hipSuccess) { e2 = "polish: D2H summary"; return -1; }
             } else if (hipMemcpyAsync(sv, b_segs.p, nsv * sizeof(SegDev), hipMemcpyDeviceToHost, st) != hipSuccess) { e2 = "polish: D2H segs"; return -1; }
             if (jk_stream_wait(st) != hipSuccess) { e2 = "polish: kernel execution failed"; return -1; }
             if (fine) {
                 tf[4] = now();
-                fprintf(stderr, "[polish]     %zu segments x %zu B: H2D %.3f ms, init + memset %.3f ms, walk %.3f ms, %s %.3f ms\n", nsv, sizeof(SegDev), tf[1] - tf[0], tf[2] - tf[1],
+                fprintf(stderr, "[polish]     %zu segments x %zu B: H2D %.3f ms, init %.3f ms, walk %.3f ms, %s %.3f ms\n", nsv, dv ? sizeof(SegDesc) : sizeof(SegDev), tf[1] - tf[0], tf[2] - tf[1],
                         tf[3] - tf[2], summary ? "summary + D2H" : "D2H", tf[4] - tf[3]);
             }
             return 0;
@@ -334,9 +370,15 @@
         for (int c = 0; c < n_chunks; ++c) all[c] = c;
         const double tb0 = dbg ? now() : 0;
         size_t ns = 0;
-        if ((rc = build_segments(all, true, segs_p, ns, first_p, err))) break;
+        SegArena pass_arena = arena, redo_arena = arena;
+        pass_arena.in_place = qv_in_place ? 1 : 0;
+        if (full_upload) {
+            descs_h.resize((size_t)max_segs);
+            if ((rc = build_segments(all, true, pass_arena, descs_h.data(), ns, first_p, err))) break;
+            expand_segments(descs_h.data(), ns, pass_arena, segs_p);
+        } else if ((rc = build_segments(all, true, pass_arena, desc_p, ns, first_p, err))) break;
         const double tb1 = dbg ? now() : 0;
-        if ((rc = run_segments(segs_p, ns, true, err))) break;
+        if ((rc = run_segments(full_upload ? nullptr : desc_p, segs_p, ns, pass_arena, true, err))) break;
         if (dbg) fprintf(stderr, "[polish]   host: build %zu segments %.3f ms, upload + walk + summary %.3f ms\n", ns, tb1 - tb0, now() - tb1);
 
         bool ordinary = !getenv("JASPER_POLISH_DEBUG") && !getenv("JASPER_POLISH_HOST_BOOKKEEPING");
@@ -375,10 +417,12 @@
             for (const SegDev &S : segs) if (!failed[S.chunk]) good.push_back(S);
             size_t tpos = 0, rpos = 0, apos = 0;
             for (const SegDev &S : segs) { tpos += al256((size_t)S.cap); rpos += S.rec_cap; apos += al256(S.aux_cap); }
-            std::vector<SegDev> redo_segs((size_t)max_segs);
+            std::vector<SegDev> redo_segs;
             size_t nredo = 0;
-            if ((rc = build_segments(redo, false, redo_segs.data(), nredo, nullptr, err))) break;
+            descs_h.resize((size_t)max_segs);
+            if ((rc = build_segments(redo, false, redo_arena, descs_h.data(), nredo, nullptr, err))) break;
             redo_segs.resize(nredo);
+            expand_segments(descs_h.data(), nredo, redo_arena, redo_segs.data());
             size_t t2 = tpos, r2 = rpos, a2 = apos;
             for (SegDev &S : redo_segs) {
                 S.buf = b_segtext.as<uint8_t>() + t2;  t2 += al256((size_t)S.cap);
@@ -387,13 +431,13 @@
                 S.aux = b_segaux.as<uint8_t>() + a2;   a2 += al256(S.aux_cap);
             }
             if (t2 > seg_text_bound || r2 > seg_rec_bound || a2 > seg_aux_bound) {
-                segs.assign((size_t)max_segs, SegDev{});
                 size_t nall = 0;
-                if ((rc = build_segments(all, false, segs.data(), nall, nullptr, err))) break;
-                segs.resize(nall);
-                if ((rc = run_segments(segs.data(), segs.size(), false, err))) break;
+                if ((rc = build_segments(all, false, redo_arena, descs_h.data(), nall, nullptr, err))) break;
+                segs.assign(nall, SegDev{});
+                expand_segments(descs_h.data(), nall, redo_arena, segs.data());
+                if ((rc = run_segments(nullptr, segs.data(), segs.size(), redo_arena, false, err))) break;
             } else {
-                if ((rc = run_segments(redo_segs.data(), redo_segs.size(), false, err))) break;
+                if ((rc = run_segments(nullptr, redo_segs.data(), redo_segs.size(), redo_arena, false, err))) break;
                 segs = good;
                 segs.insert(segs.end(), redo_segs.begin(), redo_segs.end());
                 std::stable_sort(segs.begin(), segs.end(), [](const SegDev &a, const SegDev &b) {
@@ -499,13 +543,16 @@
                 HIPCHK(jk_stream_wait(st));
             }
         }
-        const bool carry = pass < passes;
+        const bool text_stays = qv_in_place && ordinary && !reads_caller_text;
         if (carry) HIPCHK(hipMemsetAsync(b_flags.p, 0, flag_items, st));
-        launch_seg_stitch(b_segs.as<SegDev>(), (int)ns, (uint8_t *const *)dOut, carry ? (uint8_t *const *)ptrClsOut : nullptr,
-                          carry ? (uint8_t *const *)ptrFlags : nullptr, st);
-        HIPCHK(hipGetLastError());
+        if (!text_stays) {
+            launch_seg_stitch(b_segs.as<SegDev>(), (int)ns, (uint8_t *const *)dOut, carry ? (uint8_t *const *)ptrClsOut : nullptr,
+                              carry ? (uint8_t *const *)ptrFlags : nullptr, st);
+            HIPCHK(hipGetLastError());
+        }
         for (int c = 0; c < n_chunks; ++c) len[c] = newlen[c];
         if (!ordinary) HIPCHK(jk_stream_wait(st));
+        if (text_stays) break;
         std::swap(hIn, hOut);
         std::swap(dIn, dOut);
         if (pass == 0) { hOut = hSpare; dOut = dSpare; }
@@ -561,17 +608,63 @@
                 }
             }
         }
-        std::stable_sort(R.recs.begin(), R.recs.end(), [](const FixRec &a, const FixRec &b) {
-            if (a.chunk != b.chunk) return a.chunk < b.chunk;
-            if (a.pass != b.pass) return a.pass < b.pass;
-            return a.seqno < b.seqno;
-        });
+        merge_record_runs(R.recs, rec_pass_begin, n_chunks);
     }
     (void)jk_stream_wait(st);
     if (dbg) fprintf(stderr, "[polish] D2H + record sort: %.2f ms; total %.2f ms\n", now() - t_out, now() - t_begin);
     (void)hipEventDestroy(ev0);
     (void)hipEventDestroy(ev1);
     return rc;
+}
+
+struct PolishWorkers {
+    std::mutex m;
+    std::condition_variable cv_job, cv_done;
+    std::vector<std::thread> th;
+    const std::function<void(int)> *job = nullptr;
+    uint64_t epoch = 0;
+    int lanes = 0, pending = 0;
+    bool stop = false;
+    void worker(int lane) {
+        uint64_t seen = 0;
+        std::unique_lock<std::mutex> lk(m);
+        for (;;) {
+            cv_job.wait(lk, [&] { return stop || epoch != seen; });
+            if (stop) return;
+            seen = epoch;
+            if (lane >= lanes) continue;
+            const std::function<void(int)> *f = job;
+            lk.unlock();
+            (*f)(lane);
+            lk.lock();
+            if (--pending == 0) cv_done.notify_one();
+        }
+    }
+    void run(int n, const std::function<void(int)> &f) {
+        {
+            std::lock_guard<std::mutex> lk(m);
+            while ((int)th.size() < n - 1) { const int lane = (int)th.size() + 1; th.emplace_back([this, lane] { worker(lane); }); }
+            job = &f;
+            lanes = n;
+            pending = n - 1;
+            ++epoch;
+        }
+        cv_job.notify_all();
+        f(0);
+        std::unique_lock<std::mutex> lk(m);
+        cv_done.wait(lk, [&] { return pending == 0; });
+        job = nullptr;
+    }
+};
+void polish_workers_free(PolishWorkers *w) {
+    if (!w) return;
+    {
+        std::lock_guard<std::mutex> lk(w->m);
+        w->stop = true;
+    }
+    w->cv_job.notify_all();
+    for (auto &t : w->th) t.join();
+    delete w;
 }
 
 int run_polish(Table &T, int n_chunks, const char *const *seqs, const int64_t *lens, int solid_thre, int passes, int fix,
@@ -609,16 +702,12 @@
     std::vector<std::vector<int64_t>> llens(lanes);
     for (int l = 0; l < lanes; ++l)
         for (int c : mine[l]) { lseqs[l].push_back(seqs[c]); llens[l].push_back(lens[c]); }
-    auto run = [&](int l) {
+    const std::function<void(int)> run = [&](int l) {
         rcs[l] = run_polish_lane(T, l, l ? T.polish_stream[l] : T.stream, (int)mine[l].size(), lseqs[l].data(), llens[l].data(), solid_thre, passes, fix, out[l],
                                  errs[l], device_in, keep_on_device, roomy);
     };
-    {
-        std::vector<std::thread> th;
-        for (int l = 1; l < lanes; ++l) th.emplace_back(run, l);
-        run(0);
-        for (auto &t : th) t.join();
-    }
+    if (!T.polish_workers) T.polish_workers = new PolishWorkers();
+    T.polish_workers->run(lanes, run);
     for (int want : {-1, -4, -2})
         for (int l = 0; l < lanes; ++l)
             if (rcs[l] == want) { err = errs[l]; return want; }
@@ -633,6 +722,7 @@
     R.qv[0] = R.qv[1] = R.qv[2] = R.qv[3] = 0;
     R.qv_chunk.assign((size_t)4 * n_chunks, 0);
     R.lookups = 0; R.seconds = 0; R.n_segments = 0; R.n_respeculated = 0;
+    std::vector<size_t> lane_begin;
     for (int l = 0; l < lanes; ++l) {
         PolishOut &O = out[l];
         for (size_t j = 0; j < mine[l].size(); ++j) {
@@ -642,6 +732,7 @@
             if (keep_on_device) { R.d_seqs[c] = O.d_seqs[j]; R.d_lens[c] = O.d_lens[j]; }
             for (int q = 0; q < 4; ++q) R.qv_chunk[4 * (size_t)c + q] = O.qv_chunk[4 * j + q];
         }
+        lane_begin.push_back(R.recs.size());
         for (FixRec f : O.recs) { f.chunk = (uint32_t)mine[l][f.chunk]; R.recs.push_back(f); }
         for (int q = 0; q < 4; ++q) R.qv[q] += O.qv[q];
         R.lookups += O.lookups;
@@ -649,11 +740,7 @@
         R.n_respeculated += O.n_respeculated;
         R.seconds = std::max(R.seconds, O.seconds);
     }
-    std::stable_sort(R.recs.begin(), R.recs.end(), [](const FixRec &a, const FixRec &b) {
-        if (a.chunk != b.chunk) return a.chunk < b.chunk;
-        if (a.pass != b.pass) return a.pass < b.pass;
-        return a.seqno < b.seqno;
-    });
+    merge_record_runs(R.recs, lane_begin, n_chunks);
     return 0;
 }
 
diff --git a/jasper_amd/csrc/polish_seg.hpp b/jasper_amd/csrc/polish_seg.hpp
--- /dev/null
+++ b/jasper_amd/csrc/polish_seg.hpp
@@ -0,0 +1,147 @@
+#pragma once
+#include <cstddef>
+#include <cstdint>
+
+#if defined(__HIPCC__)
+#define JK_SEG_HD __host__ __device__
+#else
+#define JK_SEG_HD
+#endif
+
+namespace jk {
+
+struct FixRec {
+    int64_t index;
+    uint32_t chunk;
+    uint32_t seqno;
+    uint8_t pass;
+    uint8_t kind;
+    uint8_t newc;
+    uint8_t oldc;
+    uint32_t rep;
+    uint32_t aux_off;
+    uint32_t aux_len;
+};
+static_assert(sizeof(FixRec) == 32, "FixRec layout");
+
+struct EditRec {
+    int64_t a;
+    int32_t plen, oldlen;
+};
+
+struct SegDev {
+    uint8_t *buf;
+    int64_t cap;
+    int64_t len;
+    int64_t gs, glen;
+    int64_t len0;
+    int64_t seg_lo;
+    int64_t start_i;
+    int64_t stop_orig;
+    int32_t first, last;
+    int32_t chain_in;
+    int32_t took_shortcut;
+    long long *arrive;
+    const uint8_t *cls;
+    int64_t cls_n;
+    FixRec *recs;
+    uint32_t rec_cap, nrec;
+    uint8_t *aux;
+    uint32_t aux_cap, naux;
+    EditRec *edits;
+    uint32_t edit_cap, nedit;
+    uint32_t chunk;
+    int32_t status;
+    int32_t spec_fail;
+    int64_t wrong;
+    uint64_t lookups;
+    uint64_t ticks;
+    uint64_t tk[12];
+    int64_t own_lo, own_hi;
+    int64_t own_hi0;
+    int64_t out_off;
+};
+
+struct SegDesc {
+    int64_t cut_lo, cut_hi;
+    uint64_t tpos, rpos, apos;
+    uint32_t chunk;
+    uint32_t flags;
+};
+enum : uint32_t { SD_FIRST = 1, SD_LAST = 2, SD_CHAIN = 4 };
+
+struct SegArena {
+    int32_t k;
+    int32_t tight;
+    int64_t RM;
+    int32_t in_place;
+    uint8_t *text;
+    FixRec *recs;
+    EditRec *edits;
+    uint8_t *aux;
+    long long *arrive;
+};
+
+struct SegGeom {
+    int64_t seg_lo, len0, cap;
+    uint32_t rec_cap, aux_cap;
+};
+JK_SEG_HD inline SegGeom seg_geometry(const SegDesc &D, int64_t chunk_len, const SegArena &A) {
+    const int64_t W = 4ll * A.k, M = 3ll * A.k;
+    SegGeom G;
+    G.seg_lo = (D.flags & SD_FIRST) ? 0 : D.cut_lo - W;
+    int64_t seg_hi = chunk_len;
+    if (!(D.flags & SD_LAST) && D.cut_hi + M < chunk_len) seg_hi = D.cut_hi + M;
+    G.len0 = seg_hi - G.seg_lo;
+    const int64_t eighth = G.len0 / 8;
+    G.cap = A.in_place ? G.len0 : G.len0 + (A.tight ? 2 : A.RM * (eighth > 1024 ? eighth : 1024));
+    const int64_t rc = A.RM * (2 * G.len0 / A.k + 16), ac = A.RM * (2 * G.len0 + 1024);
+    G.rec_cap = (uint32_t)(rc < 0x7fffffff ? rc : 0x7fffffff);
+    G.aux_cap = (uint32_t)(ac < 0x7fffffff ? ac : 0x7fffffff);
+    return G;
+}
+
+JK_SEG_HD inline void seg_expand(SegDev &S, const SegDesc &D, size_t index, int64_t chunk_len, const uint8_t *chunk_cls, const uint8_t *chunk_text,
+                             const SegArena &A) {
+    const bool first = (D.flags & SD_FIRST) != 0, last = (D.flags & SD_LAST) != 0;
+    const SegGeom G = seg_geometry(D, chunk_len, A);
+    const int64_t nwin = chunk_len - A.k + 1;
+    S.buf = A.in_place ? const_cast<uint8_t *>(chunk_text) + G.seg_lo : A.text + D.tpos;
+    S.cap = G.cap;
+    S.len = G.len0;
+    S.gs = A.in_place ? G.len0 : 0;
+    S.glen = G.cap - G.len0;
+    S.len0 = G.len0;
+    S.seg_lo = G.seg_lo;
+    S.start_i = first ? 0 : 4ll * A.k;
+    S.stop_orig = last ? INT64_MAX : D.cut_hi;
+    S.first = first;
+    S.last = last;
+    S.chain_in = (D.flags & SD_CHAIN) != 0;
+    S.took_shortcut = 0;
+    S.arrive = A.arrive + index + 1;
+    S.cls = nwin > 0 ? chunk_cls : nullptr;
+    S.cls_n = nwin > 0 ? nwin : 0;
+    S.recs = A.recs + D.rpos;
+    S.rec_cap = G.rec_cap;
+    S.nrec = 0;
+    S.aux = A.aux + D.apos;
+    S.aux_cap = G.aux_cap;
+    S.naux = 0;
+    S.edits = A.edits + D.rpos;
+    S.edit_cap = G.rec_cap;
+    S.nedit = 0;
+    S.chunk = D.chunk;
+    S.status = 0;
+    S.spec_fail = 0;
+    S.wrong = 0;
+    S.lookups = 0;
+    S.ticks = 0;
+    for (int q = 0; q < 12; ++q) S.tk[q] = 0;
+    S.own_lo = first ? 0 : 2ll * A.k;
+    S.own_hi = last ? -1 : (D.cut_hi - 2ll * A.k) - G.seg_lo;
+    S.own_hi0 = S.own_hi;
+    S.out_off = 0;
+}
+
+}
diff --git a/jasper_amd/csrc/table.hip b/jasper_amd/csrc/table.hip
--- a/jasper_amd/csrc/table.hip
+++ b/jasper_amd/csrc/table.hip
@@ -637,6 +637,8 @@
     (void)hipSetDevice(device);
     if (stream) (void)jk_stream_wait(stream);
     detach_shards();
+    polish_workers_free(polish_workers);
+    polish_workers = nullptr;
     for (hipStream_t &ps : polish_stream) { if (ps) { (void)jk_stream_wait(ps); (void)hipStreamDestroy(ps); ps = nullptr; } }
     if (polish_ev) { (void)hipEventDestroy(polish_ev); polish_ev = nullptr; }
     if (jf_stream) { (void)jk_stream_wait(jf_stream); (void)hipStreamDestroy(jf_stream); jf_stream = nullptr; }
diff --git a/jasper_amd/csrc/table.hpp b/jasper_amd/csrc/table.hpp
--- a/jasper_amd/csrc/table.hpp
+++ b/jasper_amd/csrc/table.hpp
@@ -6,6 +6,10 @@
 #include <vector>
 
 namespace jk {
+
+struct PolishWorkers;
+void polish_workers_free(PolishWorkers *w);
+
 
 extern std::atomic<int> g_cancel;
 
@@ -289,6 +293,7 @@
     hipStream_t polish_stream[POLISH_LANES_MAX] = {nullptr, nullptr, nullptr, nullptr};
     hipEvent_t polish_ev = nullptr;
     uint64_t polish_calls = 0;
+    struct PolishWorkers *polish_workers = nullptr;
     hipStream_t jf_stream = nullptr;
     hipStream_t ingest_stream = nullptr;
     hipStream_t ingest_copy_stream = nullptr;
```

Measured after the change: 3104 (median of 6 runs). No clear change (+1.6%).
